# lvxianwei/DeepMerge

Measured on AMD Instinct MI355X. Metric: superpixel-pairs/sec (train step), higher is better.
Workload: dtype bf16; 1 GPU; ShfitScaleFormer_v3 depth [3, 2, 1], scales [32, 64, 128, 256] x 4ch (256x256x4 patches), 32 pairs/GPU/step, fwd+loss+bwd+allreduce+Adam (BASELINE configs[1]); pairs_per_gpu=32, global_batch=32, parallelism=dp1

## Files before the change

deepmerge_amd/_lib.py:

```python
from __future__ import annotations

import ctypes as C
import os
import re
import threading

HERE = os.path.dirname(os.path.abspath(__file__))
ROOT = os.path.dirname(HERE)
LIB_PATH = os.path.join(HERE, "libdeepmerge_hip.so")
HEADER_PATH = os.path.join(ROOT, "include", "deepmerge_hip.h")

DM_F32, DM_BF16 = 0, 1
DM_NT, DM_NN, DM_TN = 0, 1, 2
DM_BF16_PAIR = 2
DM_F64 = 3
DM_EPI_NONE, DM_EPI_GELU, DM_EPI_DGELU, DM_EPI_GELU_GRAD, DM_EPI_MUL = 0, 1, 2, 3, 4

_STATUS = {-1: "bad shape", -2: "bad dtype", -3: "bad alignment", -4: "workspace", -5: "HIP error", -6: "unsupported"}


class DeepMergeLibraryError(RuntimeError):
    pass


class DmGemmArgs(C.Structure):
    _fields_ = [
        ("layout", C.c_int32), ("ab_dtype", C.c_int32), ("c_dtype", C.c_int32), ("aux_dtype", C.c_int32),
        ("M", C.c_int32), ("N", C.c_int32), ("K", C.c_int32),
        ("epilogue", C.c_int32), ("accumulate", C.c_int32), ("split_k", C.c_int32),
        ("A", C.c_void_p), ("lda", C.c_int64),
        ("B", C.c_void_p), ("ldb", C.c_int64),
        ("C", C.c_void_p), ("ldc", C.c_int64),
        ("bias", C.c_void_p),
        ("residual", C.c_void_p), ("ldr", C.c_int64),
        ("aux", C.c_void_p), ("ldaux", C.c_int64),
        ("rows_per_group", C.c_int32), ("group_stride", C.c_int64),
        ("workspace", C.c_void_p), ("workspace_bytes", C.c_int64),
        ("colsum_a", C.c_void_p), ("colsum_accumulate", C.c_int32),
        ("k_fold", C.c_int32), ("a_fold", C.c_int64 * 3), ("b_fold", C.c_int64 * 3),
        ("c_plane", C.c_int64),
    ]


class DmReduceItem(C.Structure):
    _fields_ = [("partial", C.c_void_p), ("out0", C.c_void_p), ("out1", C.c_void_p),
                ("nrows", C.c_int32), ("width", C.c_int32), ("split", C.c_int32), ("accumulate", C.c_int32)]


class DmPairDraw(C.Structure):
    _fields_ = [("pairs", C.c_void_p), ("pair_flag", C.c_void_p), ("poly_off", C.c_void_p), ("poly_pts", C.c_void_p),
                ("pt_tile", C.c_void_p), ("pt_xy", C.c_void_p), ("pt_inner", C.c_void_p), ("pt_obj", C.c_void_p),
                ("pt_region", C.c_void_p),
                ("tile_id", C.c_void_p), ("xy", C.c_void_p), ("inner", C.c_void_p), ("obj", C.c_void_p),
                ("region", C.c_void_p), ("flag", C.c_void_p),
                ("point_id", C.c_void_p),
                ("seed", C.c_uint64),
                ("n_pairs", C.c_int32), ("n_poly", C.c_int32), ("n_poly_pts", C.c_int32), ("n_pts", C.c_int32),
                ("epoch", C.c_int32), ("batch", C.c_int32)]


class DmMergeFold(C.Structure):
    _fields_ = [("ptr", C.c_void_p), ("idx", C.c_void_p), ("edges", C.c_void_p), ("root", C.c_void_p), ("pick", C.c_void_p),
                ("rep", C.c_void_p), ("region_of", C.c_void_p),
                ("simi", C.c_void_p), ("weights", C.c_void_p),
                ("count", C.c_void_p), ("sum", C.c_void_p), ("sumsq", C.c_void_p), ("bbox", C.c_void_p), ("peri", C.c_void_p),
                ("new_id", C.c_void_p), ("hist_rank", C.c_void_p), ("new_ptr", C.c_void_p), ("new_idx", C.c_void_p),
                ("new_rep", C.c_void_p), ("new_region_of", C.c_void_p), ("n_regions", C.c_void_p),
                ("new_count", C.c_void_p), ("new_sum", C.c_void_p), ("new_sumsq", C.c_void_p), ("new_bbox", C.c_void_p),
                ("new_peri", C.c_void_p),
                ("history", C.c_void_p), ("history_simi", C.c_void_p),
                ("C", C.c_int32), ("P", C.c_int32), ("E", C.c_int32), ("S0", C.c_int32), ("bands", C.c_int32), ("round", C.c_int32),
                ("hist_base", C.c_int32), ("hist_cap", C.c_int32)]


class DmVectorTrace(C.Structure):
    _fields_ = [("dart", C.c_void_p), ("next", C.c_void_p), ("lab", C.c_void_p), ("other", C.c_void_p), ("flags", C.c_void_p),
                ("key", C.c_void_p), ("sum", C.c_void_p), ("ring_of_slot", C.c_void_p), ("ring_ptr", C.c_void_p),
                ("arc_base", C.c_void_p), ("xy", C.c_void_p), ("area2", C.c_void_p),
                ("arc_first", C.c_void_p), ("arc_left", C.c_void_p), ("arc_right", C.c_void_p), ("arc_vstart", C.c_void_p),
                ("arc_count", C.c_void_p), ("arc_pos", C.c_void_p), ("arc_ptr", C.c_void_p), ("arc_xy", C.c_void_p),
                ("W", C.c_int32), ("D", C.c_int32), ("R", C.c_int32), ("n_arcs", C.c_int32)]


class DmSceneVectorTrace(C.Structure):
    _fields_ = [("dart", C.c_void_p), ("next", C.c_void_p), ("lab", C.c_void_p), ("other", C.c_void_p), ("flags", C.c_void_p),
                ("key", C.c_void_p), ("sum", C.c_void_p), ("ring_of_slot", C.c_void_p), ("ring_ptr", C.c_void_p),
                ("arc_base", C.c_void_p), ("xy", C.c_void_p), ("area2", C.c_void_p),
                ("arc_first", C.c_void_p), ("arc_left", C.c_void_p), ("arc_right", C.c_void_p), ("arc_vstart", C.c_void_p),
                ("arc_count", C.c_void_p), ("arc_pos", C.c_void_p), ("arc_ptr", C.c_void_p), ("arc_xy", C.c_void_p),
                ("W", C.c_int64), ("D", C.c_int32), ("R", C.c_int32), ("n_arcs", C.c_int32)]


class DmSceneSimplifyRings(C.Structure):
    _fields_ = [("xy", C.c_void_p), ("ring_ptr", C.c_void_p), ("vert_ring", C.c_void_p), ("node_row", C.c_void_p), ("node_col", C.c_void_p),
                ("kept_row", C.c_void_p), ("status", C.c_void_p),
                ("n_nodes", C.c_int64), ("n_kept", C.c_int64), ("scene_h", C.c_int64), ("scene_w", C.c_int64),
                ("V", C.c_int32), ("R", C.c_int32)]


class DmSimplifyTopology(C.Structure):
    _fields_ = [("arc_xy", C.c_void_p), ("arc_ptr", C.c_void_p), ("new_ptr", C.c_void_p), ("keep", C.c_void_p),
                ("point_count", C.c_void_p), ("point_fill", C.c_void_p), ("point_ptr", C.c_void_p), ("point_xy", C.c_void_p),
                ("seg", C.c_void_p), ("kind", C.c_void_p), ("cell_count", C.c_void_p), ("cell_fill", C.c_void_p),
                ("cell_ptr", C.c_void_p), ("cell_seg", C.c_void_p), ("stack", C.c_void_p), ("status", C.c_void_p),
                ("Va", C.c_int64), ("cap", C.c_int64), ("A", C.c_int32), ("H", C.c_int32), ("W", C.c_int32), ("q", C.c_int32)]


class DmSceneSimplifyTopology(C.Structure):
    _fields_ = [("arc_xy", C.c_void_p), ("arc_ptr", C.c_void_p), ("new_ptr", C.c_void_p), ("arc_keep", C.c_void_p),
                ("point_count", C.c_void_p), ("point_fill", C.c_void_p), ("point_ptr", C.c_void_p), ("point_xy", C.c_void_p),
                ("seg", C.c_void_p), ("kind", C.c_void_p), ("cell_count", C.c_void_p), ("cell_fill", C.c_void_p),
                ("cell_ptr", C.c_void_p), ("cell_seg", C.c_void_p), ("stack", C.c_void_p), ("status", C.c_void_p),
                ("Va", C.c_int64), ("cap", C.c_int64), ("A", C.c_int32), ("H", C.c_int32), ("W", C.c_int32), ("q", C.c_int32),
                ("cell_log2", C.c_int32)]


class DmProfRow(C.Structure):
    _fields_ = [("name", C.c_char * 64), ("launches", C.c_int64), ("total_ms", C.c_double),
                ("total_flops", C.c_double), ("total_bytes", C.c_double)]


_P, _I, _L, _F, _D = C.c_void_p, C.c_int32, C.c_int64, C.c_float, C.c_double

SIGNATURES = {
    "dm_abi_version": (_I, []),
    "dm_last_error": (C.c_char_p, []),
    "dm_arch": (C.c_char_p, []),
    "dm_gemm": (_I, [C.POINTER(DmGemmArgs), _P]),
    "dm_gemm_workspace_bytes": (_L, [_I, _I, _I, _I]),
    "dm_gemm_grouped": (_I, [C.POINTER(DmGemmArgs), _I, _P]),
    "dm_attention_fwd": (_I, [_P, _P, _P, _P, _I, _I, _I, _I, _F, _I, _P]),
    "dm_attention_relpos_inkernel": (_I, [_I, _I, _I, _I, _I, _I, _I, _I]),
    "dm_attention_fwd_relpos": (_I, [_P, _P, _I, _I, _I, _P, _P, _I, _I, _I, _I, _F, _I, _P]),
    "dm_attention_split_ok": (_I, [_I, _I, _I, _I, _I, _I, _I, _I]),
    "dm_attention_split_fwd": (_I, [_P, _P, _P, _P, _I, _I, _I, _P, _P, _I, _I, _I, _I, _F, _P]),
    "dm_attention_split_fwd_pair": (_I, [_P, _P, _P, _P, _I, _I, _I, _P, _P, _P, _I, _I, _I, _I, _F, _P]),
    "dm_attention_split_bwd_chunks": (_I, [_I, _I, _I]),
    "dm_attention_split_bwd": (_I, [_P, _P, _P, _I, _I, _I, _P, _P, _P, _P, _P, _P, _P, _P, _I, _I, _I, _I, _F, _P]),
    "dm_attention_split_bwd_pair": (_I, [_P, _P, _P, _I, _I, _I, _P, _P, _P, _P, _P, _P, _P, _P, _I, _I, _I, _I, _F, _P]),
    "dm_attention_bwd_relpos": (_I, [_P, _P, _I, _I, _I, _P, _P, _P, _P, _P, _P, _P, _P, _I, _I, _I, _I, _F, _I, _P]),
    "dm_attention_bwd": (_I, [_P, _P, _P, _P, _P, _P, _P, _P, _P, _I, _I, _I, _I, _F, _I, _P]),
    "dm_attention_bwd_batch_chunks": (_I, [_I, _I, _I, _I]),
    "dm_relpos_bias_gather": (_I, [_P, _P, _P, _P, _I, _I, _I, _P]),
    "dm_relpos_bias_reduce": (_I, [_P, _P, _P, _P, _I, _I, _I, _I, _I, _P]),
    "dm_layernorm_fwd": (_I, [_P, _P, _P, _P, _I, _P, _P, _I, _I, _F, _P]),
    "dm_layernorm_bwd": (_I, [_P, _I, _P, _P, _P, _P, _P, _P, _P, _P, _P, _I, _P, _I, _I, _P]),
    "dm_layernorm_bwd_partials": (_I, [_P, _I, _P, _P, _P, _P, _P, _P, _P, _P, _I, _I, C.POINTER(C.c_int32), _P]),
    "dm_layernorm_bwd_partials_pair": (_I, [_P, _I, _P, _P, _P, _P, _P, _P, _P, _P, _I, _I, C.POINTER(C.c_int32), _P]),
    "dm_layernorm_bwd_partials_regroup": (_I, [_P, _I, _P, _P, _P, _P, _P, _P, _P, _P, _I, _I, _I, _I, C.POINTER(C.c_int32), _P]),
    "dm_pool_layernorm_ok": (_I, [_I]),
    "dm_pool_layernorm_fwd": (_I, [_P, _P, _P, _P, _P, _P, _P, _I, _I, _I, _I, _F, _P]),
    "dm_pool_layernorm_bwd": (_I, [_P, _P, _P, _P, _P, _P, _P, _P, _P, _I, _P, C.POINTER(C.c_int32), _I, _I, _I, _I, _P]),
    "dm_partial_reduce_batch": (_I, [C.POINTER(DmReduceItem), _I, _P]),
    "dm_layernorm_bwd_partial_floats": (_L, [_I]),
    "dm_token_pool_fwd": (_I, [_P, _P, _I, _I, _I, _I, _P]),
    "dm_token_pool_bwd": (_I, [_P, _P, _I, _I, _I, _I, _P]),
    "dm_group_mean_fwd": (_I, [_P, _P, _I, _I, _I, _P]),
    "dm_group_mean_bwd": (_I, [_P, _P, _I, _I, _I, _P]),
    "dm_colsum": (_I, [_P, _I, _L, _P, _I, _I, _I, _P, _P]),
    "dm_colsum_partial_floats": (_L, [_I]),
    "dm_cast": (_I, [_P, _P, _I, _L, _P]),
    "dm_split_bf16": (_I, [_P, _L, _L, _L, _P, _I, _I, _P]),
    "dm_split_colsum_partial_floats": (_L, [_L, _L]),
    "dm_split_bf16_colsum": (_I, [_P, _L, _L, _L, _P, _I, _I, _P, _P, _P]),
    "dm_split_bf16_planes": (_I, [_P, _L, _L, _L, _P, _P, _P, _P]),
    "dm_patchify": (_I, [_P, _P, _I, _I, _I, _I, _I, _P]),
    "dm_contrastive_loss": (_I, [_P, _P, _P, _F, _F, _P, _P, _P, _I, _I, _P]),
    "dm_cross_entropy": (_I, [_P, _P, _P, _F, _P, _P, _I, _I, _P]),
    "dm_batchnorm_workspace_bytes": (_L, [_I, _I]),
    "dm_batchnorm_fwd": (_I, [_P, _P, _P, _P, _P, _P, _I, _P, _P, _P, _I, _I, _F, _F, _I, _I, _P, _P]),
    "dm_batchnorm_bwd": (_I, [_P, _P, _P, _P, _P, _I, _P, _P, _P, _P, _P, _I, _I, _I, _I, _I, _P, _P]),
    "dm_adam_step": (_I, [_P, _P, _P, _P, _P, _L, _I, _D, _D, _D, _D, _D, _P]),
    "dm_adam_hyper": (_I, [_I, _D, _D, _D, _P]),
    "dm_adam_step_dev": (_I, [_P, _P, _P, _P, _P, _L, _P, _D, _D, _D, _D, _P]),
    "dm_adam_step_dev_pair": (_I, [_P, _P, _P, _P, _P, _P, _L, _P, _D, _D, _D, _D, _P]),
    "dm_segment_mean": (_I, [_P, _P, _P, _P, _I, _I, _P]),
    "dm_edge_similarity": (_I, [_P, _P, _P, _P, _I, _I, _F, _P]),
    "dm_pairwise_distance": (_I, [_P, _P, _P, _I, _I, _I, _I, _P]),
    "dm_patch_pyramid": (_I, [_P, _I, _I, _I, _P, _P, _I, _I, _I, _I, _P, _P]),
    "dm_patch_pyramid_cols": (_I, [_P, _I, _I, _I, _P, _P, _I, _I, _I, _I, _I, _P, _I, _P]),
    "dm_pair_batch_gather": (_I, [_P, _I, _I, _I, _I, _P, _P, _P, _P, _I, _I, _I, _I, _I, _I, _P, _I, _P, _P, _P, _P]),
    "dm_pair_epoch_draw": (_I, [C.POINTER(DmPairDraw), _P]),
    "dm_contrastive_terms": (_I, [_P, _P, _P, _F, _P, _P, _I, _I, _P]),
    "dm_pair_eval_workspace_bytes": (_L, [_L, _I]),
    "dm_pair_eval_summary": (_I, [_P, _P, _P, _L, _P, _I, _P, _P, _P, _P, _P]),
    "dm_label_stats": (_I, [_P, _P, _I, _I, _I, _I, _P, _P, _P, _P, _P, _P]),
    "dm_label_features": (_I, [_P, _P, _P, _P, _P, _I, _I, _P, _P]),
    "dm_rag_edges": (_I, [_P, _I, _I, _I, _P, _P, _I, _P, _P, _I, _P, _P, _P]),
    "dm_seam_stitch": (_I, [_P, _P, _L, _L, _P, _P, _P, _I, _P, _P, _I, _P, _P, _P]),
    "dm_merge_round": (_I, [_P, _P, _I, _I, _P, _P, _I, _P]),
    "dm_merge_best": (_I, [_P, _P, _I, _I, _F, _P, _P]),
    "dm_merge_match": (_I, [_P, _P, _I, _I, _P, _P, _P, _P, _P]),
    "dm_merge_fold_regions": (_I, [C.POINTER(DmMergeFold), _P]),
    "dm_merge_edge_keys": (_I, [_P, _P, _P, _I, _I, _P, _P]),
    "dm_merge_fold_edges": (_I, [_P, _P, _P, _I, _P, _P, _P, _P]),
    "dm_relabel_raster": (_I, [_P, _P, _P, _L, _I, _P]),
    "dm_region_merge_cost": (_I, [_P, _P, _P, _P, _P, _P, _P, _I, _I, _I, _D, _D, _D, _D, _D, _P, _P]),
    "dm_pixel_regions": (_I, [_P, _I, _I, _I, _P, _P, _P, _P, _P, _P, _P, _P]),
    "dm_label_clearance": (_I, [_P, _I, _I, _I, _P, _P, _P, _P]),
    "dm_point_select_round": (_I, [_P, _P, _I, _I, _I, _I, _I, _P, _P, _P, _P, _P, _P]),
    "dm_point_emit": (_I, [_P, _P, _P, _P, _I, _I, _I, _I, _P, _P, _P, _P, _P, _P, _P]),
    "dm_scene_point_init": (_I, [_P, _P, _P, _I, _P]),
    "dm_scene_point_select": (_I, [_P, _P, _I, _I, _I, _I, _I, _I, _L, _L, _L, _L, _I, _I, _I, _P, _P, _P, _P, _P]),
    "dm_scene_point_commit": (_I, [_P, _L, _L, _I, _I, _P, _P, _P, _P]),
    "dm_label_overlap": (_I, [_P, _P, _I, _I, _L, _L, _P, _P, _I, _P, _P, _I, _P, _P, _P]),
    "dm_overlap_reduce": (_I, [_P, _P, _I, _L, _L, _P, _P, _P, _P, _P, _P, _P, _P, _P]),
    "dm_pair_flags": (_I, [_P, _I, _P, _P, _P, _I, _I, _P, _P]),
    "dm_boundary_bits": (_I, [_P, _I, _I, _I, _P, _P, _P, _P]),
    "dm_boundary_counts": (_I, [_P, _P, _P, _I, _I, _I, _I, _I, _I, _I, _P, _P]),
    "dm_slic_iterate": (_I, [_P, _I, _I, _I, _I, _I, _I, _P, _P, _P, _P]),
    "dm_connected_labels": (_I, [_P, _I, _I, _I, _I, _P, _P, _P, _P, _P]),
    "dm_label_area": (_I, [_P, _I, _I, _I, _P, _P]),
    "dm_slic_absorb_pick": (_I, [_P, _P, _I, _P, _I, _I, _P, _P, _P, _P]),
    "dm_scene_slic_init": (_I, [_P, _I, _I, _I, _I, _I, _I, _I, _I, _P, _P, _P]),
    "dm_scene_slic_pass": (_I, [_P, _I, _I, _I, _I, _I, _I, _I, _I, _I, _P, _P, _P, _P]),
    "dm_scene_slic_update": (_I, [_I, _P, _P, _P]),
    "dm_vector_count": (_I, [_P, _I, _I, _P, _P, _P, _P]),
    "dm_vector_emit": (_I, [_P, _P, _I, _I, _P, _P, _P]),
    "dm_vector_link": (_I, [_P, _P, _P, _P, _I, _I, _I, _P, _P, _P, _P, _P, _P]),
    "dm_vector_head_round": (_I, [_P, _P, _P, _P, _I, _P, _P]),
    "dm_vector_rank_init": (_I, [_P, _P, _P, _P, _I, _P, _P, _P, _P, _P, _I, _P]),
    "dm_vector_rank_round": (_I, [_P, _P, _P, _P, _I, _P, _P]),
    "dm_vector_ring_emit": (_I, [C.POINTER(DmVectorTrace), _P]),
    "dm_vector_arc_emit": (_I, [C.POINTER(DmVectorTrace), _P]),
    "dm_scene_vector_count": (_I, [_P, _I, _I, _I, _I, _I, _I, _P, _P, _P, _P, _P]),
    "dm_scene_vector_link": (_I, [_P, _P, _P, _I, _I, _I, _L, _L, _L, _L, _P, _P, _P, _P, _P, _P]),
    "dm_scene_vector_ring_emit": (_I, [C.POINTER(DmSceneVectorTrace), _P]),
    "dm_scene_vector_arc_emit": (_I, [C.POINTER(DmSceneVectorTrace), _P]),
    "dm_rasterize_count": (_I, [_P, _P, _P, _I, _I, _I, _I, _P, _P]),
    "dm_rasterize_emit": (_I, [_P, _P, _P, _P, _P, _I, _I, _L, _I, _I, _L, _P, _P]),
    "dm_rasterize_fill": (_I, [_P, _L, _I, _I, _I, _P, _P, _P]),
    "dm_rasterize_count_rows": (_I, [_P, _P, _P, _I, _I, _I, _I, _I, _I, _P, _P]),
    "dm_rasterize_emit_rows": (_I, [_P, _P, _P, _P, _P, _I, _I, _L, _I, _I, _I, _I, _L, _P, _P]),
    "dm_rasterize_fill_window": (_I, [_P, _L, _I, _I, _I, _I, _I, _I, _I, _P, _P, _P]),
    "dm_simplify_nodes": (_I, [_P, _I, _I, _P, _P]),
    "dm_simplify_chains": (_I, [_P, _P, _I, _L, _I, _I, _I, _P, _P, _P]),
    "dm_simplify_arc_count": (_I, [_P, _P, _I, _L, _I, _I, _P, _P, _P]),
    "dm_simplify_arc_emit": (_I, [_P, _P, _P, _I, _L, _L, _I, _I, _P, _P, _P]),
    "dm_simplify_ring_count": (_I, [_P, _P, _P, _I, _I, _I, _I, _P, _P, _P]),
    "dm_simplify_ring_emit": (_I, [_P, _P, _P, _P, _P, _I, _I, _L, _I, _I, _P, _P, _P, _P]),
    "dm_simplify_topology_point_count": (_I, [C.POINTER(DmSimplifyTopology), _P]),
    "dm_simplify_topology_point_fill": (_I, [C.POINTER(DmSimplifyTopology), _P]),
    "dm_simplify_topology_segments": (_I, [C.POINTER(DmSimplifyTopology), _P]),
    "dm_simplify_topology_bin_count": (_I, [C.POINTER(DmSimplifyTopology), _P]),
    "dm_simplify_topology_bin_fill": (_I, [C.POINTER(DmSimplifyTopology), _P]),
    "dm_simplify_topology_pairs": (_I, [C.POINTER(DmSimplifyTopology), _P]),
    "dm_simplify_topology_jumps": (_I, [C.POINTER(DmSimplifyTopology), _P]),
    "dm_simplify_topology_refine": (_I, [C.POINTER(DmSimplifyTopology), _I, _P]),
    "dm_scene_simplify_node_count": (_I, [_P, _I, _I, _I, _I, _I, _I, _L, _L, _L, _L, _P, _P, _P]),
    "dm_scene_simplify_node_emit": (_I, [_P, _I, _I, _I, _I, _I, _I, _L, _L, _L, _L, _P, _I, _P, _P]),
    "dm_scene_simplify_chains": (_I, [_P, _P, _I, _L, _L, _L, _I, _P, _P, _P]),
    "dm_scene_simplify_arc_count": (_I, [_P, _P, _I, _L, _L, _L, _P, _P, _P]),
    "dm_scene_simplify_arc_emit": (_I, [_P, _P, _P, _I, _L, _L, _L, _L, _P, _P, _P]),
    "dm_scene_simplify_ring_count": (_I, [C.POINTER(DmSceneSimplifyRings), _P, _P]),
    "dm_scene_simplify_ring_emit": (_I, [C.POINTER(DmSceneSimplifyRings), _P, _P, _L, _P, _P, _P]),
    "dm_scene_simplify_topology_point_count": (_I, [C.POINTER(DmSceneSimplifyTopology), _P]),
    "dm_scene_simplify_topology_point_fill": (_I, [C.POINTER(DmSceneSimplifyTopology), _P]),
    "dm_scene_simplify_topology_segments": (_I, [C.POINTER(DmSceneSimplifyTopology), _P]),
    "dm_scene_simplify_topology_bin_count": (_I, [C.POINTER(DmSceneSimplifyTopology), _P]),
    "dm_scene_simplify_topology_bin_fill": (_I, [C.POINTER(DmSceneSimplifyTopology), _P]),
    "dm_scene_simplify_topology_pairs": (_I, [C.POINTER(DmSceneSimplifyTopology), _P]),
    "dm_scene_simplify_topology_jumps": (_I, [C.POINTER(DmSceneSimplifyTopology), _P]),
    "dm_scene_simplify_topology_refine": (_I, [C.POINTER(DmSceneSimplifyTopology), _I, _P]),
    "dm_gru_cell_fwd": (_I, [_P, _L, _P, _P, _P, _P, _I, _I, _P]),
    "dm_gru_cell_bwd": (_I, [_P, _P, _P, _P, _P, _P, _I, _I, _P]),
    "dm_prof_enable": (_I, [_I]),
    "dm_prof_collect": (_I, [C.POINTER(DmProfRow), _I]),
}

_lock = threading.Lock()
_lib = None


def declared_symbols(header_path: str = HEADER_PATH):
    text = open(header_path).read()
    text = re.sub(r"/\*.*?\*/", "", text, flags=re.S)
    return sorted(set(re.findall(r"\b(dm_[a-z0-9_]+)\s*\(", text)))


def lib() -> C.CDLL:
    global _lib
    if _lib is not None:
        return _lib
    with _lock:
        if _lib is not None:
            return _lib
        if not os.path.exists(LIB_PATH):
            raise DeepMergeLibraryError(
                f"{LIB_PATH} not found: build the HIP kernels first "
                f"(`python -c 'import __graft_entry__ as g; g.build()'` or `make -C deepmerge_amd/csrc`). "
                f"deepmerge_amd has no CPU fallback.")
        try:
            handle = C.CDLL(LIB_PATH)
        except OSError as e:
            raise DeepMergeLibraryError(f"cannot load {LIB_PATH}: {e}") from e
        for name, (res, args) in SIGNATURES.items():
            try:
                fn = getattr(handle, name)
            except AttributeError as e:
                raise DeepMergeLibraryError(f"{LIB_PATH} does not export {name}") from e
            fn.restype = res
            fn.argtypes = args
        if handle.dm_abi_version() != 7:
            raise DeepMergeLibraryError(f"ABI version mismatch: library {handle.dm_abi_version()} != 7")
        _lib = handle
        return _lib
# ... 11 lines not shown
```

deepmerge_amd/csrc/dm_rows.hip:

```cpp
#include <cstdlib>

#include "dm_common.h"

int dm_layernorm_wide_fwd(const float *x, const float *gamma, const float *beta, void *y, int y_dtype, float *mean, float *rstd, int rows,
                          int cols, float eps, hipStream_t s);
int dm_layernorm_wide_bwd(const void *dy, int dy_dtype, const float *x, const float *gamma, const float *mean, const float *rstd,
                          const float *dres, float *dx, void *dx_lp, float *partial, int max_slices, int *slices, int rows, int cols,
                          hipStream_t s);
int dm_patchify_any(const float *x, void *cols, int dtype, int B, int C, int side, int p, hipStream_t s);

namespace {

constexpr int MAXCH = 4;
constexpr int LN_WIDE_MAX = 8192;
static int ln_max_wg() {
  static const int v = [] { const char *e = getenv("DM_LN_WG"); return e ? atoi(e) : 768; }();
  return v;
}
constexpr int CS_MAX_SLICES = 64;

template <typename T> struct Raw4;
template <> struct Raw4<float> { typedef f32x4 type; };
template <> struct Raw4<bf16_t> { typedef bf16x4 type; };
template <typename T>
__device__ __forceinline__ typename Raw4<T>::type dm_load_raw4(const T *p) { return *reinterpret_cast<const typename Raw4<T>::type *>(p); }
__device__ __forceinline__ f32x4 dm_widen4(f32x4 v) { return v; }
__device__ __forceinline__ f32x4 dm_widen4(bf16x4 v) { return (f32x4){(float)v[0], (float)v[1], (float)v[2], (float)v[3]}; }

template <typename TY, bool PAIR, int CH, bool FULL, bool POOL = false>
__global__ __launch_bounds__(256) void layernorm_fwd_kernel(const float *__restrict__ x, const float *__restrict__ gamma,
                                                            const float *__restrict__ beta, TY *__restrict__ y,
                                                            float *__restrict__ mean_out, float *__restrict__ rstd_out,
                                                            int rows, int cols, float eps, float *__restrict__ pooled = nullptr, int pool_side = 0) {
  __shared__ f32x4 gb[2][CH * 64];
  const int lane = threadIdx.x & 63, wave = __builtin_amdgcn_readfirstlane(threadIdx.x >> 6);
  const int nch = cols >> 2;
  for (int c = threadIdx.x; c < nch; c += 256) {
    gb[0][c] = dm_load4(gamma + 4 * c);
    gb[1][c] = dm_load4(beta + 4 * c);
  }
  __syncthreads();
  const int stride = gridDim.x * 4;
  int row = blockIdx.x * 4 + wave;
  if (row >= rows) return;
  auto request = [&](int r, f32x4(&dst)[CH]) __attribute__((always_inline)) {
    if constexpr (POOL) {
      const int half = pool_side >> 1, px = r % half, q = r / half, py = q % half, bs = q / half;
      const float *src = x + (((long long)bs * pool_side + 2 * py) * pool_side + 2 * px) * cols;
      const long long down = (long long)pool_side * cols;
      float *pr = pooled + (long long)r * cols;
#pragma unroll
      for (int i = 0; i < CH; ++i) {
        const int c = lane + 64 * i;
        if (FULL || c < nch) {
          const f32x4 a = dm_load4(src + 4 * c), b = dm_load4(src + cols + 4 * c), d = dm_load4(src + down + 4 * c), e = dm_load4(src + down + cols + 4 * c);
          dst[i] = ((a + b) + (d + e)) * 0.25f;
          dm_store4(pr + 4 * c, dst[i]);
        } else {
          dst[i] = (f32x4){0.f, 0.f, 0.f, 0.f};
        }
      }
      return;
    }
    const float *xr = x + (long long)r * cols;
#pragma unroll
    for (int i = 0; i < CH; ++i) {
      const int c = lane + 64 * i;
      dst[i] = (FULL || c < nch) ? dm_load4(xr + 4 * c) : (f32x4){0.f, 0.f, 0.f, 0.f};
    }
  };
  auto finish = [&](int row, const f32x4(&v)[CH]) __attribute__((always_inline)) {
    float s = 0.f;
#pragma unroll
    for (int i = 0; i < CH; ++i) s += (v[i][0] + v[i][1]) + (v[i][2] + v[i][3]);
    const float mean = dm_wave_sum(s) / (float)cols;
    float q = 0.f;
#pragma unroll
    for (int i = 0; i < CH; ++i) {
      const int c = lane + 64 * i;
      if (FULL || c < nch) {
#pragma unroll
        for (int e = 0; e < 4; ++e) {
          const float d = v[i][e] - mean;
          q += d * d;
        }
      }
    }
    const float rstd = rsqrtf(dm_wave_sum(q) / (float)cols + eps);
    if (lane == 0) {
      mean_out[row] = mean;
      rstd_out[row] = rstd;
    }
    TY *yr = y + (long long)row * cols;
#pragma unroll
    for (int i = 0; i < CH; ++i) {
      const int c = lane + 64 * i;
      if (FULL || c < nch) {
        int cl = c;
        asm volatile("" : "+v"(cl));
        const f32x4 g = gb[0][cl], b = gb[1][cl];
        f32x4 o;
#pragma unroll
        for (int e = 0; e < 4; ++e) o[e] = (v[i][e] - mean) * rstd * g[e] + b[e];
        if constexpr (PAIR) {
          bf16x4 h, l;
#pragma unroll
          for (int e = 0; e < 4; ++e) {
            h[e] = (bf16_t)o[e];
            l[e] = (bf16_t)(o[e] - (float)h[e]);
          }
          *reinterpret_cast<bf16x4 *>(yr + 4 * c) = h;
          *reinterpret_cast<bf16x4 *>(yr + (long long)rows * cols + 4 * c) = l;
        } else {
          dm_store4(yr + 4 * c, o);
        }
      }
    }
  };
  f32x4 v[CH], nv[CH];
  if constexpr (!FULL || POOL) {
    for (; row < rows; row += stride) {
      request(row, v);
      finish(row, v);
    }
    return;
  }
  request(row, v);
  int next = row + stride;
  if (next < rows) request(next, nv);
  finish(row, v);
  while (next < rows) {
    row = next;
    next = row + stride;
#pragma unroll
    for (int i = 0; i < CH; ++i) v[i] = nv[i];
    if (next < rows) request(next, nv);
    finish(row, v);
  }
}

template <typename TDY, int CH, bool FULL, bool POOL = false>
__global__ __launch_bounds__(256) void layernorm_bwd_kernel(const TDY *__restrict__ dy, const float *__restrict__ x,
                                                            const float *__restrict__ gamma, const float *__restrict__ mean,
                                                            const float *__restrict__ rstd, const float *__restrict__ dres,
                                                            float *__restrict__ dx, bf16_t *__restrict__ dx_lp,
                                                            float *__restrict__ partial, int rows, int cols, long long lp_plane,
                                                            int pool_side = 0, int rg_s = 0, int rg_t = 0) {
  __shared__ float red[4][2][CH * 256];
  const int lane = threadIdx.x & 63, wave = __builtin_amdgcn_readfirstlane(threadIdx.x >> 6);
  const int nch = cols >> 2;
  f32x4 dg[CH], db[CH], gam[CH];
#pragma unroll
  for (int i = 0; i < CH; ++i) {
    dg[i] = db[i] = (f32x4){0.f, 0.f, 0.f, 0.f};
    const int c = lane + 64 * i;
    gam[i] = (FULL || c < nch) ? dm_load4(gamma + 4 * c) : (f32x4){0.f, 0.f, 0.f, 0.f};
  }
  f32x4 rx[CH], rdr[CH];
  typename Raw4<TDY>::type rdy[CH];
  float rmu = 0.f, rrs = 0.f;
  auto request = [&](int row) __attribute__((always_inline)) {
    const long long off = (long long)row * cols;
    rmu = mean[row];
    rrs = rstd[row];
#pragma unroll
    for (int i = 0; i < CH; ++i) {
      const int c = lane + 64 * i;
      rdr[i] = (dres && (FULL || c < nch)) ? dm_load4(dres + off + 4 * c) : (f32x4){0.f, 0.f, 0.f, 0.f};
    }
#pragma unroll
    for (int i = 0; i < CH; ++i) {
      const int c = lane + 64 * i;
      if (FULL || c < nch) {
        rx[i] = dm_load4(x + off + 4 * c);
        rdy[i] = dm_load_raw4(dy + off + 4 * c);
      }
    }
  };
  f32x4 xh[CH], g[CH], dr[CH];
  float rs = 0.f, s1 = 0.f, s2 = 0.f;
  auto consume = [&]() __attribute__((always_inline)) {
    const float mu = rmu;
    rs = rrs;
    s1 = s2 = 0.f;
#pragma unroll
    for (int i = 0; i < CH; ++i) {
      const int c = lane + 64 * i;
      dr[i] = rdr[i];
      if (FULL || c < nch) {
        const f32x4 xv = rx[i];
        const f32x4 d = dm_widen4(rdy[i]);
#pragma unroll
        for (int e = 0; e < 4; ++e) {
          xh[i][e] = (xv[e] - mu) * rs;
          g[i][e] = d[e] * gam[i][e];
          s1 += g[i][e];
          s2 += g[i][e] * xh[i][e];
          dg[i][e] += d[e] * xh[i][e];
          db[i][e] += d[e];
        }
      } else {
        xh[i] = g[i] = (f32x4){0.f, 0.f, 0.f, 0.f};
      }
    }
  };
  auto finish = [&](int row) __attribute__((always_inline)) {
    const long long off = (long long)row * cols;
    float t1 = s1, t2 = s2;
#pragma unroll
    for (int o = 32; o > 0; o >>= 1) {
      const float u1 = __shfl_xor(t1, o, 64), u2 = __shfl_xor(t2, o, 64);
      t1 += u1;
      t2 += u2;
    }
    const float c1 = t1 / (float)cols, c2 = t2 / (float)cols;
    if constexpr (POOL) {
      const int half = pool_side >> 1, px = row % half, q = row / half, py = q % half, bs = q / half;
      const long long base = (((long long)bs * pool_side + 2 * py) * pool_side + 2 * px) * cols, down = (long long)pool_side * cols;
#pragma unroll
      for (int i = 0; i < CH; ++i) {
        const int c = lane + 64 * i;
        if (FULL || c < nch) {
          f32x4 o;
#pragma unroll
          for (int e = 0; e < 4; ++e) o[e] = rs * (g[i][e] - c1 - xh[i][e] * c2);
          o = o * 0.25f;
          const long long at[4] = {base, base + cols, base + down, base + down + cols};
#pragma unroll
          for (int k = 0; k < 4; ++k) {
            dm_store4(dx + at[k] + 4 * c, o);
            if (dx_lp) dm_store4(dx_lp + at[k] + 4 * c, o);
          }
        }
      }
      return;
    }
    long long off_lp = off;
    if (rg_t > 0) {
      const int st = rg_s * rg_t, b = row / st, rem = row - b * st, sc = rem / rg_t, t = rem - sc * rg_t;
      off_lp = ((long long)(sc * (rows / st) + b) * rg_t + t) * cols;
    }
#pragma unroll
    for (int i = 0; i < CH; ++i) {
      const int c = lane + 64 * i;
      if (FULL || c < nch) {
        f32x4 o;
#pragma unroll
        for (int e = 0; e < 4; ++e) o[e] = rs * (g[i][e] - c1 - xh[i][e] * c2);
        if (dres) o += dr[i];
        dm_store4(dx + off + 4 * c, o);
        if (dx_lp) {
          if (lp_plane > 0) {
            bf16x4 h, l;
#pragma unroll
            for (int e = 0; e < 4; ++e) {
              h[e] = (bf16_t)o[e];
              l[e] = (bf16_t)(o[e] - (float)h[e]);
            }
            *reinterpret_cast<bf16x4 *>(dx_lp + off + 4 * c) = h;
            *reinterpret_cast<bf16x4 *>(dx_lp + lp_plane + off + 4 * c) = l;
          } else {
            dm_store4(dx_lp + off_lp + 4 * c, o);
          }
        }
      }
    }
  };
  int row = blockIdx.x * 4 + wave;
  const int stride = gridDim.x * 4;
  if constexpr (CH == MAXCH) {
    for (; row < rows; row += stride) {
      request(row);
      consume();
      finish(row);
    }
  } else if (row < rows) {
    request(row);
    consume();
    for (;;) {
      const int next = row + stride;
      if (next < rows) request(next);
      finish(row);
      if (next >= rows) break;
      row = next;
      consume();
    }
  }
#pragma unroll
  for (int i = 0; i < CH; ++i) {
#pragma unroll
    for (int e = 0; e < 4; ++e) {
      red[wave][0][(lane + 64 * i) * 4 + e] = dg[i][e];
      red[wave][1][(lane + 64 * i) * 4 + e] = db[i][e];
    }
  }
  __syncthreads();
  float *prow = partial + (long long)blockIdx.x * 2 * cols;
  for (int c = threadIdx.x; c < 2 * cols; c += 256) {
    const int which = c / cols, col = c % cols;
    prow[c] = (red[0][which][col] + red[1][which][col]) + (red[2][which][col] + red[3][which][col]);
  }
}

__global__ __launch_bounds__(256) void partial_reduce_kernel(const float *__restrict__ partial, float *__restrict__ out0,
                                                             float *__restrict__ out1, int nrows, int width, int split,
                                                             int accumulate) {
  __shared__ float red[16][17];
  const int tx = threadIdx.x & 15, ty = threadIdx.x >> 4;
  const int j = blockIdx.x * 16 + tx;
  float s = 0.f;
  if (j < width) {
    float s0 = 0.f, s1 = 0.f, s2 = 0.f, s3 = 0.f;
    int r = ty;
    for (; r + 48 < nrows; r += 64) {
      s0 += partial[(long long)r * width + j];
      s1 += partial[(long long)(r + 16) * width + j];
      s2 += partial[(long long)(r + 32) * width + j];
      s3 += partial[(long long)(r + 48) * width + j];
    }
    for (; r < nrows; r += 16) s0 += partial[(long long)r * width + j];
    s = (s0 + s1) + (s2 + s3);
  }
  red[ty][tx] = s;
  __syncthreads();
  if (ty == 0 && j < width) {
    float t[16];
#pragma unroll
    for (int k = 0; k < 16; ++k) t[k] = red[k][tx];
#pragma unroll
    for (int w = 8; w > 0; w >>= 1)
#pragma unroll
      for (int k = 0; k < w; ++k) t[k] = t[2 * k] + t[2 * k + 1];
    s = t[0];
    float *o = (j < split) ? out0 + j : out1 + (j - split);
    *o = accumulate ? *o + s : s;
  }
}

struct ReduceBatch {
  DmReduceItem it[32];
  int start[33];
  int n;
};
__global__ __launch_bounds__(256) void partial_reduce_batch_kernel(const ReduceBatch rb) {
  __shared__ float red[16][17];
  int job = 0;
  while (job + 1 < rb.n && (int)blockIdx.x >= rb.start[job + 1]) ++job;
  const DmReduceItem &it = rb.it[job];
  const float *__restrict__ partial = it.partial;
  const int nrows = it.nrows, width = it.width;
  const int tx = threadIdx.x & 15, ty = threadIdx.x >> 4;
  const int j = ((int)blockIdx.x - rb.start[job]) * 16 + tx;
  float s = 0.f;
  if (j < width) {
    float s0 = 0.f, s1 = 0.f, s2 = 0.f, s3 = 0.f;
    int r = ty;
    for (; r + 48 < nrows; r += 64) {
      s0 += partial[(long long)r * width + j];
      s1 += partial[(long long)(r + 16) * width + j];
      s2 += partial[(long long)(r + 32) * width + j];
      s3 += partial[(long long)(r + 48) * width + j];
    }
    for (; r < nrows; r += 16) s0 += partial[(long long)r * width + j];
    s = (s0 + s1) + (s2 + s3);
  }
  red[ty][tx] = s;
  __syncthreads();
  if (ty == 0 && j < width) {
    float t[16];
#pragma unroll
    for (int k = 0; k < 16; ++k) t[k] = red[k][tx];
#pragma unroll
    for (int w = 8; w > 0; w >>= 1)
#pragma unroll
      for (int k = 0; k < w; ++k) t[k] = t[2 * k] + t[2 * k + 1];
    s = t[0];
    float *o = (j < it.split) ? it.out0 + j : it.out1 + (j - it.split);
    *o = it.accumulate ? *o + s : s;
  }
}

__global__ void token_pool_fwd_kernel(const float *__restrict__ x, float *__restrict__ y, int B, int S, int side, int C) {
  const int half = side >> 1, c4 = C >> 2;
  const long long total = (long long)B * S * half * half * c4;
  for (long long i = (long long)blockIdx.x * blockDim.x + threadIdx.x; i < total; i += (long long)gridDim.x * blockDim.x) {
    const int c = (int)(i % c4);
    long long r = i / c4;
    const int px = (int)(r % half); r /= half;
    const int py = (int)(r % half); r /= half;
    const float *src = x + ((r * side + 2 * py) * side + 2 * px) * (long long)C + 4 * c;
    const f32x4 a = dm_load4(src), b = dm_load4(src + C), d = dm_load4(src + (long long)side * C), e = dm_load4(src + (long long)side * C + C);
    dm_store4(y + ((r * half + py) * half + px) * (long long)C + 4 * c, ((a + b) + (d + e)) * 0.25f);
  }
}
__global__ void token_pool_bwd_kernel(const float *__restrict__ dy, float *__restrict__ dx, int B, int S, int side, int C) {
  const int half = side >> 1, c4 = C >> 2;
  const long long total = (long long)B * S * side * side * c4;
  for (long long i = (long long)blockIdx.x * blockDim.x + threadIdx.x; i < total; i += (long long)gridDim.x * blockDim.x) {
    const int c = (int)(i % c4);
    long long r = i / c4;
    const int xx = (int)(r % side); r /= side;
    const int yy = (int)(r % side); r /= side;
    const f32x4 g = dm_load4(dy + ((r * half + (yy >> 1)) * half + (xx >> 1)) * (long long)C + 4 * c);
    dm_store4(dx + ((r * side + yy) * side + xx) * (long long)C + 4 * c, g * 0.25f);
  }
}
__global__ void group_mean_fwd_kernel(const float *__restrict__ x, float *__restrict__ y, int rows, int g, int C) {
  const int c4 = C >> 2;
  const long long total = (long long)rows * c4;
  const float inv = 1.0f / (float)g;
  for (long long i = (long long)blockIdx.x * blockDim.x + threadIdx.x; i < total; i += (long long)gridDim.x * blockDim.x) {
    const int c = (int)(i % c4);
    const long long r = i / c4;
    f32x4 s = {0.f, 0.f, 0.f, 0.f};
    for (int k = 0; k < g; ++k) s += dm_load4(x + (r * g + k) * C + 4 * c);
    dm_store4(y + r * C + 4 * c, s * inv);
  }
}
__global__ void group_mean_bwd_kernel(const float *__restrict__ dy, float *__restrict__ dx, int rows, int g, int C) {
  const int c4 = C >> 2;
  const long long total = (long long)rows * g * c4;
  const float inv = 1.0f / (float)g;
  for (long long i = (long long)blockIdx.x * blockDim.x + threadIdx.x; i < total; i += (long long)gridDim.x * blockDim.x) {
    const int c = (int)(i % c4);
    const long long r = i / c4;
    dm_store4(dx + r * C + 4 * c, dm_load4(dy + (r / g) * C + 4 * c) * inv);
  }
}

template <typename T>
__global__ __launch_bounds__(256) void colsum_kernel(const T *__restrict__ X, long long ldx, float *__restrict__ partial,
                                                     int M, int N, int rows_per_slice, int direct) {
  __shared__ f32x4 red[16][16];
  const int tx = threadIdx.x & 15, ty = threadIdx.x >> 4;
  const int n = blockIdx.x * 64 + tx * 4;
  const int r0 = blockIdx.y * rows_per_slice, r1 = min(M, r0 + rows_per_slice);
  f32x4 s = {0.f, 0.f, 0.f, 0.f};
  if (n < N)
    for (int r = r0 + ty; r < r1; r += 16) s += dm_load4(X + (long long)r * ldx + n);
  red[ty][tx] = s;
  __syncthreads();
  if (ty == 0 && n < N) {
    f32x4 a = red[0][tx];
#pragma unroll
    for (int k = 1; k < 16; ++k) a += red[k][tx];
    if (direct == 1) a = dm_load4(partial + n) + a;
    dm_store4(partial + (long long)blockIdx.y * N + n, a);
  }
}

template <typename T>
__global__ __launch_bounds__(256) void colsum_generic_kernel(const T *__restrict__ X, long long ldx, float *__restrict__ partial,
                                                             int M, int N, int rows_per_slice) {
  const int n = blockIdx.x * 256 + threadIdx.x;
  if (n >= N) return;
  const int r0 = blockIdx.y * rows_per_slice, r1 = min(M, r0 + rows_per_slice);
  float s = 0.f;
  for (int r = r0; r < r1; ++r) s += (float)X[(long long)r * ldx + n];
  partial[(long long)blockIdx.y * N + n] = s;
}

__global__ void cast_bf16_kernel(const float *__restrict__ src, bf16_t *__restrict__ dst, long long n) {
  const long long n8 = n >> 3;
  for (long long i = (long long)blockIdx.x * blockDim.x + threadIdx.x; i < n8; i += (long long)gridDim.x * blockDim.x) {
    const f32x4 a = dm_load4(src + 8 * i), b = dm_load4(src + 8 * i + 4);
    bf16x8 o = {(bf16_t)a[0], (bf16_t)a[1], (bf16_t)a[2], (bf16_t)a[3], (bf16_t)b[0], (bf16_t)b[1], (bf16_t)b[2], (bf16_t)b[3]};
    *reinterpret_cast<bf16x8 *>(dst + 8 * i) = o;
  }
  if (blockIdx.x == 0 && threadIdx.x < (n & 7)) dst[(n8 << 3) + threadIdx.x] = (bf16_t)src[(n8 << 3) + threadIdx.x];
}
__global__ void split_bf16_kernel(const float *__restrict__ src, long long ld, long long rows, long long cols, bf16_t *__restrict__ dst,
                                  int stack, int pattern) {
  const long long c4 = cols >> 2, total = rows * c4;
  const long long piece = stack ? rows * cols : cols, ldd = stack ? cols : 3 * cols;
  for (long long i = (long long)blockIdx.x * blockDim.x + threadIdx.x; i < total; i += (long long)gridDim.x * blockDim.x) {
    const long long r = i / c4, c = (i - r * c4) << 2;
    const f32x4 x = dm_load4(src + r * ld + c);
    bf16x4 hi, lo;
#pragma unroll
    for (int j = 0; j < 4; ++j) {
      hi[j] = (bf16_t)x[j];
      lo[j] = (bf16_t)(x[j] - (float)hi[j]);
    }
    bf16_t *d = dst + r * ldd + c;
#pragma unroll
    for (int j = 0; j < 3; ++j) *reinterpret_cast<bf16x4 *>(d + j * piece) = ((pattern >> j) & 1) ? lo : hi;
  }
}
template <bool CS>
__global__ __launch_bounds__(256) void split_bf16_rows_kernel(const float *__restrict__ src, long long ld, int rows, int cols,
                                                              bf16_t *__restrict__ dst, int stack, int pattern, float *__restrict__ partial, int pieces) {
  __shared__ float red[CS ? 8 : 1][CS ? 264 : 1];
  const int c = (blockIdx.x * 32 + threadIdx.x) * 8;
  const bool live = c < cols;
  if (!CS && !live) return;
  const long long piece = stack ? (long long)rows * cols : cols, ldd = stack ? cols : 3LL * cols;
  float cs[8] = {0.f, 0.f, 0.f, 0.f, 0.f, 0.f, 0.f, 0.f};
  for (int r = blockIdx.y * 8 + threadIdx.y; live && r < rows; r += gridDim.y * 8) {
    const float *sp = src + (long long)r * ld + c;
    const f32x4 x0 = dm_load4(sp), x1 = dm_load4(sp + 4);
    if constexpr (CS) {
#pragma unroll
      for (int j = 0; j < 4; ++j) { cs[j] += x0[j]; cs[4 + j] += x1[j]; }
    }
    u32x4 hi, lo;
#pragma unroll
    for (int j = 0; j < 4; ++j) {
      const float a = j < 2 ? x0[2 * j] : x1[2 * j - 4], b = j < 2 ? x0[2 * j + 1] : x1[2 * j - 3];
      const bf16x2 h2 = {(bf16_t)a, (bf16_t)b};
      const bf16x2 l2 = {(bf16_t)(a - (float)h2[0]), (bf16_t)(b - (float)h2[1])};
      hi[j] = __builtin_bit_cast(unsigned, h2);
      lo[j] = __builtin_bit_cast(unsigned, l2);
    }
    bf16_t *d = dst + (long long)r * ldd + c;
#pragma unroll
    for (int j = 0; j < 3; ++j)
      if (j < pieces) *reinterpret_cast<u32x4 *>(d + j * piece) = ((pattern >> j) & 1) ? lo : hi;
  }
  if constexpr (CS) {
#pragma unroll
    for (int j = 0; j < 8; ++j) red[threadIdx.y][threadIdx.x * 8 + j] = cs[j];
    __syncthreads();
    if (threadIdx.y == 0 && live) {
#pragma unroll
      for (int j = 0; j < 8; ++j) {
        const int x = threadIdx.x * 8 + j;
        partial[(long long)blockIdx.y * cols + c + j] = ((red[0][x] + red[1][x]) + (red[2][x] + red[3][x])) + ((red[4][x] + red[5][x]) + (red[6][x] + red[7][x]));
      }
    }
  }
}
__global__ void copy_f32_kernel(const float *__restrict__ src, float *__restrict__ dst, long long n) {
  const long long n4 = n >> 2;
  for (long long i = (long long)blockIdx.x * blockDim.x + threadIdx.x; i < n4; i += (long long)gridDim.x * blockDim.x)
    dm_store4(dst + 4 * i, dm_load4(src + 4 * i));
  if (blockIdx.x == 0 && threadIdx.x < (n & 3)) dst[(n4 << 2) + threadIdx.x] = src[(n4 << 2) + threadIdx.x];
}

template <typename T>
__global__ void patchify_kernel(const float *__restrict__ x, T *__restrict__ cols, int B, int C, int side, int p) {
  const int grid = side / p, p4 = p >> 2;
  const long long K = (long long)C * p * p;
  const long long total = (long long)B * grid * grid * (K >> 2);
  for (long long i = (long long)blockIdx.x * blockDim.x + threadIdx.x; i < total; i += (long long)gridDim.x * blockDim.x) {
    long long r = i;
    const int dx4 = (int)(r % p4); r /= p4;
    const int dy = (int)(r % p); r /= p;
    const int c = (int)(r % C); r /= C;
    const int px = (int)(r % grid);
    const long long bp = r / grid;
    const int py = (int)(bp % grid);
    const long long b = bp / grid;
    const f32x4 v = dm_load4(x + ((b * C + c) * side + (py * p + dy)) * (long long)side + px * p + 4 * dx4);
    dm_store4(cols + r * K + ((long long)c * p + dy) * p + 4 * dx4, v);
  }
}

__global__ __launch_bounds__(256) void contrastive_loss_kernel(const float *__restrict__ a, const float *__restrict__ b,
                                                               const float *__restrict__ flag, float margin, float upstream,
                                                               float *__restrict__ loss, float *__restrict__ da,
                                                               float *__restrict__ db, int B, int D) {
  __shared__ float wsum[4];
  const int lane = threadIdx.x & 63, wave = threadIdx.x >> 6;
  float acc = 0.f;
  const float gscale = upstream / (float)B;
  for (int r = wave; r < B; r += 4) {
    float d = 0.f;
    for (int c = lane; c < D; c += 64) {
      const float t = a[(long long)r * D + c] - b[(long long)r * D + c];
      d += t * t;
    }
    d = dm_wave_sum(d);
    const float f = flag[r];
    const float hinge = margin - d;
    acc += f * d + (1.f - f) * fmaxf(hinge, 0.f);
    if (da) {
      const float coef = (f - (1.f - f) * (hinge > 0.f ? 1.f : 0.f)) * 2.f * gscale;
      for (int c = lane; c < D; c += 64) {
        const float t = a[(long long)r * D + c] - b[(long long)r * D + c];
        da[(long long)r * D + c] = coef * t;
        db[(long long)r * D + c] = -coef * t;
      }
    }
  }
  if (lane == 0) wsum[wave] = acc;
  __syncthreads();
  if (threadIdx.x == 0) loss[0] = ((wsum[0] + wsum[1]) + (wsum[2] + wsum[3])) / (float)B;
}

__global__ __launch_bounds__(256) void cross_entropy_kernel(const float *__restrict__ logits, const long long *__restrict__ tidx,
                                                            const float *__restrict__ tprob, float upstream,
                                                            float *__restrict__ loss, float *__restrict__ dlogits, int B, int K) {
  __shared__ float wsum[4];
  const int lane = threadIdx.x & 63, wave = threadIdx.x >> 6;
  const float gscale = upstream / (float)B;
  float acc = 0.f;
  for (int r = wave; r < B; r += 4) {
    const float *x = logits + (long long)r * K;
    float mx = -INFINITY;
    for (int c = lane; c < K; c += 64) mx = fmaxf(mx, x[c]);
    mx = dm_wave_max(mx);
    float se = 0.f;
    for (int c = lane; c < K; c += 64) se += expf(x[c] - mx);
    se = dm_wave_sum(se);
    const float lse = mx + logf(se);
    float l = 0.f, psum = 0.f;
    if (tidx) {
      const long long t = tidx[r];
      if (lane == 0) l = lse - x[t];
      psum = 1.f;
    } else {
      const float *q = tprob + (long long)r * K;
      for (int c = lane; c < K; c += 64) { l += q[c] * (lse - x[c]); psum += q[c]; }
      psum = dm_wave_sum(psum);
    }
    acc += dm_wave_sum(l);
    if (dlogits) {
      float *g = dlogits + (long long)r * K;
      for (int c = lane; c < K; c += 64) {
        const float sm = expf(x[c] - lse);
        const float tgt = tidx ? ((long long)c == tidx[r] ? 1.f : 0.f) : tprob[(long long)r * K + c];
        g[c] = (sm * psum - tgt) * gscale;
      }
    }
  }
  if (lane == 0) wsum[wave] = acc;
  __syncthreads();
  if (threadIdx.x == 0) loss[0] = ((wsum[0] + wsum[1]) + (wsum[2] + wsum[3])) / (float)B;
}

__global__ void adam_kernel(float *__restrict__ param, const float *__restrict__ grad, float *__restrict__ m,
                            float *__restrict__ v, bf16_t *__restrict__ lp, long long n, float beta1, float beta2,
                            float omb1, float omb2, float eps, float step_size, float bc2_sqrt, float grad_scale,
                            const float *__restrict__ hyper, bf16_t *__restrict__ lo = nullptr) {
  if (hyper) {
    step_size = hyper[0];
    bc2_sqrt = hyper[1];
  }
  const long long n4 = n >> 2;
  for (long long i = (long long)blockIdx.x * blockDim.x + threadIdx.x; i < n4; i += (long long)gridDim.x * blockDim.x) {
    f32x4 p = __builtin_nontemporal_load(reinterpret_cast<const f32x4 *>(param + 4 * i));
    f32x4 g = __builtin_nontemporal_load(reinterpret_cast<const f32x4 *>(grad + 4 * i)) * grad_scale;
    f32x4 mm = __builtin_nontemporal_load(reinterpret_cast<const f32x4 *>(m + 4 * i)), vv = __builtin_nontemporal_load(reinterpret_cast<const f32x4 *>(v + 4 * i));
#pragma unroll
    for (int e = 0; e < 4; ++e) {
      mm[e] = mm[e] * beta1 + g[e] * omb1;
      vv[e] = vv[e] * beta2 + (g[e] * g[e]) * omb2;
      const float denom = sqrtf(vv[e]) / bc2_sqrt + eps;
      p[e] = p[e] - step_size * (mm[e] / denom);
    }
    __builtin_nontemporal_store(p, reinterpret_cast<f32x4 *>(param + 4 * i));
    __builtin_nontemporal_store(mm, reinterpret_cast<f32x4 *>(m + 4 * i));
    __builtin_nontemporal_store(vv, reinterpret_cast<f32x4 *>(v + 4 * i));
    if (lp) dm_store4(lp + 4 * i, p);
    if (lo) {
      bf16x4 l;
#pragma unroll
      for (int e = 0; e < 4; ++e) l[e] = (bf16_t)(p[e] - (float)(bf16_t)p[e]);
      *reinterpret_cast<bf16x4 *>(lo + 4 * i) = l;
    }
  }
  if (blockIdx.x == 0 && threadIdx.x < (n & 3)) {
    const long long i = (n4 << 2) + threadIdx.x;
    const float g = grad[i] * grad_scale;
    const float mm = m[i] * beta1 + g * omb1;
    const float vv = v[i] * beta2 + (g * g) * omb2;
    const float p = param[i] - step_size * (mm / (sqrtf(vv) / bc2_sqrt + eps));
    param[i] = p; m[i] = mm; v[i] = vv;
    if (lp) lp[i] = (bf16_t)p;
    if (lo) lo[i] = (bf16_t)(p - (float)(bf16_t)p);
  }
}

__global__ void relpos_gather_kernel(const float *__restrict__ table, const int *__restrict__ index,
                                     float *__restrict__ bias, float *__restrict__ bias_t, int N, int H, int n_bins) {
  const int NN = N * N;
  for (int ij = blockIdx.x * blockDim.x + threadIdx.x; ij < NN; ij += gridDim.x * blockDim.x) {
    int bin = index[ij];
    bin = min(max(bin, 0), n_bins - 1);
    for (int h = 0; h < H; ++h) bias[(long long)h * NN + ij] = table[bin * H + h];
    if (bias_t) {
      const int i = ij / N, j = ij % N;
      int bt = index[j * N + i];
      bt = min(max(bt, 0), n_bins - 1);
      for (int h = 0; h < H; ++h) bias_t[(long long)h * NN + ij] = table[bt * H + h];
    }
  }
}
template <int U>
__device__ __forceinline__ void chunk_add(f32x4 &v, const float *slab, long long plane4, long long i, int c) {
  f32x4 a[U];
#pragma unroll
  for (int u = 0; u < U; ++u) a[u] = dm_load4(slab + ((long long)(c + u) * plane4 + i) * 4);
#pragma unroll
  for (int u = 0; u < U; ++u) v += a[u];
}
__global__ void chunk_sum_kernel(float *__restrict__ slab, long long plane4, int chunks) {
  for (long long i = (long long)blockIdx.x * blockDim.x + threadIdx.x; i < plane4; i += (long long)gridDim.x * blockDim.x) {
    f32x4 v = dm_load4(slab + 4 * i);
    int c = 1;
    for (; c + 8 <= chunks; c += 8) chunk_add<8>(v, slab, plane4, i, c);
    if (c + 4 <= chunks) { chunk_add<4>(v, slab, plane4, i, c); c += 4; }
    if (c + 2 <= chunks) { chunk_add<2>(v, slab, plane4, i, c); c += 2; }
    if (c < chunks) chunk_add<1>(v, slab, plane4, i, c);
    dm_store4(slab + 4 * i, v);
  }
}

__global__ __launch_bounds__(256) void relpos_reduce_kernel(const float *__restrict__ slab, const int *__restrict__ pos,
                                                            const int *__restrict__ off, float *__restrict__ dtable, int chunks,
                                                            int H, int N, int n_bins, int accumulate) {
  const int lane = threadIdx.x & 63, wave = threadIdx.x >> 6;
  const int bin = blockIdx.x, h = blockIdx.y * 4 + wave;
  if (h >= H) return;
  const int beg = off[bin], cnt = off[bin + 1] - beg;
  const long long plane = (long long)N * N;
  float acc = 0.f;
  for (int c = 0; c < chunks; ++c) {
    const float *pl = slab + ((long long)c * H + h) * plane;
#pragma unroll 4
    for (int j = lane; j < cnt; j += 64) acc += pl[pos[beg + j]];
  }
  acc = dm_wave_sum(acc);
  if (lane == 0) {
    float *o = dtable + (long long)bin * H + h;
    *o = accumulate ? *o + acc : acc;
  }
}

inline int grid_for(long long work_items, int block = 256, int cap = 4096) {
  long long g = (work_items + block - 1) / block;
  if (g < 1) g = 1;
  if (g > cap) g = cap;
  return (int)g;
}

static int adam_grid(long long n) {
  static const int cap = [] { const char *e = getenv("DM_ADAM_GRID"); return e ? atoi(e) : 16384; }();
  return grid_for(n / 4 + 1, 256, cap);
}

}

extern "C" int dm_layernorm_fwd(const float *x, const float *gamma, const float *beta, void *y, int32_t y_dtype,
                                float *mean, float *rstd, int32_t rows, int32_t cols, float eps, void *stream) {
  DM_REQUIRE(rows > 0 && cols > 0 && cols % 4 == 0 && cols <= LN_WIDE_MAX, DM_ERR_BAD_SHAPE,
             "dm_layernorm_fwd: rows=%d cols=%d (cols must be a multiple of 4, <= %d)", rows, cols, LN_WIDE_MAX);
  DM_REQUIRE(x && gamma && beta && y && mean && rstd, DM_ERR_BAD_SHAPE, "dm_layernorm_fwd: null pointer");
  hipStream_t s = reinterpret_cast<hipStream_t>(stream);
  if (cols > MAXCH * 256) {
    DM_REQUIRE(y_dtype != DM_BF16_PAIR, DM_ERR_UNSUPPORTED, "dm_layernorm_fwd: a plane-pair result needs cols <= %d", MAXCH * 256);
    const int rc = dm_layernorm_wide_fwd(x, gamma, beta, y, y_dtype, mean, rstd, rows, cols, eps, s);
    DM_REQUIRE(rc == DM_OK, rc, "dm_layernorm_fwd: bad y_dtype %d", y_dtype);
    DM_LAUNCH_CHECK("dm_layernorm_fwd(wide)");
    return DM_OK;
  }
  const int grid = grid_for((long long)rows, 4, 2048);
  const bool full3 = cols == 768;
#define DM_LN_FWD(T, PAIR_)                                                                                                                \
  do {                                                                                                                                     \
    if (full3)                                                                                                                             \
      hipLaunchKernelGGL((layernorm_fwd_kernel<T, PAIR_, 3, true>), dim3(grid), dim3(256), 0, s, x, gamma, beta, (T *)y, mean, rstd, rows, cols, eps); \
    else                                                                                                                                   \
      hipLaunchKernelGGL((layernorm_fwd_kernel<T, PAIR_, MAXCH, false>), dim3(grid), dim3(256), 0, s, x, gamma, beta, (T *)y, mean, rstd, rows, cols, eps); \
  } while (0)
  if (y_dtype == DM_F32) DM_LN_FWD(float, false);
  else if (y_dtype == DM_BF16) DM_LN_FWD(bf16_t, false);
  else if (y_dtype == DM_BF16_PAIR) DM_LN_FWD(bf16_t, true);
  else DM_REQUIRE(false, DM_ERR_BAD_DTYPE, "dm_layernorm_fwd: bad y_dtype %d", y_dtype);
#undef DM_LN_FWD
  DM_LAUNCH_CHECK("dm_layernorm_fwd");
  return DM_OK;
}

extern "C" int64_t dm_layernorm_bwd_partial_floats(int32_t cols) { return (int64_t)ln_max_wg() * 2 * cols; }

static int ln_bwd_main(const void *dy, int32_t dy_dtype, const float *x, const float *gamma, const float *mean, const float *rstd,
                       const float *dres, float *dx, void *dx_lp, float *partial, int32_t rows, int32_t cols, int32_t *n_partial, hipStream_t s,
                       const char *who, bool lp_pair = false, int pool_side = 0, int rg_s = 0, int rg_t = 0) {
  const long long lp_plane = lp_pair ? (long long)rows * cols : 0;
  DM_REQUIRE(!lp_pair || (dx_lp && cols <= MAXCH * 256), DM_ERR_UNSUPPORTED, "%s: the plane-pair copy needs dx_lp and cols <= %d", who, MAXCH * 256);
  DM_REQUIRE(rows > 0 && cols > 0 && cols % 4 == 0 && cols <= LN_WIDE_MAX, DM_ERR_BAD_SHAPE, "%s: rows=%d cols=%d", who, rows, cols);
  DM_REQUIRE(dy && x && gamma && mean && rstd && dx && partial && n_partial, DM_ERR_BAD_SHAPE, "%s: null pointer", who);
  if (cols > MAXCH * 256) {
    int slices = 0;
    const int rc = dm_layernorm_wide_bwd(dy, dy_dtype, x, gamma, mean, rstd, dres, dx, dx_lp, partial, ln_max_wg(), &slices, rows, cols, s);
    DM_REQUIRE(rc == DM_OK, rc, "%s: bad dy_dtype %d", who, dy_dtype);
    DM_LAUNCH_CHECK("dm_layernorm_bwd(wide)");
    *n_partial = slices;
    return DM_OK;
  }
  const int grid = grid_for((long long)rows, 4, ln_max_wg());
  DM_REQUIRE(dy_dtype == DM_F32 || dy_dtype == DM_BF16, DM_ERR_BAD_DTYPE, "%s: bad dy_dtype %d", who, dy_dtype);
  if (pool_side > 0) {
    hipLaunchKernelGGL((layernorm_bwd_kernel<float, 3, true, true>), dim3(grid), dim3(256), 0, s, (const float *)dy, x, gamma, mean, rstd, (const float *)nullptr,
                       dx, (bf16_t *)dx_lp, partial, rows, cols, 0LL, pool_side, 0, 0);
    DM_LAUNCH_CHECK("dm_pool_layernorm_bwd");
    *n_partial = grid;
    return DM_OK;
  }
  const bool narrow = cols <= 768, full = cols == 768;
#define DM_LN_BWD(T, CH_, FULL_)                                                                                                      \
  hipLaunchKernelGGL((layernorm_bwd_kernel<T, CH_, FULL_>), dim3(grid), dim3(256), 0, s, (const T *)dy, x, gamma, mean, rstd, dres, dx, \
                     (bf16_t *)dx_lp, partial, rows, cols, lp_plane, 0, rg_s, rg_t)
  if (dy_dtype == DM_F32) {
    if (full) DM_LN_BWD(float, 3, true);
    else if (narrow) DM_LN_BWD(float, 3, false);
    else DM_LN_BWD(float, MAXCH, false);
  } else {
    if (full) DM_LN_BWD(bf16_t, 3, true);
    else if (narrow) DM_LN_BWD(bf16_t, 3, false);
    else DM_LN_BWD(bf16_t, MAXCH, false);
  }
#undef DM_LN_BWD
  DM_LAUNCH_CHECK("dm_layernorm_bwd");
  *n_partial = grid;
  return DM_OK;
}

extern "C" int dm_layernorm_bwd(const void *dy, int32_t dy_dtype, const float *x, const float *gamma, const float *mean,
                                const float *rstd, const float *dres, float *dx, void *dx_lp, float *dgamma, float *dbeta,
                                int32_t accumulate_params, float *partial, int32_t rows, int32_t cols, void *stream) {
  DM_REQUIRE(dgamma && dbeta, DM_ERR_BAD_SHAPE, "dm_layernorm_bwd: null pointer");
  hipStream_t s = reinterpret_cast<hipStream_t>(stream);
  int32_t slices = 0;
  if (const int rc = ln_bwd_main(dy, dy_dtype, x, gamma, mean, rstd, dres, dx, dx_lp, partial, rows, cols, &slices, s, "dm_layernorm_bwd")) return rc;
  hipLaunchKernelGGL(partial_reduce_kernel, dim3((2 * cols + 15) / 16), dim3(256), 0, s, partial, dgamma, dbeta, slices, 2 * cols, cols, accumulate_params);
  DM_LAUNCH_CHECK("dm_layernorm_bwd(reduce)");
  return DM_OK;
}

extern "C" int dm_layernorm_bwd_partials(const void *dy, int32_t dy_dtype, const float *x, const float *gamma, const float *mean,
                                         const float *rstd, const float *dres, float *dx, void *dx_lp, float *partial, int32_t rows,
                                         int32_t cols, int32_t *n_partial, void *stream) {
  return ln_bwd_main(dy, dy_dtype, x, gamma, mean, rstd, dres, dx, dx_lp, partial, rows, cols, n_partial, reinterpret_cast<hipStream_t>(stream),
                     "dm_layernorm_bwd_partials");
}

extern "C" int dm_layernorm_bwd_partials_pair(const void *dy, int32_t dy_dtype, const float *x, const float *gamma, const float *mean,
                                              const float *rstd, const float *dres, float *dx, void *dx_pair, float *partial, int32_t rows,
                                              int32_t cols, int32_t *n_partial, void *stream) {
  return ln_bwd_main(dy, dy_dtype, x, gamma, mean, rstd, dres, dx, dx_pair, partial, rows, cols, n_partial, reinterpret_cast<hipStream_t>(stream),
                     "dm_layernorm_bwd_partials_pair", true);
}

extern "C" int dm_layernorm_bwd_partials_regroup(const void *dy, int32_t dy_dtype, const float *x, const float *gamma, const float *mean,
                                                 const float *rstd, const float *dres, float *dx, void *dx_lp, float *partial, int32_t rows,
                                                 int32_t cols, int32_t S, int32_t T, int32_t *n_partial, void *stream) {
  DM_REQUIRE(dx_lp && S > 0 && T > 0 && rows > 0 && rows % (S * T) == 0, DM_ERR_BAD_SHAPE,
             "dm_layernorm_bwd_partials_regroup: rows=%d must be whole (S=%d, T=%d) groups, and dx_lp set", rows, S, T);
  DM_REQUIRE(cols <= MAXCH * 256, DM_ERR_UNSUPPORTED, "dm_layernorm_bwd_partials_regroup: cols=%d (the register-resident widths only, <= %d)", cols, MAXCH * 256);
  return ln_bwd_main(dy, dy_dtype, x, gamma, mean, rstd, dres, dx, dx_lp, partial, rows, cols, n_partial, reinterpret_cast<hipStream_t>(stream),
                     "dm_layernorm_bwd_partials_regroup", false, 0, S, T);
}

extern "C" int dm_pool_layernorm_ok(int32_t cols) { return cols == 768; }

extern "C" int dm_pool_layernorm_fwd(const float *x, const float *gamma, const float *beta, float *pooled, float *y, float *mean, float *rstd,
                                     int32_t B, int32_t S, int32_t side, int32_t C, float eps, void *stream) {
  DM_REQUIRE(B > 0 && S > 0 && side >= 2 && side % 2 == 0 && (long long)B * S * (side / 2) * (side / 2) < (1LL << 31), DM_ERR_BAD_SHAPE,
             "dm_pool_layernorm_fwd: B=%d S=%d side=%d C=%d", B, S, side, C);
  DM_REQUIRE(dm_pool_layernorm_ok(C), DM_ERR_UNSUPPORTED, "dm_pool_layernorm_fwd: C=%d (768 only: pool and normalise in two calls)", C);
  DM_REQUIRE(x && gamma && beta && pooled && y && mean && rstd, DM_ERR_BAD_SHAPE, "dm_pool_layernorm_fwd: null pointer");
  const int rows = B * S * (side / 2) * (side / 2);
  hipLaunchKernelGGL((layernorm_fwd_kernel<float, false, 3, true, true>), dim3(grid_for((long long)rows, 4, 2048)), dim3(256), 0,
                     reinterpret_cast<hipStream_t>(stream), x, gamma, beta, y, mean, rstd, rows, C, eps, pooled, side);
  DM_LAUNCH_CHECK("dm_pool_layernorm_fwd");
  return DM_OK;
}

extern "C" int dm_pool_layernorm_bwd(const float *dy, const float *pooled, const float *gamma, const float *mean, const float *rstd, float *dx,
                                     void *dx_lp, float *dgamma, float *dbeta, int32_t accumulate_params, float *partial, int32_t *n_partial,
                                     int32_t B, int32_t S, int32_t side, int32_t C, void *stream) {
  DM_REQUIRE(B > 0 && S > 0 && side >= 2 && side % 2 == 0 && (long long)B * S * (side / 2) * (side / 2) < (1LL << 31), DM_ERR_BAD_SHAPE,
             "dm_pool_layernorm_bwd: B=%d S=%d side=%d C=%d", B, S, side, C);
  DM_REQUIRE(dm_pool_layernorm_ok(C), DM_ERR_UNSUPPORTED, "dm_pool_layernorm_bwd: C=%d (768 only: the three separate calls)", C);
  DM_REQUIRE((dgamma != nullptr) == (dbeta != nullptr) && (dgamma || n_partial), DM_ERR_BAD_SHAPE,
             "dm_pool_layernorm_bwd: dgamma and dbeta together, or n_partial for the partial rows alone");
  hipStream_t s = reinterpret_cast<hipStream_t>(stream);
  const int rows = B * S * (side / 2) * (side / 2);
  int32_t slices = 0;
  if (const int rc = ln_bwd_main(dy, DM_F32, pooled, gamma, mean, rstd, nullptr, dx, dx_lp, partial, rows, C, &slices, s, "dm_pool_layernorm_bwd", false, side))
    return rc;
  if (n_partial) *n_partial = slices;
  if (dgamma) {
    hipLaunchKernelGGL(partial_reduce_kernel, dim3((2 * C + 15) / 16), dim3(256), 0, s, partial, dgamma, dbeta, slices, 2 * C, C, accumulate_params);
    DM_LAUNCH_CHECK("dm_pool_layernorm_bwd(reduce)");
  }
  return DM_OK;
}

extern "C" int dm_partial_reduce_batch(const DmReduceItem *items, int32_t n, void *stream) {
  DM_REQUIRE(items && n > 0, DM_ERR_BAD_SHAPE, "dm_partial_reduce_batch: no items");
  hipStream_t s = reinterpret_cast<hipStream_t>(stream);
  for (int32_t base = 0; base < n; base += 32) {
    ReduceBatch rb;
    rb.n = (n - base < 32) ? n - base : 32;
    int total = 0;
    for (int i = 0; i < rb.n; ++i) {
      const DmReduceItem &it = items[base + i];
      DM_REQUIRE(it.partial && it.out0 && it.out1 && it.nrows > 0 && it.width > 0 && it.split >= 0 && it.split <= it.width, DM_ERR_BAD_SHAPE,
                 "dm_partial_reduce_batch: item %d: nrows=%d width=%d split=%d", base + i, it.nrows, it.width, it.split);
      rb.it[i] = it;
      rb.start[i] = total;
      total += (it.width + 15) / 16;
    }
    for (int i = rb.n; i <= 32; ++i) rb.start[i] = total;
    hipLaunchKernelGGL(partial_reduce_batch_kernel, dim3(total), dim3(256), 0, s, rb);
    DM_LAUNCH_CHECK("dm_partial_reduce_batch");
  }
  return DM_OK;
}

extern "C" int dm_token_pool_fwd(const float *x, float *y, int32_t B, int32_t S, int32_t side, int32_t C, void *stream) {
  DM_REQUIRE(B > 0 && S > 0 && side >= 2 && side % 2 == 0 && C % 4 == 0, DM_ERR_BAD_SHAPE, "dm_token_pool_fwd: B=%d S=%d side=%d C=%d", B, S, side, C);
  const long long total = (long long)B * S * (side / 2) * (side / 2) * (C / 4);
  hipLaunchKernelGGL(token_pool_fwd_kernel, dim3(grid_for(total)), dim3(256), 0, reinterpret_cast<hipStream_t>(stream), x, y, B, S, side, C);
  DM_LAUNCH_CHECK("dm_token_pool_fwd");
  return DM_OK;
}
extern "C" int dm_token_pool_bwd(const float *dy, float *dx, int32_t B, int32_t S, int32_t side, int32_t C, void *stream) {
  DM_REQUIRE(B > 0 && S > 0 && side >= 2 && side % 2 == 0 && C % 4 == 0, DM_ERR_BAD_SHAPE, "dm_token_pool_bwd: B=%d S=%d side=%d C=%d", B, S, side, C);
  const long long total = (long long)B * S * side * side * (C / 4);
  hipLaunchKernelGGL(token_pool_bwd_kernel, dim3(grid_for(total)), dim3(256), 0, reinterpret_cast<hipStream_t>(stream), dy, dx, B, S, side, C);
  DM_LAUNCH_CHECK("dm_token_pool_bwd");
  return DM_OK;
}
extern "C" int dm_group_mean_fwd(const float *x, float *y, int32_t rows, int32_t g, int32_t C, void *stream) {
  DM_REQUIRE(rows > 0 && g > 0 && C % 4 == 0, DM_ERR_BAD_SHAPE, "dm_group_mean_fwd: rows=%d g=%d C=%d", rows, g, C);
  hipLaunchKernelGGL(group_mean_fwd_kernel, dim3(grid_for((long long)rows * (C / 4))), dim3(256), 0, reinterpret_cast<hipStream_t>(stream), x, y, rows, g, C);
  DM_LAUNCH_CHECK("dm_group_mean_fwd");
  return DM_OK;
}
extern "C" int dm_group_mean_bwd(const float *dy, float *dx, int32_t rows, int32_t g, int32_t C, void *stream) {
  DM_REQUIRE(rows > 0 && g > 0 && C % 4 == 0, DM_ERR_BAD_SHAPE, "dm_group_mean_bwd: rows=%d g=%d C=%d", rows, g, C);
  hipLaunchKernelGGL(group_mean_bwd_kernel, dim3(grid_for((long long)rows * g * (C / 4))), dim3(256), 0, reinterpret_cast<hipStream_t>(stream), dy, dx, rows, g, C);
  DM_LAUNCH_CHECK("dm_group_mean_bwd");
  return DM_OK;
}

extern "C" int64_t dm_colsum_partial_floats(int32_t N) { return (int64_t)CS_MAX_SLICES * N; }

extern "C" int dm_colsum(const void *X, int32_t dtype, int64_t ldx, float *out, int32_t M, int32_t N, int32_t accumulate,
                         float *partial, void *stream) {
  DM_REQUIRE(M > 0 && N > 0 && ldx >= N, DM_ERR_BAD_SHAPE, "dm_colsum: M=%d N=%d ldx=%lld", M, N, (long long)ldx);
  const bool vec = (N % 4 == 0) && (ldx % 4 == 0) && dm_aligned16(X);
  DM_REQUIRE(X && out && partial, DM_ERR_BAD_SHAPE, "dm_colsum: null pointer");
  hipStream_t s = reinterpret_cast<hipStream_t>(stream);
  int slices = (M + 255) / 256;
  if (slices > CS_MAX_SLICES) slices = CS_MAX_SLICES;
  const int rps = (M + slices - 1) / slices;
  slices = (M + rps - 1) / rps;
  dim3 grid((N + 63) / 64, slices), ggrid((N + 255) / 256, slices);
  const bool direct = slices == 1 && vec && dm_aligned16(out);
  float *dst = direct ? out : partial;
  const int dflag = direct ? (accumulate ? 1 : 0) : -1;
  if (dtype == DM_F32) {
    if (vec) hipLaunchKernelGGL(colsum_kernel<float>, grid, dim3(256), 0, s, (const float *)X, (long long)ldx, dst, M, N, rps, dflag);
    else hipLaunchKernelGGL(colsum_generic_kernel<float>, ggrid, dim3(256), 0, s, (const float *)X, (long long)ldx, partial, M, N, rps);
  } else if (dtype == DM_BF16) {
    if (vec) hipLaunchKernelGGL(colsum_kernel<bf16_t>, grid, dim3(256), 0, s, (const bf16_t *)X, (long long)ldx, dst, M, N, rps, dflag);
    else hipLaunchKernelGGL(colsum_generic_kernel<bf16_t>, ggrid, dim3(256), 0, s, (const bf16_t *)X, (long long)ldx, partial, M, N, rps);
  } else DM_REQUIRE(false, DM_ERR_BAD_DTYPE, "dm_colsum: bad dtype %d", dtype);
  DM_LAUNCH_CHECK("dm_colsum");
  if (direct) return DM_OK;
  hipLaunchKernelGGL(partial_reduce_kernel, dim3((N + 15) / 16), dim3(256), 0, s, partial, out, out, slices, N, N, accumulate);
  DM_LAUNCH_CHECK("dm_colsum(reduce)");
  return DM_OK;
}

extern "C" int dm_cast(const float *src, void *dst, int32_t dst_dtype, int64_t n, void *stream) {
  DM_REQUIRE(src && dst && n > 0, DM_ERR_BAD_SHAPE, "dm_cast: bad arguments");
  hipStream_t s = reinterpret_cast<hipStream_t>(stream);
  if (dst_dtype == DM_BF16) hipLaunchKernelGGL(cast_bf16_kernel, dim3(grid_for(n / 8 + 1)), dim3(256), 0, s, src, (bf16_t *)dst, (long long)n);
  else if (dst_dtype == DM_F32) hipLaunchKernelGGL(copy_f32_kernel, dim3(grid_for(n / 4 + 1)), dim3(256), 0, s, src, (float *)dst, (long long)n);
  else DM_REQUIRE(false, DM_ERR_BAD_DTYPE, "dm_cast: bad dtype %d", dst_dtype);
  DM_LAUNCH_CHECK("dm_cast");
  return DM_OK;
}

static bool split_rows_ok(const float *src, int64_t ld, int64_t rows, int64_t cols, const void *dst, int32_t stack) {
  return cols % 8 == 0 && rows < (1LL << 31) && cols < (1LL << 31) && dm_aligned16(src) && dm_aligned16(dst) && ld % 4 == 0 &&
         (stack ? (rows * cols) % 8 == 0 : true);
}
static void split_rows_grid(int64_t rows, int64_t cols, int &gx, int &gy, bool colsum = false) {
  gx = (int)((cols / 8 + 31) / 32);
  long long y = (rows + 7) / 8;
  const int blocks = colsum ? 2048 : 8192;
  const long long cap = blocks / gx > 0 ? blocks / gx : 1;
  gy = (int)(y > cap ? cap : y);
}

extern "C" int64_t dm_split_colsum_partial_floats(int64_t rows, int64_t cols) {
  if (rows <= 0 || cols <= 0 || cols % 8) return 0;
  int gx, gy;
  split_rows_grid(rows, cols, gx, gy, true);
  return (int64_t)gy * cols;
}

extern "C" int dm_split_bf16_colsum(const float *src, int64_t ld, int64_t rows, int64_t cols, void *dst, int32_t stack, int32_t pattern,
                                    float *partial, int32_t *n_partial, void *stream) {
  DM_REQUIRE(src && dst && partial && n_partial && rows > 0 && cols > 0 && ld >= cols && pattern >= 0 && pattern < 8, DM_ERR_BAD_SHAPE,
             "dm_split_bf16_colsum: bad arguments (rows=%lld cols=%lld ld=%lld)", (long long)rows, (long long)cols, (long long)ld);
  DM_REQUIRE(split_rows_ok(src, ld, rows, cols, dst, stack), DM_ERR_UNSUPPORTED,
             "dm_split_bf16_colsum: needs cols %% 8 == 0, ld %% 4 == 0 and 16-byte aligned tensors (cols=%lld ld=%lld)", (long long)cols, (long long)ld);
  int gx, gy;
  split_rows_grid(rows, cols, gx, gy, true);
  hipLaunchKernelGGL(split_bf16_rows_kernel<true>, dim3(gx, (unsigned)gy), dim3(32, 8), 0, reinterpret_cast<hipStream_t>(stream), src, (long long)ld,
                     (int)rows, (int)cols, (bf16_t *)dst, stack ? 1 : 0, pattern, partial, 3);
  DM_LAUNCH_CHECK("dm_split_bf16_colsum");
  *n_partial = gy;
  return DM_OK;
}

extern "C" int dm_split_bf16_planes(const float *src, int64_t ld, int64_t rows, int64_t cols, void *dst, float *partial, int32_t *n_partial,
                                    void *stream) {
  DM_REQUIRE(src && dst && rows > 0 && cols > 0 && ld >= cols && ((partial == nullptr) == (n_partial == nullptr)), DM_ERR_BAD_SHAPE,
             "dm_split_bf16_planes: bad arguments (rows=%lld cols=%lld ld=%lld)", (long long)rows, (long long)cols, (long long)ld);
  DM_REQUIRE(split_rows_ok(src, ld, rows, cols, dst, 1), DM_ERR_UNSUPPORTED,
             "dm_split_bf16_planes: needs cols %% 8 == 0, ld %% 4 == 0 and 16-byte aligned tensors (cols=%lld ld=%lld)", (long long)cols, (long long)ld);
  int gx, gy;
  split_rows_grid(rows, cols, gx, gy, partial != nullptr);
  hipStream_t s = reinterpret_cast<hipStream_t>(stream);
  if (partial)
    hipLaunchKernelGGL(split_bf16_rows_kernel<true>, dim3(gx, (unsigned)gy), dim3(32, 8), 0, s, src, (long long)ld, (int)rows, (int)cols, (bf16_t *)dst, 1, 0b10, partial, 2);
  else
    hipLaunchKernelGGL(split_bf16_rows_kernel<false>, dim3(gx, (unsigned)gy), dim3(32, 8), 0, s, src, (long long)ld, (int)rows, (int)cols, (bf16_t *)dst, 1, 0b10,
                       (float *)nullptr, 2);
  DM_LAUNCH_CHECK("dm_split_bf16_planes");
  if (n_partial) *n_partial = gy;
  return DM_OK;
}

extern "C" int dm_split_bf16(const float *src, int64_t ld, int64_t rows, int64_t cols, void *dst, int32_t stack, int32_t pattern,
                             void *stream) {
  DM_REQUIRE(src && dst && rows > 0 && cols > 0 && cols % 4 == 0 && ld >= cols && ld % 4 == 0, DM_ERR_BAD_SHAPE,
             "dm_split_bf16: rows=%lld cols=%lld ld=%lld (cols and ld must be multiples of 4)", (long long)rows, (long long)cols, (long long)ld);
  DM_REQUIRE(pattern >= 0 && pattern < 8, DM_ERR_BAD_SHAPE, "dm_split_bf16: pattern %d", pattern);
  hipStream_t s = reinterpret_cast<hipStream_t>(stream);
  if (split_rows_ok(src, ld, rows, cols, dst, stack)) {
    int gx, gy;
    split_rows_grid(rows, cols, gx, gy);
    hipLaunchKernelGGL(split_bf16_rows_kernel<false>, dim3(gx, (unsigned)gy), dim3(32, 8), 0, s, src, (long long)ld, (int)rows, (int)cols,
                       (bf16_t *)dst, stack ? 1 : 0, pattern, (float *)nullptr, 3);
  } else {
    hipLaunchKernelGGL(split_bf16_kernel, dim3(grid_for(rows * (cols / 4))), dim3(256), 0, s, src, (long long)ld, (long long)rows,
                       (long long)cols, (bf16_t *)dst, stack ? 1 : 0, pattern);
  }
  DM_LAUNCH_CHECK("dm_split_bf16");
  return DM_OK;
}

extern "C" int dm_patchify(const float *x, void *cols, int32_t dtype, int32_t B, int32_t C, int32_t side, int32_t p, void *stream) {
  DM_REQUIRE(B > 0 && C > 0 && p > 0 && side % p == 0, DM_ERR_BAD_SHAPE,
             "dm_patchify: B=%d C=%d side=%d patch=%d (patch must divide side)", B, C, side, p);
  hipStream_t s = reinterpret_cast<hipStream_t>(stream);
  if (p % 4 != 0) {
    const int rc = dm_patchify_any(x, cols, dtype, B, C, side, p, s);
    DM_REQUIRE(rc == DM_OK, rc, "dm_patchify: bad dtype %d", dtype);
    DM_LAUNCH_CHECK("dm_patchify(any)");
    return DM_OK;
  }
  const long long total = (long long)B * (side / p) * (side / p) * ((long long)C * p * p / 4);
  if (dtype == DM_F32) hipLaunchKernelGGL(patchify_kernel<float>, dim3(grid_for(total)), dim3(256), 0, s, x, (float *)cols, B, C, side, p);
  else if (dtype == DM_BF16) hipLaunchKernelGGL(patchify_kernel<bf16_t>, dim3(grid_for(total)), dim3(256), 0, s, x, (bf16_t *)cols, B, C, side, p);
  else DM_REQUIRE(false, DM_ERR_BAD_DTYPE, "dm_patchify: bad dtype %d", dtype);
  DM_LAUNCH_CHECK("dm_patchify");
  return DM_OK;
}

extern "C" int dm_cross_entropy(const float *logits, const int64_t *target_index, const float *target_prob, float upstream,
                                float *loss, float *dlogits, int32_t B, int32_t K, void *stream) {
  DM_REQUIRE(logits && loss && B > 0 && K > 0, DM_ERR_BAD_SHAPE, "dm_cross_entropy: bad arguments");
  DM_REQUIRE((target_index != nullptr) != (target_prob != nullptr), DM_ERR_BAD_SHAPE,
             "dm_cross_entropy: exactly one of target_index / target_prob must be given");
  hipLaunchKernelGGL(cross_entropy_kernel, dim3(1), dim3(256), 0, reinterpret_cast<hipStream_t>(stream), logits,
                     reinterpret_cast<const long long *>(target_index), target_prob, upstream, loss, dlogits, B, K);
  DM_LAUNCH_CHECK("dm_cross_entropy");
  return DM_OK;
}

extern "C" int dm_contrastive_loss(const float *a, const float *b, const float *flag, float margin, float upstream,
                                   float *loss, float *da, float *db, int32_t B, int32_t D, void *stream) {
  DM_REQUIRE(a && b && flag && loss && B > 0 && D > 0, DM_ERR_BAD_SHAPE, "dm_contrastive_loss: bad arguments");
  DM_REQUIRE((da == nullptr) == (db == nullptr), DM_ERR_BAD_SHAPE, "dm_contrastive_loss: da and db must both be set or both NULL");
  hipLaunchKernelGGL(contrastive_loss_kernel, dim3(1), dim3(256), 0, reinterpret_cast<hipStream_t>(stream), a, b, flag, margin, upstream, loss, da, db, B, D);
  DM_LAUNCH_CHECK("dm_contrastive_loss");
  return DM_OK;
}

extern "C" int dm_adam_step(float *param, const float *grad, float *m, float *v, void *param_lp, int64_t n, int32_t step,
                            double lr, double beta1, double beta2, double eps, double grad_scale, void *stream) {
  DM_REQUIRE(param && grad && m && v && n > 0 && step >= 1, DM_ERR_BAD_SHAPE, "dm_adam_step: bad arguments");
  const double bc1 = 1.0 - pow(beta1, (double)step);
  const double bc2 = 1.0 - pow(beta2, (double)step);
  const float step_size = (float)(lr / bc1);
  const float bc2_sqrt = (float)sqrt(bc2);
  hipLaunchKernelGGL(adam_kernel, dim3(adam_grid(n)), dim3(256), 0, reinterpret_cast<hipStream_t>(stream), param, grad, m, v,
                     (bf16_t *)param_lp, (long long)n, (float)beta1, (float)beta2, (float)(1.0 - beta1), (float)(1.0 - beta2),
                     (float)eps, step_size, bc2_sqrt, (float)grad_scale, (const float *)nullptr);
  DM_LAUNCH_CHECK("dm_adam_step");
  return DM_OK;
}

extern "C" int dm_adam_hyper(int32_t step, double lr, double beta1, double beta2, float *hyper_host) {
  DM_REQUIRE(step >= 1 && hyper_host, DM_ERR_BAD_SHAPE, "dm_adam_hyper: step is 1-based and hyper_host must be set");
  hyper_host[0] = (float)(lr / (1.0 - pow(beta1, (double)step)));
  hyper_host[1] = (float)sqrt(1.0 - pow(beta2, (double)step));
  return DM_OK;
}

extern "C" int dm_adam_step_dev(float *param, const float *grad, float *m, float *v, void *param_lp, int64_t n, const float *hyper_dev,
                                double beta1, double beta2, double eps, double grad_scale, void *stream) {
  DM_REQUIRE(param && grad && m && v && hyper_dev && n > 0, DM_ERR_BAD_SHAPE, "dm_adam_step_dev: bad arguments");
  DM_REQUIRE(dm_aligned16(param) && dm_aligned16(grad) && dm_aligned16(m) && dm_aligned16(v) && dm_aligned16(param_lp), DM_ERR_BAD_ALIGN,
             "dm_adam_step_dev: buffers must be 16-byte aligned");
  hipLaunchKernelGGL(adam_kernel, dim3(adam_grid(n)), dim3(256), 0, reinterpret_cast<hipStream_t>(stream), param, grad, m, v,
                     (bf16_t *)param_lp, (long long)n, (float)beta1, (float)beta2, (float)(1.0 - beta1), (float)(1.0 - beta2),
                     (float)eps, 0.f, 1.f, (float)grad_scale, hyper_dev);
  DM_LAUNCH_CHECK("dm_adam_step_dev");
  return DM_OK;
}

extern "C" int dm_adam_step_dev_pair(float *param, const float *grad, float *m, float *v, void *param_hi, void *param_lo, int64_t n,
                                     const float *hyper_dev, double beta1, double beta2, double eps, double grad_scale, void *stream) {
  DM_REQUIRE(param && grad && m && v && hyper_dev && param_hi && param_lo && n > 0, DM_ERR_BAD_SHAPE, "dm_adam_step_dev_pair: bad arguments");
  DM_REQUIRE(dm_aligned16(param) && dm_aligned16(grad) && dm_aligned16(m) && dm_aligned16(v) && dm_aligned16(param_hi) && dm_aligned16(param_lo),
             DM_ERR_BAD_ALIGN, "dm_adam_step_dev_pair: buffers must be 16-byte aligned");
  hipLaunchKernelGGL(adam_kernel, dim3(adam_grid(n)), dim3(256), 0, reinterpret_cast<hipStream_t>(stream), param, grad, m, v,
                     (bf16_t *)param_hi, (long long)n, (float)beta1, (float)beta2, (float)(1.0 - beta1), (float)(1.0 - beta2),
                     (float)eps, 0.f, 1.f, (float)grad_scale, hyper_dev, (bf16_t *)param_lo);
  DM_LAUNCH_CHECK("dm_adam_step_dev_pair");
  return DM_OK;
}

extern "C" int dm_relpos_bias_gather(const float *table, const int32_t *index, float *bias, float *bias_t, int32_t N, int32_t H,
                                     int32_t n_bins, void *stream) {
  DM_REQUIRE(table && index && bias && N > 0 && H > 0 && n_bins > 0, DM_ERR_BAD_SHAPE, "dm_relpos_bias_gather: bad arguments");
  hipLaunchKernelGGL(relpos_gather_kernel, dim3(grid_for((long long)N * N)), dim3(256), 0, reinterpret_cast<hipStream_t>(stream), table, index, bias, bias_t, N, H, n_bins);
  DM_LAUNCH_CHECK("dm_relpos_bias_gather");
  return DM_OK;
}
extern "C" int dm_relpos_bias_reduce(float *dbias_slab, const int32_t *positions, const int32_t *offsets, float *dtable,
                                     int32_t chunks, int32_t H, int32_t N, int32_t n_bins, int32_t accumulate, void *stream) {
  DM_REQUIRE(dbias_slab && positions && offsets && dtable && chunks > 0 && H > 0 && N > 0 && n_bins > 0, DM_ERR_BAD_SHAPE,
             "dm_relpos_bias_reduce: bad arguments");
  DM_REQUIRE(n_bins <= 65535 * 32, DM_ERR_BAD_SHAPE, "dm_relpos_bias_reduce: too many bins (%d)", n_bins);
  const long long plane = (long long)H * N * N;
  if (chunks > 1 && plane % 4 == 0 && dm_aligned16(dbias_slab)) {
    hipLaunchKernelGGL(chunk_sum_kernel, dim3(grid_for(plane / 4, 256, 2048)), dim3(256), 0, reinterpret_cast<hipStream_t>(stream), dbias_slab,
                       plane / 4, chunks);
    chunks = 1;
  }
  hipLaunchKernelGGL(relpos_reduce_kernel, dim3(n_bins, (H + 3) / 4), dim3(256), 0, reinterpret_cast<hipStream_t>(stream), dbias_slab,
                     positions, offsets, dtable, chunks, H, N, n_bins, accumulate);
  DM_LAUNCH_CHECK("dm_relpos_bias_reduce");
  return DM_OK;
}
```

deepmerge_amd/nets/ShfitScaleFormer.py:

```python
from __future__ import annotations

import math
from typing import List, Optional, Sequence

import torch
import torch.nn as nn

from .. import ops

__all__ = ["PatchEmbed", "Mlp", "FeatureEmbed", "CrossScaleAttention", "CrossScaleBlock", "ShfitScaleFormer",
           "ShfitScaleFormer_v2", "ShfitScaleFormer_v3", "ShfitScaleFormer_v6"]


def drop_path(x, drop_prob: float = 0., training: bool = False):
    if drop_prob == 0. or not training:
        return x
    keep = 1 - drop_prob
    mask = keep + torch.rand((x.shape[0],) + (1,) * (x.ndim - 1), dtype=x.dtype, device=x.device)
    mask.floor_()
    return x.div(keep) * mask


class DropPath(nn.Module):
    def __init__(self, drop_prob=None):
        super().__init__()
        self.drop_prob = drop_prob

    def forward(self, x):
        return drop_path(x, self.drop_prob, self.training)


def stochastic_block_forward(block, x, table_args):
    x = x.float()
    dt = ops.act_dtype(block.numerics)
    y = ops.LayerNormFn.apply(x, block.norm1.weight, block.norm1.bias, block.norm1.eps, dt)
    x = x + block.drop_path(block.attn(y))
    y = ops.LayerNormFn.apply(x, block.norm2.weight, block.norm2.bias, block.norm2.eps, dt)
    return x + block.drop_path(block.mlp(y).float())


def _mode(numerics: Optional[str], module=None) -> str:
    return ops.bind_numerics(module, numerics or ops.get_numerics())


def relative_position_index(cube: Sequence[int]) -> torch.Tensor:
    S, H, W = (int(c) for c in cube)
    t = torch.arange(S * H * W)
    z, y, x = t // (H * W), (t // W) % H, t % W
    d = lambda a, n: a[:, None] - a[None, :] + (n - 1)
    return (d(z, S) * ((2 * H - 1) * (2 * W - 1)) + d(y, H) * (2 * W - 1) + d(x, W)).to(torch.int64)


class PatchEmbed(nn.Module):

    def __init__(self, img_size=224, patch_size=16, in_c=3, out_c=768, norm_layer=None, numerics=None):
        super().__init__()
        self.img_size = (img_size, img_size)
        self.patch_size = (patch_size, patch_size)
        self.grid_size = (img_size // patch_size, img_size // patch_size)
        self.num_patches = self.grid_size[0] * self.grid_size[1]
        self.proj = nn.Conv2d(in_c, out_c, kernel_size=patch_size, stride=patch_size)
        self.norm = norm_layer(out_c) if norm_layer else nn.Identity()
        self.numerics = _mode(numerics, self)

    def operand_rows(self, x):
        B, C, H, W = x.shape
        assert H == self.img_size[0] and W == self.img_size[1], \
            f"Input image size ({H}*{W}) doesn't match model ({self.img_size[0]}*{self.img_size[1]})."
        if isinstance(x, ops.PatchCols):
            if x.patch != self.patch_size[0] or x.cols.dtype != ops.act_dtype(self.numerics):
                raise ValueError("PatchCols were built for another patch size / numerics mode")
            return x.cols
        return ops.patchify(x.float(), self.patch_size[0], ops.act_dtype(self.numerics))

    def forward(self, x):
        B = x.shape[0]
        cols = self.operand_rows(x)
        y = ops.LinearFn.apply(cols, self.proj.weight, self.proj.bias, None, torch.float32)
        return self.norm(y.view(B, self.num_patches, -1))


class Mlp(nn.Module):

    def __init__(self, in_features, hidden_features=None, out_features=None, act_layer=nn.GELU, drop=0., numerics=None):
        super().__init__()
        out_features = out_features or in_features
        hidden_features = hidden_features or in_features
        if act_layer is not nn.GELU:
            raise ValueError("the fused MLP kernel implements nn.GELU (erf) only")
        if drop != 0.:
            raise ValueError("dropout > 0 is not part of the accelerated path (reference uses drop=0)")
        self.fc1 = nn.Linear(in_features, hidden_features)
        self.act = act_layer()
        self.fc2 = nn.Linear(hidden_features, out_features)
        self.drop = nn.Dropout(drop)
        self.numerics = _mode(numerics, self)

    def _run(self, x2d, residual2d, out_dtype):
        return ops.MlpFn.apply(x2d, self.fc1.weight, self.fc1.bias, self.fc2.weight, self.fc2.bias, residual2d, out_dtype)

    def forward(self, x):
        shp = x.shape
        xin = _CastFn.apply(x.reshape(-1, shp[-1]), ops.act_dtype(self.numerics))
        y = self._run(xin, None, torch.float32)
        return y.view(*shp[:-1], y.shape[-1])


class _CastFn(torch.autograd.Function):

    @staticmethod
    def forward(ctx, x, dtype):
        return ops._as_operand(x, dtype)

    @staticmethod
    def backward(ctx, g):
        return g.float(), None


class FeatureEmbed(nn.Module):

    def __init__(self, feature_size=19, embed_dim=768, act_layer=nn.GELU, norm_layer=None, numerics=None):
        super().__init__()
        self.proj0 = nn.Conv1d(feature_size, embed_dim, kernel_size=1, stride=1)
        self.proj1 = nn.Conv1d(embed_dim, embed_dim, kernel_size=1, stride=1)
        self.proj2 = nn.Conv1d(embed_dim, embed_dim, kernel_size=1, stride=1)
        self.norm = norm_layer(embed_dim) if norm_layer else nn.Identity()
        self.act = act_layer()
        self.numerics = _mode(numerics, self)

    def forward(self, x):
        B, T, F = x.shape
        h = ops.MlpFn.apply(x.reshape(B * T, F).float(), self.proj0.weight, self.proj0.bias,
                            self.proj1.weight, self.proj1.bias, None, torch.float32)
        y = ops.LinearFn.apply(h, self.proj2.weight, self.proj2.bias, None, torch.float32)
        return self.norm(y.view(B, T, -1))


class CrossScaleAttention(nn.Module):

    def __init__(self, dim, num_heads, cube_size, qkv_bias=False, qk_scale=None, attn_drop_ratio=0., proj_drop_ratio=0,
                 numerics=None):
        super().__init__()
        if attn_drop_ratio != 0. or proj_drop_ratio != 0:
            raise ValueError("dropout > 0 is not part of the accelerated path (reference uses 0)")
        self.num_heads = num_heads
        head_dim = dim // num_heads
        self.scale = qk_scale or head_dim ** -0.5
        self.qkv = nn.Linear(dim, dim * 3, bias=qkv_bias)
        self.attn_drop = nn.Dropout(attn_drop_ratio)
        self.proj = nn.Linear(dim, dim)
        self.proj_drop = nn.Dropout(proj_drop_ratio)
        self.cube_size = cube_size
        self.relative_position_bias_table = nn.Parameter(torch.zeros(self._table_rows(cube_size), num_heads))
        self.register_buffer("relative_position_index", self._make_index(cube_size))
        nn.init.trunc_normal_(self.relative_position_bias_table, std=.02)
        self.numerics = _mode(numerics, self)
        self._idx32 = None

    @staticmethod
    def _table_rows(cube):
        return (2 * cube[0] - 1) * (2 * cube[1] - 1) * (2 * cube[2] - 1)

    @staticmethod
    def _make_index(cube):
        return relative_position_index(cube)

    def _index32(self) -> torch.Tensor:
        src = self.relative_position_index
        tag = (src.data_ptr(), src._version, src.device)
        if self._idx32 is None or self._idx32[0] != tag:
            idx = src.to(torch.int32).contiguous()
            cube = tuple(int(c) for c in self.cube_size)
            if len(cube) == 3 and tuple(src.shape) == (cube[0] * cube[1] * cube[2],) * 2 and \
                    bool((src == relative_position_index(cube).to(src.device)).all()):
                idx._dm_cube = cube
            self._idx32 = (tag, idx)
        return self._idx32[1]

    def _run(self, y, residual2d, out_dtype):
        B, N, Cc = y.shape
        H = self.num_heads
        qkv = ops.LinearFn.apply(y.reshape(B * N, Cc), self.qkv.weight, self.qkv.bias, None, y.dtype)
        o = ops.AttentionFn.apply(qkv, self.relative_position_bias_table, self._index32(), B, N, H, Cc // H, float(self.scale))
        return ops.LinearFn.apply(o.reshape(B * N, Cc), self.proj.weight, self.proj.bias, residual2d, out_dtype)

    def forward(self, x):
        B_, N, Cc = x.shape
        y = _CastFn.apply(x, ops.act_dtype(self.numerics))
        return self._run(y, None, torch.float32).view(B_, N, Cc)


class CrossScaleBlock(nn.Module):
    _dm_fused_block = True

    _attention_cls = CrossScaleAttention

    def __init__(self, dim, num_heads, cube_size, mlp_ratio=4., qkv_bias=True, qk_scale=None, drop_ratio=0.,
                 attn_drop_ratio=0., drop_path_ratio=0., act_layer=nn.GELU, norm_layer=nn.LayerNorm, numerics=None):
        super().__init__()
        self.numerics = _mode(numerics, self)
        self.norm1 = norm_layer(dim)
        self.attn = self._attention_cls(dim=dim, num_heads=num_heads, cube_size=cube_size, qkv_bias=qkv_bias,
                                        qk_scale=qk_scale, attn_drop_ratio=attn_drop_ratio, proj_drop_ratio=drop_ratio,
                                        numerics=self.numerics)
        self.drop_path = DropPath(drop_path_ratio) if drop_path_ratio > 0. else nn.Identity()
        if drop_path_ratio > 0.:
            self._dm_fused_block = False
        self.norm2 = norm_layer(dim)
        self.mlp = Mlp(in_features=dim, hidden_features=int(dim * mlp_ratio), act_layer=act_layer, drop=drop_ratio,
                       numerics=self.numerics)

    def forward(self, x):
        a, m = self.attn, self.mlp
        if self.training and isinstance(self.drop_path, DropPath):
            return stochastic_block_forward(self, x, None)
        if a.qkv.bias is None:
            raise ValueError("the fused block kernel path expects qkv_bias=True (the reference default, :165)")
        return ops.BlockFn.apply(x.float(), self.norm1.weight, self.norm1.bias, a.relative_position_bias_table, a._index32(),
                                 a.qkv.weight, a.qkv.bias, a.proj.weight, a.proj.bias, self.norm2.weight, self.norm2.bias,
                                 m.fc1.weight, m.fc1.bias, m.fc2.weight, m.fc2.bias,
                                 a.num_heads, self.norm1.eps, float(a.scale), ops.act_dtype(self.numerics))


class ShfitScaleFormer_v3(nn.Module):
    _dm_first_write_blocks = True

    def __init__(self, num_classes=11, is_designed_feature_embedding=True, FeatureEmbed=FeatureEmbed, PatchEmbed=PatchEmbed,
                 cube_size=[8, 8], input_image_scales=[32, 64, 128], embed_dim=768, depth=[6, 4, 2], num_heads=12,
                 mlp_ratio=4.0, drop_path_ratio=0., drop_ratio=0., attn_drop_ratio=0., norm_layer=nn.LayerNorm,
                 act_layer=nn.GELU, cuda=True, in_c=3, numerics=None):
        super().__init__()
        self.numerics = _mode(numerics, self)
        self.name = "S2Former_v3-3CH" + ("-3DP-SEF" if is_designed_feature_embedding else "")
        self.name = "{0}-{1}{2}{3}".format(self.name, depth[0], depth[1], depth[2])
        self.num_classes = num_classes
        self.is_designed_feature_embedding = is_designed_feature_embedding
        self.patch_embed_layer, self.feature_embed_layer = PatchEmbed, FeatureEmbed
        self.input_image_scales = input_image_scales
        self.input_scales_num = S = len(input_image_scales)
        self.cube_size = cube_size
        self.cube_size.insert(0, S)
        grid = self.cube_size[1]
        self.num_features = int(S * embed_dim)
        self.depth = depth
        self.in_c = in_c
        kw = {"numerics": self.numerics} if PatchEmbed is globals()["PatchEmbed"] else {}
        self.patch_embed_blocks = nn.ModuleList(
            [PatchEmbed(img_size=s, patch_size=int(s / grid), in_c=in_c, out_c=embed_dim, **kw) for s in input_image_scales])
        self.feature_embed = FeatureEmbed(feature_size=19, embed_dim=embed_dim) if is_designed_feature_embedding else None

        def stage(cube, n):
            return nn.Sequential(*[getattr(self, "_block_cls", CrossScaleBlock)(dim=embed_dim, num_heads=num_heads, cube_size=cube, mlp_ratio=mlp_ratio,
                                                   drop_ratio=drop_ratio, attn_drop_ratio=attn_drop_ratio, drop_path_ratio=0,
                                                   norm_layer=norm_layer, act_layer=act_layer, numerics=self.numerics)
                                   for _ in range(n)])
        self.blocks0 = stage(self.cube_size, depth[0])
        self.blocks1 = stage([S, grid // 2, grid // 2], depth[1])
        self.blocks2 = stage([S, grid // 4, grid // 4], depth[2])
        self.norm = norm_layer(embed_dim)
        self.pos_drop = nn.Dropout(p=drop_ratio)
        self.avgpool = nn.AdaptiveAvgPool1d(1)
        self.final_features = nn.Linear(int(S * embed_dim), 100)
        self.final_features_with_design = nn.Linear(int((S + 1) * embed_dim), 100)
        self.head = nn.Linear(100, num_classes) if num_classes > 0 else nn.Identity()
        self.avgpool2D = nn.AvgPool2d(kernel_size=2, stride=2)
        self.apply(self._init_weights)

    def patch_embed(self, x: List[torch.Tensor]):
        layers = list(self.patch_embed_blocks)
        if not all(type(l) is PatchEmbed and isinstance(l.norm, nn.Identity) and l.num_patches == layers[0].num_patches for l in layers):
            return torch.cat([layer(x[i]) for i, layer in enumerate(layers)], 1)
        cols = [l.operand_rows(x[i]) for i, l in enumerate(layers)]
        return ops.PatchEmbedCatFn.apply(len(layers), layers[0].num_patches, *cols, *[l.proj.weight for l in layers], *[l.proj.bias for l in layers])

    def designed_feature_embed(self, x):
        return self.feature_embed(x)

    def _ln(self, x, out_dtype=torch.float32, grad_lp=None):
        return ops.LayerNormFn.apply(x, self.norm.weight, self.norm.bias, self.norm.eps, out_dtype, grad_lp)

    def _pool_ln(self, x, side):
        return ops.pool_norm(x, self.norm.weight, self.norm.bias, self.norm.eps, self.input_scales_num, side, self.numerics)

    _dp_cut = None

    def backbone(self, x):
        S, side = self.input_scales_num, self.cube_size[1]
        if self._dp_cut is None:
            x = self.blocks0(x)
        else:
            for blk in self.blocks0:
                x = self._dp_cut(blk(x), blk)
        x = self._pool_ln(x, side)
        x = self.blocks1(x)
        x = self._pool_ln(x, side // 2)
        return self.blocks2(x)

    def _pooled_tokens(self, x):
        B = x[0].shape[0]
        x = self.pos_drop(self.patch_embed(x))
        if self._dp_cut is not None:
            x = self._dp_cut(x, self.patch_embed_blocks)
        x = self._ln(self.backbone(x), grad_lp=ops.act_dtype(self.numerics) if len(self.blocks2) else None)
        g = x.shape[1] // self.input_scales_num
        return ops.GroupMeanFn.apply(x, g).view(B, -1)

    def forward_once_design_feature(self, x, designed_features):
        x = self._pooled_tokens(x)
        d = torch.squeeze(self.designed_feature_embed(designed_features), dim=1)
        x = torch.cat((x, self._ln(d)), 1)
        return ops.LinearFn.apply(x, self.final_features_with_design.weight, self.final_features_with_design.bias, None, torch.float32)

    def forward_once(self, x):
        x = self._pooled_tokens(x)
        return ops.LinearFn.apply(x, self.final_features.weight, self.final_features.bias, None, torch.float32)

    def extract_features_with_design_features(self, x_path, x_designed_features):
        return self.forward_once_design_feature(x_path, x_designed_features)

    def extract_features(self, x_path):
        return self.forward_once(x_path)

    def forward(self, x1_patches, x1_designed_features, x2_patches=None, x2_designed_features=None):
        S = self.input_scales_num
        if self.training:
            B = x1_patches[0].shape[0]
            both = [ops.cat_batch(x1_patches[i], x2_patches[i]) for i in range(S)]
            if self.is_designed_feature_embedding:
                f = self.forward_once_design_feature(both, torch.cat((x1_designed_features, x2_designed_features), 0))
            else:
                f = self.forward_once(both)
            return ops.split_halves(f)
        if self.is_designed_feature_embedding:
            return self.forward_once_design_feature(x1_patches, x1_designed_features)
        return self.forward_once(x1_patches)

    def forward_pair_batched(self, both_patches, both_designed):
        B = both_patches[0].shape[0] // 2
        if self.is_designed_feature_embedding:
            f = self.forward_once_design_feature(both_patches, both_designed)
        else:
            f = self.forward_once(both_patches)
        return ops.split_halves(f)

    def _init_weights(self, m):
        if isinstance(m, nn.Linear):
            nn.init.trunc_normal_(m.weight, std=.02)
            if m.bias is not None:
                nn.init.constant_(m.bias, 0)
        elif isinstance(m, nn.LayerNorm):
            nn.init.constant_(m.bias, 0)
            nn.init.constant_(m.weight, 1.0)


def relative_position_index_v5(cube: Sequence[int]) -> torch.Tensor:
    base = relative_position_index(cube)
    n = base.shape[0]
    bins = CrossScaleAttention._table_rows(cube)
    col = bins + torch.arange(n, dtype=torch.int64)[:, None]
    idx = torch.cat([base, col], 1)
    row = bins + n + torch.arange(n + 1, dtype=torch.int64)[None, :]
    idx = torch.cat([idx, row], 0)
    idx[-1, -1] = idx[0, 0]
    return idx


class CrossScaleAttention_v5(CrossScaleAttention):

    @staticmethod
    def _table_rows(cube):
        return CrossScaleAttention._table_rows(cube) + 2 * cube[0] * cube[1] * cube[2]

    @staticmethod
    def _make_index(cube):
        return relative_position_index_v5(cube)


class CrossScaleBlock_v5(CrossScaleBlock):
    _attention_cls = CrossScaleAttention_v5


class AuxBolck(nn.Module):
    _v5 = False

    def __init__(self, in_c=768, out_c=100, cube_size=[3, 8, 8], norm_layer=nn.LayerNorm, numerics=None):
        super().__init__()
        self.cube_size = cube_size
        self.aux = nn.Sequential(
            nn.Conv2d(in_c, in_c, kernel_size=2, padding=0, bias=False),
            nn.BatchNorm2d(in_c),
            nn.ReLU(inplace=True),
            nn.Dropout2d(p=0.3),
            nn.Conv2d(in_c, int(in_c / cube_size[0]), kernel_size=1))
        self.avgpool = nn.AdaptiveAvgPool1d(1)
        width = in_c * 2 if self._v5 else in_c
        self.norm = norm_layer(width)
        self.out_features = nn.Linear(width, out_c)
        self.numerics = _mode(numerics, self)

    def _scale_head(self, t):
        B, n, Cc = t.shape
        side = int(math.isqrt(n))
        o = side - 1
        t4 = t.reshape(B, side, side, Cc)
        cols = torch.stack([t4[:, ky:ky + o, kx:kx + o, :] for ky in (0, 1) for kx in (0, 1)], dim=-1).reshape(B * o * o, Cc * 4)
        dt = ops.act_dtype(self.numerics)
        y = ops.LinearFn.apply(_CastFn.apply(cols, dt), self.aux[0].weight, None, None, torch.float32)
        bn, drop = self.aux[1], self.aux[3]
        if bn.momentum is None or not bn.track_running_stats or not bn.affine:
            raise ValueError("the HIP BatchNorm path implements the reference's default BatchNorm2d (affine, momentum 0.1, running stats)")
        training = self.training
        mask = None
        if training and drop.p > 0:
            mask = torch.empty((B, Cc), dtype=torch.float32, device=y.device).bernoulli_(1.0 - drop.p).div_(1.0 - drop.p)
        y = ops.BatchNormReluFn.apply(y, bn.weight, bn.bias, bn.running_mean, bn.running_var, mask, o * o, bn.eps, bn.momentum, training, True)
        if training:
            bn.num_batches_tracked += 1
        y = ops.LinearFn.apply(_CastFn.apply(y, dt), self.aux[4].weight, self.aux[4].bias, None, torch.float32)
        return ops.GroupMeanFn.apply(y.view(B, o * o, -1), o * o).view(B, -1)

    def forward(self, x):
        S, side = self.cube_size[0], self.cube_size[1]
        n = side * side
        y = torch.cat([self._scale_head(x[:, n * i:n * (i + 1), :]) for i in range(S)], 1)
        if self._v5:
# ... 300 lines not shown
```

deepmerge_amd/ops.py:

```python
from __future__ import annotations

import os

import ctypes as C
from typing import Optional

import torch

from . import _lib
from ._lib import DM_BF16, DM_EPI_DGELU, DM_EPI_GELU, DM_EPI_GELU_GRAD, DM_EPI_MUL, DM_EPI_NONE, DM_F32, DM_NN, DM_NT, DM_TN, DmGemmArgs, check

_NUMERICS = "bf16"


NUMERICS_MODES = ("bf16", "fp32", "bf16x3")
_FP32_PRODUCTS = "mfma_f32"
_SPLIT_MIN_WORK = 1 << 24
_PAIR_LN_MAX_COLS = 1024


def set_numerics(mode: str) -> None:
    global _NUMERICS
    _NUMERICS = check_numerics(mode)

# ... 185 lines not shown
        A, B, lda, ldb, K = A.t, B.t, a_cols, b_cols, 3 * K
    _need_cuda(A, B, C_out, bias, residual, aux, colsum_out)
    if A.dtype != B.dtype:
        raise ValueError(f"A/B dtype mismatch: {A.dtype} vs {B.dtype}")
    if lda is None:
        lda = A.stride(-2) if A.dim() >= 2 else K
    if ldb is None:
        ldb = B.stride(-2) if B.dim() >= 2 else K
    if (_FP32_PRODUCTS == "bf16x3" and A.dtype == torch.float32 and M * N * K >= _SPLIT_MIN_WORK
            and M % 8 == 0 and N % 8 == 0 and K % 8 == 0 and lda % 4 == 0 and ldb % 4 == 0):
        a_rows, a_cols = (M, K) if layout != DM_TN else (K, M)
        b_rows, b_cols = (N, K) if layout == DM_NT else (K, N)
        a_stack, b_stack = int(layout == DM_TN), int(layout != DM_NT)
        A3 = workspace(6 * a_rows * a_cols, A.device, ws_slot + ".split_a").view(torch.bfloat16)
        B3 = workspace(6 * b_rows * b_cols, A.device, ws_slot + ".split_b").view(torch.bfloat16)
        fused_ok = colsum_out is not None and a_cols % 8 == 0 and A.data_ptr() % 16 == 0 and (a_rows * a_cols) % 8 == 0
        n_part = _lib.lib().dm_split_colsum_partial_floats(a_rows, a_cols) if fused_ok else 0
        if n_part > 0:
            part = workspace(4 * n_part, A.device, ws_slot + ".partial").view(torch.float32)
            rows_out = C.c_int32(0)
            check(_lib.lib().dm_split_bf16_colsum(A.data_ptr(), lda, a_rows, a_cols, A3.data_ptr(), a_stack, 0b100, part.data_ptr(),
                                                  C.byref(rows_out), _stream()), "dm_split_bf16_colsum")
            item = (_lib.DmReduceItem * 1)()
            item[0].partial, item[0].out0, item[0].out1 = part.data_ptr(), colsum_out.data_ptr(), colsum_out.data_ptr()
            item[0].nrows, item[0].width, item[0].split, item[0].accumulate = rows_out.value, a_cols, a_cols, int(bool(colsum_accumulate))
            check(_lib.lib().dm_partial_reduce_batch(item, 1, _stream()), "dm_partial_reduce_batch")
        else:
            check(_lib.lib().dm_split_bf16(A.data_ptr(), lda, a_rows, a_cols, A3.data_ptr(), a_stack, 0b100, _stream()), "dm_split_bf16")
            if colsum_out is not None:
                colsum(torch.as_strided(A, (a_rows, a_cols), (lda, 1)), colsum_out, accumulate=colsum_accumulate, ws_slot=ws_slot + ".partial")
        check(_lib.lib().dm_split_bf16(B.data_ptr(), ldb, b_rows, b_cols, B3.data_ptr(), b_stack, 0b010, _stream()), "dm_split_bf16")
        return gemm(layout, A3, B3, C_out, M, N, 3 * K, lda=(a_cols if a_stack else 3 * a_cols), ldb=(b_cols if b_stack else 3 * b_cols),
                    ldc=ldc, bias=bias, residual=residual, ldr=ldr, epilogue=epilogue, aux=aux, ldaux=ldaux, accumulate=accumulate,
                    split_k=split_k, rows_per_group=rows_per_group, group_stride=group_stride, ws_slot=ws_slot)
    a = _gemm_args(layout, A, B, C_out, M, N, K, lda, ldb, ldc, bias, residual, ldr, epilogue, aux, ldaux, accumulate, split_k,
                   rows_per_group, group_stride, colsum_out, colsum_accumulate, ws_slot, c_pair, fold)
    check(_lib.lib().dm_gemm(C.byref(a), _stream()), "dm_gemm")
    return c_pair if c_pair is not None else C_out


def _gemm_args(layout, A, B, C_out, M, N, K, lda, ldb, ldc, bias, residual, ldr, epilogue, aux, ldaux, accumulate, split_k,
               rows_per_group, group_stride, colsum_out, colsum_accumulate, ws_slot, c_pair=None, fold=None, min_slabs: int = 0) -> DmGemmArgs:
    a = DmGemmArgs()
    a.layout, a.ab_dtype, a.c_dtype = layout, _dt(A), _dt(C_out)
    if c_pair is not None:
        if _dt(A) != DM_BF16:
            raise ValueError("a plane-pair result goes with bf16 / folded operands")
        a.c_dtype, a.c_plane = _lib.DM_BF16_PAIR, M * N
    a.aux_dtype = _dt(aux) if aux is not None else DM_F32
    a.M, a.N, a.K = M, N, K
    a.epilogue, a.accumulate, a.split_k = epilogue, int(accumulate), split_k
    a.A, a.lda = A.data_ptr(), lda
    a.B, a.ldb = B.data_ptr(), ldb
    a.C, a.ldc = C_out.data_ptr(), (ldc if ldc is not None else N)
    a.bias = _ptr(bias)
    if bias is not None and (bias.dtype != torch.float32 or bias.numel() < N):
        raise ValueError("bias must be fp32 with >= N elements")
    a.residual, a.ldr = _ptr(residual), (ldr if ldr is not None else N)
    if residual is not None and residual.dtype != torch.float32:
        raise ValueError("residual must be fp32")
    a.aux, a.ldaux = _ptr(aux), (ldaux if ldaux is not None else N)
    a.rows_per_group, a.group_stride = rows_per_group, group_stride
    if colsum_out is not None:
        if colsum_out.dtype != torch.float32 or colsum_out.numel() < M or not colsum_out.is_contiguous():
            raise ValueError("colsum_out must be a contiguous fp32 tensor with >= M elements")
        a.colsum_a, a.colsum_accumulate = colsum_out.data_ptr(), int(colsum_accumulate)
    if fold is not None:
        a.k_fold = fold[0]
        a.a_fold[0], a.a_fold[1], a.a_fold[2] = 0, 0, fold[1]
        a.b_fold[0], a.b_fold[1], a.b_fold[2] = 0, fold[2], 0
    ws_bytes = _lib.lib().dm_gemm_workspace_bytes(layout, M, N, K) if (split_k != 1 or colsum_out is not None) else 0
    if split_k > 1:
        ws_bytes = max(ws_bytes, _lib.lib().dm_gemm_workspace_bytes(layout, M, N, K) + split_k * M * N * 4)
    if min_slabs > 0:
        ws_bytes = max(ws_bytes, _lib.lib().dm_gemm_workspace_bytes(layout, M, N, K) + min_slabs * M * N * 4)
    if ws_bytes > 0:
        ws = workspace(ws_bytes, A.device, ws_slot)
        a.workspace, a.workspace_bytes = ws.data_ptr(), ws.numel()
    return a


def gemm_grouped(calls) -> None:
    if not calls:
        return
    plain = len(calls) > 1
    for args, kw in calls:
        A, B = args[1], args[2]
        pair = isinstance(A, Planes) and isinstance(B, Planes)
        plain = plain and not isinstance(args[3], Planes) and (pair or (not isinstance(A, Planes) and not isinstance(B, Planes) and A.dtype == torch.bfloat16))
    if not plain:
        for args, kw in calls:
            gemm(*args, **kw)
        return
    arr = (DmGemmArgs * len(calls))()
    for i, (args, kw) in enumerate(calls):
        layout, A, B, C_out, M, N, K = args
        lda, ldb, fold = kw.get("lda"), kw.get("ldb"), None
        if isinstance(A, Planes):
            a_rows, a_cols = (M, K) if layout != DM_TN else (K, M)
            b_rows, b_cols = (N, K) if layout == DM_NT else (K, N)
            if (A.rows, A.cols) != (a_rows, a_cols) or (B.rows, B.cols) != (b_rows, b_cols):
                raise ValueError(f"plane pair shapes {(A.rows, A.cols)} / {(B.rows, B.cols)} do not match the product {(a_rows, a_cols)} / {(b_rows, b_cols)}")
            fold = (K, A.t.stride(0), B.t.stride(0))
            A, B, lda, ldb, K = A.t, B.t, a_cols, b_cols, 3 * K
        _need_cuda(A, B, C_out, kw.get("colsum_out"))
        if A.dtype != B.dtype:
            raise ValueError(f"A/B dtype mismatch: {A.dtype} vs {B.dtype}")
        lda = lda if lda is not None else (A.stride(-2) if A.dim() >= 2 else K)
        ldb = ldb if ldb is not None else (B.stride(-2) if B.dim() >= 2 else K)
        arr[i] = _gemm_args(layout, A, B, C_out, M, N, K, lda, ldb, kw.get("ldc"), kw.get("bias"), kw.get("residual"), kw.get("ldr"),
                            kw.get("epilogue", DM_EPI_NONE), kw.get("aux"), kw.get("ldaux"), kw.get("accumulate", False), kw.get("split_k", 0),
                            kw.get("rows_per_group", 0), kw.get("group_stride", 0), kw.get("colsum_out"), kw.get("colsum_accumulate", False),
                            f"{kw.get('ws_slot', 'gemm')}.g{i}", None, fold, min_slabs=16 if layout == DM_TN else 0)
    check(_lib.lib().dm_gemm_grouped(arr, len(calls), _stream()), "dm_gemm_grouped")


def cast(src: torch.Tensor, dtype: torch.dtype) -> torch.Tensor:
    if src.dtype == dtype:
        return src
    _need_cuda(src)
    if src.dtype != torch.float32:
        raise ValueError("dm_cast source must be fp32")
    src = src.contiguous()
    dst = torch.empty(src.shape, dtype=dtype, device=src.device)
    check(_lib.lib().dm_cast(src.data_ptr(), dst.data_ptr(), _dt(dst), src.numel(), _stream()), "dm_cast")
    return dst


def colsum(X: torch.Tensor, out: torch.Tensor, accumulate: bool = False, ws_slot: str = "partial") -> torch.Tensor:
    _need_cuda(X, out)
    M, N = X.shape
    part = workspace(_lib.lib().dm_colsum_partial_floats(N) * 4, X.device, ws_slot)
    check(_lib.lib().dm_colsum(X.data_ptr(), _dt(X), X.stride(0), out.data_ptr(), M, N, int(accumulate), part.data_ptr(), _stream()), "dm_colsum")
    return out


def layernorm_fwd(x: torch.Tensor, gamma, beta, eps: float, out_dtype: torch.dtype, pair: bool = False):
    _need_cuda(x, gamma, beta)
    rows, cols = x.numel() // x.shape[-1], x.shape[-1]
    mean = torch.empty(rows, dtype=torch.float32, device=x.device)
    rstd = torch.empty(rows, dtype=torch.float32, device=x.device)
    if pair:
        yp = torch.empty((2, rows, cols), dtype=torch.bfloat16, device=x.device)
        check(_lib.lib().dm_layernorm_fwd(x.data_ptr(), gamma.data_ptr(), beta.data_ptr(), yp.data_ptr(), _lib.DM_BF16_PAIR, mean.data_ptr(),
                                          rstd.data_ptr(), rows, cols, eps, _stream()), "dm_layernorm_fwd")
        return Planes(yp), mean, rstd
    y = torch.empty(x.shape, dtype=out_dtype, device=x.device)
    check(_lib.lib().dm_layernorm_fwd(x.data_ptr(), gamma.data_ptr(), beta.data_ptr(), y.data_ptr(), _dt(y), mean.data_ptr(),
                                      rstd.data_ptr(), rows, cols, eps, _stream()), "dm_layernorm_fwd")
    return y, mean, rstd


_pending_reduce = []
_pending_out = set()
_flush_queued = False
_flush_task = -1


def _in_backward() -> bool:
    return torch._C._current_graph_task_id() != -1


def flush_reductions() -> None:
    global _flush_queued
    _flush_queued = False
    if not _pending_reduce:
        return
    items = (_lib.DmReduceItem * len(_pending_reduce))()
    for i, (f, _keep) in enumerate(_pending_reduce):
        items[i].partial, items[i].out0, items[i].out1, items[i].nrows, items[i].width, items[i].split, items[i].accumulate = f
    n = len(_pending_reduce)
    keep = list(_pending_reduce)
    _pending_reduce.clear()
    _pending_out.clear()
    check(_lib.lib().dm_partial_reduce_batch(items, n, _stream()), "dm_partial_reduce_batch")
    del keep


def _queue_reduce(part, out0, out1, nrows, width, split, accumulate) -> None:
    global _flush_queued, _flush_task
    task = torch._C._current_graph_task_id()
    if task != _flush_task:
        _pending_reduce.clear()
        _pending_out.clear()
        _flush_queued = False
        _flush_task = task
    keys = (out0.data_ptr(), out1.data_ptr())
    if keys[0] in _pending_out or keys[1] in _pending_out:
        flush_reductions()
    _pending_reduce.append(((part.data_ptr(), keys[0], keys[1], int(nrows), int(width), int(split), int(bool(accumulate))), (part, out0, out1)))
    _pending_out.update(keys)
    if not _flush_queued:
        torch.autograd.Variable._execution_engine.queue_callback(flush_reductions)
        _flush_queued = True


def _reduce_partials(part, dgamma, dbeta, n_part, cols, accumulate, deferred) -> None:
    if deferred:
        _queue_reduce(part, dgamma, dbeta, n_part, 2 * cols, cols, accumulate)
        return
    item = (_lib.DmReduceItem * 1)()
    item[0].partial, item[0].out0, item[0].out1 = part.data_ptr(), dgamma.data_ptr(), dbeta.data_ptr()
    item[0].nrows, item[0].width, item[0].split, item[0].accumulate = n_part, 2 * cols, cols, int(bool(accumulate))
    check(_lib.lib().dm_partial_reduce_batch(item, 1, _stream()), "dm_partial_reduce_batch")


def layernorm_bwd(dy, x, gamma, mean, rstd, dres=None, dgamma=None, dbeta=None, accumulate=False, want_lp=False, defer=False, want_pair=False,
                  regroup=None):
    _need_cuda(dy, x)
    if not (dy.is_contiguous() and x.is_contiguous()) or dy.numel() != x.numel():
        raise ValueError("layernorm_bwd: dy and x must be contiguous and of the same size (an expanded gradient has no rows to read)")
    rows, cols = x.numel() // x.shape[-1], x.shape[-1]
    dx = torch.empty(x.shape, dtype=torch.float32, device=x.device)
    dx_lp = torch.empty(x.shape, dtype=torch.bfloat16, device=x.device) if want_lp else None
    if dgamma is None:
        dgamma = torch.empty(cols, dtype=torch.float32, device=x.device)
        dbeta = torch.empty(cols, dtype=torch.float32, device=x.device)
        accumulate = False
        defer = False
    if want_pair:
        pair = torch.empty((2, rows, cols), dtype=torch.bfloat16, device=x.device)
        deferred = defer and _DEFER_REDUCTIONS and _in_backward()
        part = (torch.empty(_lib.lib().dm_layernorm_bwd_partial_floats(cols), dtype=torch.float32, device=x.device) if deferred
                else workspace(_lib.lib().dm_layernorm_bwd_partial_floats(cols) * 4, x.device, "partial").view(torch.float32))
        n_part = C.c_int32(0)
        check(_lib.lib().dm_layernorm_bwd_partials_pair(dy.data_ptr(), _dt(dy), x.data_ptr(), gamma.data_ptr(), mean.data_ptr(), rstd.data_ptr(),
                                                        _ptr(dres), dx.data_ptr(), pair.data_ptr(), part.data_ptr(), rows, cols, C.byref(n_part),
                                                        _stream()), "dm_layernorm_bwd_partials_pair")
        if deferred:
            _queue_reduce(part, dgamma, dbeta, n_part.value, 2 * cols, cols, accumulate)
        else:
            item = (_lib.DmReduceItem * 1)()
            item[0].partial, item[0].out0, item[0].out1 = part.data_ptr(), dgamma.data_ptr(), dbeta.data_ptr()
            item[0].nrows, item[0].width, item[0].split, item[0].accumulate = n_part.value, 2 * cols, cols, int(bool(accumulate))
            check(_lib.lib().dm_partial_reduce_batch(item, 1, _stream()), "dm_partial_reduce_batch")
        return dx, Planes(pair), dgamma, dbeta
    if regroup is not None:
        S, T = regroup
        if not want_lp or rows % (S * T) or cols > _PAIR_LN_MAX_COLS:
            raise ValueError("layernorm_bwd: regroup needs want_lp, rows in whole (S, T) groups and a register-resident width")
        dx_lp = torch.empty((S, rows // (S * T), T, cols), dtype=torch.bfloat16, device=x.device)
        deferred = defer and _DEFER_REDUCTIONS and _in_backward()
        part = (torch.empty(_lib.lib().dm_layernorm_bwd_partial_floats(cols), dtype=torch.float32, device=x.device) if deferred
                else workspace(_lib.lib().dm_layernorm_bwd_partial_floats(cols) * 4, x.device, "partial").view(torch.float32))
        n_part = C.c_int32(0)
        check(_lib.lib().dm_layernorm_bwd_partials_regroup(dy.data_ptr(), _dt(dy), x.data_ptr(), gamma.data_ptr(), mean.data_ptr(), rstd.data_ptr(),
                                                           _ptr(dres), dx.data_ptr(), dx_lp.data_ptr(), part.data_ptr(), rows, cols, S, T,
                                                           C.byref(n_part), _stream()), "dm_layernorm_bwd_partials_regroup")
        _reduce_partials(part, dgamma, dbeta, n_part.value, cols, accumulate, deferred)
        return dx, dx_lp, dgamma, dbeta
    if defer and _DEFER_REDUCTIONS and _in_backward():
        part = torch.empty(_lib.lib().dm_layernorm_bwd_partial_floats(cols), dtype=torch.float32, device=x.device)
        n_part = C.c_int32(0)
        check(_lib.lib().dm_layernorm_bwd_partials(dy.data_ptr(), _dt(dy), x.data_ptr(), gamma.data_ptr(), mean.data_ptr(), rstd.data_ptr(),
                                                   _ptr(dres), dx.data_ptr(), _ptr(dx_lp), part.data_ptr(), rows, cols, C.byref(n_part),
                                                   _stream()), "dm_layernorm_bwd_partials")
        _queue_reduce(part, dgamma, dbeta, n_part.value, 2 * cols, cols, accumulate)
        return (dx, dx_lp, dgamma, dbeta) if want_lp else (dx, dgamma, dbeta)
    part = workspace(_lib.lib().dm_layernorm_bwd_partial_floats(cols) * 4, x.device, "partial")
    check(_lib.lib().dm_layernorm_bwd(dy.data_ptr(), _dt(dy), x.data_ptr(), gamma.data_ptr(), mean.data_ptr(), rstd.data_ptr(),
                                      _ptr(dres), dx.data_ptr(), _ptr(dx_lp), dgamma.data_ptr(), dbeta.data_ptr(), int(accumulate),
                                      part.data_ptr(), rows, cols, _stream()), "dm_layernorm_bwd")
    return (dx, dx_lp, dgamma, dbeta) if want_lp else (dx, dgamma, dbeta)


_DEFER_REDUCTIONS = os.environ.get("DM_DEFER_REDUCTIONS", "1") != "0"
_FUSED_GLUE = os.environ.get("DM_FUSED_GLUE", "1") != "0"


def relpos_bias_gather(table: torch.Tensor, index32: torch.Tensor, N: int, transposed: bool = False):
    _need_cuda(table, index32)
    n_bins, H = table.shape
    bias = torch.empty((H, N, N), dtype=torch.float32, device=table.device)
    bias_t = torch.empty_like(bias) if transposed else None
    check(_lib.lib().dm_relpos_bias_gather(table.data_ptr(), index32.data_ptr(), bias.data_ptr(), _ptr(bias_t), N, H, n_bins, _stream()),
          "dm_relpos_bias_gather")
    return (bias, bias_t) if transposed else bias


def attention_fwd(qkv: torch.Tensor, bias: Optional[torch.Tensor], B: int, N: int, H: int, D: int, scale: float):
    _need_cuda(qkv, bias)
    out = torch.empty((B, N, H * D), dtype=qkv.dtype, device=qkv.device)
    lse = torch.empty((B, H, N), dtype=torch.float32, device=qkv.device)
    check(_lib.lib().dm_attention_fwd(qkv.data_ptr(), _ptr(bias), out.data_ptr(), lse.data_ptr(), B, N, H, D, scale, _dt(qkv), _stream()),
          "dm_attention_fwd")
    return out, lse


def _split_attention(table, index32, qkv, B, N, H, D):
    if (qkv if isinstance(qkv, torch.dtype) else qkv.dtype) != torch.float32 or _FP32_PRODUCTS != "bf16x3" or not _SPLIT_ATTENTION:
        return False, None
    cube = None if table is None else getattr(index32, "_dm_cube", None)
    if table is not None and cube is None:
        return False, None
    return attention_split_ok(B, N, H, D, cube), cube


_SPLIT_ATTENTION = os.environ.get("DM_ATTN_X3", "1") != "0"


def _inkernel_cube(table, index32, B, N, H, D, dtype):
    cube = None if table is None else getattr(index32, "_dm_cube", None)
    if cube is None or _INKERNEL_TABLE is False or not relpos_inkernel(B, N, H, D, cube, dtype):
        return None
    return cube


_INKERNEL_TABLE = os.environ.get("DM_ATTN_TABLE_IN_KERNEL", "1") != "0"


def relpos_inkernel(B: int, N: int, H: int, D: int, cube, dtype: torch.dtype) -> bool:
    if cube is None or len(cube) != 3:
        return False
    return bool(_lib.lib().dm_attention_relpos_inkernel(B, N, H, D, int(cube[0]), int(cube[1]), int(cube[2]),
                                                        DM_BF16 if dtype == torch.bfloat16 else DM_F32))


def attention_fwd_relpos(qkv: torch.Tensor, table: torch.Tensor, cube, B: int, N: int, H: int, D: int, scale: float):
    _need_cuda(qkv, table)
    if table.dtype != torch.float32 or not table.is_contiguous() or tuple(table.shape) != ((2 * cube[0] - 1) * (2 * cube[1] - 1) * (2 * cube[2] - 1), H):
        raise ValueError(f"attention_fwd_relpos: table must be contiguous fp32 [(2s-1)(2h-1)(2w-1), H], got {tuple(table.shape)} {table.dtype}")
    out = torch.empty((B, N, H * D), dtype=qkv.dtype, device=qkv.device)
    lse = torch.empty((B, H, N), dtype=torch.float32, device=qkv.device)
    check(_lib.lib().dm_attention_fwd_relpos(qkv.data_ptr(), table.data_ptr(), int(cube[0]), int(cube[1]), int(cube[2]), out.data_ptr(),
                                             lse.data_ptr(), B, N, H, D, scale, _dt(qkv), _stream()), "dm_attention_fwd_relpos")
    return out, lse


def attention_split_ok(B: int, N: int, H: int, D: int, cube=None) -> bool:
    c = (0, 0, 0) if cube is None else tuple(int(v) for v in cube)
    return bool(_lib.lib().dm_attention_split_ok(B, N, H, D, int(cube is not None), c[0], c[1], c[2]))


def attention_fwd_split(qkv: torch.Tensor, table: Optional[torch.Tensor], cube, B: int, N: int, H: int, D: int, scale: float, out_pair: bool = False):
    if table is not None and (table.dtype != torch.float32 or not table.is_contiguous()):
        raise ValueError("attention_fwd_split: table must be contiguous fp32")
    if isinstance(qkv, Planes):
        _need_cuda(qkv.t, table)
        hi, lo, src, dev = qkv.t[0], qkv.t[1], None, qkv.t.device
    else:
        _need_cuda(qkv, table)
        if qkv.dtype != torch.float32 or not qkv.is_contiguous():
            raise ValueError("attention_fwd_split: qkv must be a contiguous fp32 tensor")
        hi = torch.empty(qkv.shape, dtype=torch.bfloat16, device=qkv.device)
        lo = torch.empty(qkv.shape, dtype=torch.bfloat16, device=qkv.device)
        src, dev = qkv.data_ptr(), qkv.device
    out = torch.empty((B, N, H * D), dtype=torch.float32, device=dev)
    lse = torch.empty((B, H, N), dtype=torch.float32, device=dev)
    c = (0, 0, 0) if cube is None else tuple(int(v) for v in cube)
    if out_pair:
        op = torch.empty((2, B * N, H * D), dtype=torch.bfloat16, device=dev)
        check(_lib.lib().dm_attention_split_fwd_pair(src, hi.data_ptr(), lo.data_ptr(), _ptr(table), c[0], c[1], c[2], out.data_ptr(), op.data_ptr(),
                                                     lse.data_ptr(), B, N, H, D, scale, _stream()), "dm_attention_split_fwd_pair")
        return out, lse, hi, lo, Planes(op)
    check(_lib.lib().dm_attention_split_fwd(src, hi.data_ptr(), lo.data_ptr(), _ptr(table), c[0], c[1], c[2], out.data_ptr(),
                                            lse.data_ptr(), B, N, H, D, scale, _stream()), "dm_attention_split_fwd")
    return out, lse, hi, lo


def attention_bwd_split(hi, lo, table, cube, out, dout, lse, B, N, H, D, scale, index32=None, n_bins=0, pair=False):
    _need_cuda(hi, lo, table, out, dout, lse, index32)
    if out.dtype != torch.float32 or dout.dtype != torch.float32 or not (out.is_contiguous() and dout.is_contiguous()):
        raise ValueError("attention_bwd_split: out / dout must be contiguous fp32")
    dqkv = (torch.empty((2, B * N, 3 * H * D), dtype=torch.bfloat16, device=hi.device) if pair
            else torch.empty(hi.shape, dtype=torch.float32, device=hi.device))
    delta = torch.empty((B, H, N), dtype=torch.float32, device=hi.device)
    dhi = torch.empty(dout.shape, dtype=torch.bfloat16, device=hi.device)
    dlo = torch.empty(dout.shape, dtype=torch.bfloat16, device=hi.device)
    slab, info = None, None
    if index32 is not None and table is not None:
        chunks = _lib.lib().dm_attention_split_bwd_chunks(B, N, H)
        slab = torch.empty((chunks, H, N, N), dtype=torch.float32, device=hi.device)
        info = (chunks, N, relpos_index_csr(index32, n_bins))
    c = (0, 0, 0) if cube is None else tuple(int(v) for v in cube)
    fn = _lib.lib().dm_attention_split_bwd_pair if pair else _lib.lib().dm_attention_split_bwd
    check(fn(hi.data_ptr(), lo.data_ptr(), _ptr(table), c[0], c[1], c[2], out.data_ptr(), dout.data_ptr(),
             dhi.data_ptr(), dlo.data_ptr(), lse.data_ptr(), dqkv.data_ptr(), delta.data_ptr(), _ptr(slab),
             B, N, H, D, scale, _stream()), "dm_attention_split_bwd")
    return (Planes(dqkv) if pair else dqkv), slab, info


def relpos_index_csr(index32: torch.Tensor, n_bins: int):
    key = (index32._version, n_bins)
    hit = getattr(index32, "_dm_csr", None)
    if hit is None or hit[0] != key:
        flat = index32.reshape(-1).to(torch.int64)
        ok = (flat >= 0) & (flat < n_bins)
        where = torch.nonzero(ok).reshape(-1)
        order = torch.argsort(flat[where], stable=True)
        positions = where[order].to(torch.int32).contiguous()
        counts = torch.bincount(flat[where], minlength=n_bins)
        offsets = torch.zeros(n_bins + 1, dtype=torch.int64, device=index32.device)
        offsets[1:] = torch.cumsum(counts, 0)
        hit = index32._dm_csr = (key, positions, offsets.to(torch.int32).contiguous())
    return hit[1], hit[2]


def attention_bwd(qkv, bias, out, dout, lse, B, N, H, D, scale, index32=None, n_bins=0, bias_t=None, table=None, cube=None):
    _need_cuda(qkv, bias, out, dout, lse, index32, bias_t, table)
    dqkv = torch.empty_like(qkv)
    delta = torch.empty((B, H, N), dtype=torch.float32, device=qkv.device)
    slab, info = None, None
    if index32 is not None:
        if D != 64 or N > 256:
            raise ValueError(f"the relative-position bias gradient needs head dim 64 and N <= 256 (got D={D}, N={N})")
        chunks = _lib.lib().dm_attention_bwd_batch_chunks(B, N, H, _dt(qkv))
        slab = torch.empty((chunks, H, N, N), dtype=torch.float32, device=qkv.device)
        info = (chunks, N, relpos_index_csr(index32, n_bins))
    if table is not None and cube is not None:
        check(_lib.lib().dm_attention_bwd_relpos(qkv.data_ptr(), table.data_ptr(), int(cube[0]), int(cube[1]), int(cube[2]), _ptr(bias),
                                                 _ptr(bias_t), out.data_ptr(), dout.data_ptr(), lse.data_ptr(), dqkv.data_ptr(),
                                                 delta.data_ptr(), _ptr(slab), B, N, H, D, scale, _dt(qkv), _stream()),
              "dm_attention_bwd_relpos")
        return dqkv, slab, info
    check(_lib.lib().dm_attention_bwd(qkv.data_ptr(), _ptr(bias), _ptr(bias_t), out.data_ptr(), dout.data_ptr(), lse.data_ptr(), dqkv.data_ptr(),
                                      delta.data_ptr(), _ptr(slab), B, N, H, D, scale, _dt(qkv), _stream()),
          "dm_attention_bwd")
    return dqkv, slab, info


def relpos_bias_scatter(slab, dtable, B, H, info, n_bins, accumulate=False):
    _need_cuda(slab, dtable)
    chunks, N, (positions, offsets) = info
    check(_lib.lib().dm_relpos_bias_reduce(slab.data_ptr(), positions.data_ptr(), offsets.data_ptr(), dtable.data_ptr(), chunks, H, N,
                                           n_bins, int(accumulate), _stream()), "dm_relpos_bias_reduce")
    return dtable


def patchify(x: torch.Tensor, patch: int, dtype: torch.dtype) -> torch.Tensor:
    _need_cuda(x)
    B, Cc, H, W = x.shape
    if H != W:
        raise ValueError("square images only")
    x = x.contiguous()
    g = H // patch
    cols = torch.empty((B * g * g, Cc * patch * patch), dtype=dtype, device=x.device)
    check(_lib.lib().dm_patchify(x.data_ptr(), cols.data_ptr(), _dt(cols), B, Cc, H, patch, _stream()), "dm_patchify")
    return cols


RESIZE_RULES = {"opencv": 0, "exact_area": 1}


def _resize_rule(resize: str) -> int:
    if resize not in RESIZE_RULES:
        raise ValueError(f"resize must be one of {tuple(RESIZE_RULES)}, got {resize!r}")
    return RESIZE_RULES[resize]


def patch_pyramid(tile: torch.Tensor, xy: torch.Tensor, windows: torch.Tensor, target: int, max_window: Optional[int] = None,
                  resize: str = "opencv") -> torch.Tensor:
    _need_cuda(tile, xy, windows)
    if tile.dtype != torch.uint8:
        raise ValueError("tile must be uint8")
    bands, H, W = tile.shape
    P = xy.shape[0]
    if max_window is None:
        max_window = int(windows.max().item())
    out = torch.empty((P, bands, target, target), dtype=torch.float32, device=tile.device)
    check(_lib.lib().dm_patch_pyramid(tile.contiguous().data_ptr(), bands, H, W, xy.to(torch.int32).contiguous().data_ptr(),
                                      windows.to(torch.int32).contiguous().data_ptr(), max_window, P, target, _resize_rule(resize),
                                      out.data_ptr(), _stream()), "dm_patch_pyramid")
    return out


class PatchCols:

    def __init__(self, cols: torch.Tensor, batch: int, side: int, patch: int, bands: int):
        self.cols, self.batch, self.side, self.patch, self.bands = cols, batch, side, patch, bands

    @property
    def shape(self):
        return (self.batch, self.bands, self.side, self.side)

    def __getitem__(self, sl):
        g2 = (self.side // self.patch) ** 2
        if not isinstance(sl, slice) or sl.step not in (None, 1):
            raise TypeError("PatchCols supports contiguous batch slices only")
        a, b, _ = sl.indices(self.batch)
        return PatchCols(self.cols[a * g2:b * g2], b - a, self.side, self.patch, self.bands)

    def to(self, *_a, **_k):
        return self

    @staticmethod
    def cat(a: "PatchCols", b: "PatchCols") -> "PatchCols":
        if (a.side, a.patch, a.bands, a.cols.dtype) != (b.side, b.patch, b.bands, b.cols.dtype):
            raise ValueError("PatchCols.cat: the two sides were built for different scales / dtypes")
        ca, cb = a.cols, b.cols
        if (ca.is_contiguous() and cb.is_contiguous() and ca.untyped_storage().data_ptr() == cb.untyped_storage().data_ptr()
                and cb.data_ptr() == ca.data_ptr() + ca.numel() * ca.element_size()):
            both = ca.as_strided((ca.shape[0] + cb.shape[0], ca.shape[1]), (ca.shape[1], 1), ca.storage_offset())
        else:
            both = torch.cat((ca, cb), 0)
        return PatchCols(both, a.batch + b.batch, a.side, a.patch, a.bands)


def cat_batch(a, b):
    if isinstance(a, PatchCols) or isinstance(b, PatchCols):
        return PatchCols.cat(a, b)
    return torch.cat((a, b), 0)


def pair_batch_gather(tiles: torch.Tensor, tile_id: Optional[torch.Tensor], xy: torch.Tensor, inner: torch.Tensor, obj: torch.Tensor,
                      scale_index: int, target: int, max_window: int, out: torch.Tensor, grid: int = 0, resize: str = "opencv",
                      region_features: Optional[torch.Tensor] = None, designed: Optional[torch.Tensor] = None,
                      error_flag: Optional[torch.Tensor] = None) -> None:
    _need_cuda(tiles, tile_id, xy, inner, obj, out, region_features, designed, error_flag)
    if tiles.dtype != torch.uint8 or tiles.dim() != 4 or not tiles.is_contiguous():
        raise ValueError("tiles must be a contiguous uint8 [T, bands, H, W] tensor")
    for name, t in (("tile_id", tile_id), ("xy", xy), ("inner", inner), ("obj", obj), ("error_flag", error_flag)):
        if t is not None and (t.dtype != torch.int32 or not t.is_contiguous()):
            raise ValueError(f"{name} must be a contiguous int32 tensor (a per-step cast would be a launch of its own)")
    T, bands, H, W = tiles.shape
    P = xy.shape[0]
    if not out.is_contiguous() or out.numel() != P * bands * target * target:
        raise ValueError(f"out must be contiguous with {P * bands * target * target} elements, got {tuple(out.shape)}")
    if (region_features is None) != (designed is None):
        raise ValueError("designed rows need the region features (and vice versa)")
    if designed is not None and (designed.dtype != torch.float32 or designed.numel() != P * 19 or not designed.is_contiguous()
                                 or region_features.dtype != torch.float32 or region_features.numel() != P * 15 or not region_features.is_contiguous()):
        raise ValueError("region_features must be contiguous float32 [P, 15] and designed contiguous float32 [P, 1, 19]")
    check(_lib.lib().dm_pair_batch_gather(tiles.data_ptr(), T, bands, H, W, _ptr(tile_id), xy.data_ptr(), inner.data_ptr(), obj.data_ptr(),
                                          scale_index, max_window, P, target, grid, _resize_rule(resize), out.data_ptr(), _dt(out),
                                          _ptr(region_features), _ptr(designed), _ptr(error_flag), _stream()), "dm_pair_batch_gather")


def pair_epoch_draw(pairs: torch.Tensor, pair_flag: torch.Tensor, poly_off: torch.Tensor, poly_pts: torch.Tensor, pt_tile: torch.Tensor,
                    pt_xy: torch.Tensor, pt_inner: torch.Tensor, pt_obj: torch.Tensor, pt_region: torch.Tensor, seed: int, epoch: int, batch: int,
                    tile_id: torch.Tensor, xy: torch.Tensor, inner: torch.Tensor, obj: torch.Tensor, region: torch.Tensor, flag: torch.Tensor,
                    point_id: Optional[torch.Tensor] = None) -> None:
    if pairs.dim() != 2 or pairs.shape[1] != 2:
        raise ValueError(f"pair_epoch_draw: pairs must be [N, 2], got {tuple(pairs.shape)}")
    N, n_pts = pairs.shape[0], pt_tile.numel()
    cols = {"pairs": (pairs, torch.int32, 2 * N), "pair_flag": (pair_flag, torch.int32, N), "poly_off": (poly_off, torch.int32, poly_off.numel()),
            "poly_pts": (poly_pts, torch.int32, poly_pts.numel()), "pt_tile": (pt_tile, torch.int32, n_pts), "pt_xy": (pt_xy, torch.int32, 2 * n_pts),
            "pt_inner": (pt_inner, torch.int32, n_pts), "pt_obj": (pt_obj, torch.int32, n_pts), "pt_region": (pt_region, torch.float32, 15 * n_pts),
            "tile_id": (tile_id, torch.int32, 2 * N), "xy": (xy, torch.int32, 4 * N), "inner": (inner, torch.int32, 2 * N),
            "obj": (obj, torch.int32, 2 * N), "region": (region, torch.float32, 30 * N), "flag": (flag, torch.float32, N),
            "point_id": (point_id, torch.int32, 2 * N)}
    _need_cuda(*(t for t, _, _ in cols.values()))
    for name, (t, dtype, numel) in cols.items():
        if t is not None and (t.dtype != dtype or not t.is_contiguous() or t.numel() != numel):
            raise ValueError(f"pair_epoch_draw: {name} must be a contiguous {dtype} tensor of {numel} elements, got {t.dtype} {tuple(t.shape)}")
    a = _lib.DmPairDraw()
    for name, (t, _, _) in cols.items():
        setattr(a, name, _ptr(t))
    a.seed = int(seed) & 0xFFFFFFFFFFFFFFFF
    a.n_pairs, a.n_poly, a.n_poly_pts, a.n_pts = N, poly_off.numel() - 1, poly_pts.numel(), n_pts
    a.epoch, a.batch = int(epoch), int(batch)
    with torch.cuda.device(pairs.device):
        check(_lib.lib().dm_pair_epoch_draw(C.byref(a), _stream()), "dm_pair_epoch_draw")


def patch_pyramid_cols(tile: torch.Tensor, xy: torch.Tensor, windows: torch.Tensor, target: int, grid: int = 8,
                       dtype: torch.dtype = torch.bfloat16, max_window: Optional[int] = None, resize: str = "opencv") -> PatchCols:
    _need_cuda(tile, xy, windows)
    if tile.dtype != torch.uint8:
        raise ValueError("tile must be uint8")
    bands, H, W = tile.shape
    P = xy.shape[0]
    if target % grid:
        raise ValueError(f"target {target} is not a multiple of the token grid {grid}")
    ps = target // grid
    if max_window is None:
        max_window = int(windows.max().item())
    cols = torch.empty((P * grid * grid, bands * ps * ps), dtype=dtype, device=tile.device)
    check(_lib.lib().dm_patch_pyramid_cols(tile.contiguous().data_ptr(), bands, H, W, xy.to(torch.int32).contiguous().data_ptr(),
                                           windows.to(torch.int32).contiguous().data_ptr(), max_window, P, target, grid, _resize_rule(resize),
                                           cols.data_ptr(), _dt(cols), _stream()), "dm_patch_pyramid_cols")
    return PatchCols(cols, P, target, ps, bands)


def adam_step(param, grad, m, v, step, lr=1e-4, beta1=0.9, beta2=0.999, eps=1e-8, grad_scale=1.0, param_lp=None):
    _need_cuda(param, grad, m, v)
    check(_lib.lib().dm_adam_step(param.data_ptr(), grad.data_ptr(), m.data_ptr(), v.data_ptr(), _ptr(param_lp), param.numel(), step,
                                  lr, beta1, beta2, eps, grad_scale, _stream()), "dm_adam_step")


def adam_hyper(step: int, lr: float, beta1: float = 0.9, beta2: float = 0.999) -> torch.Tensor:
    h = torch.empty(2, dtype=torch.float32).pin_memory() if torch.cuda.is_available() else torch.empty(2, dtype=torch.float32)
    check(_lib.lib().dm_adam_hyper(step, lr, beta1, beta2, h.data_ptr()), "dm_adam_hyper")
    return h


def adam_step_dev(param, grad, m, v, hyper_dev, beta1=0.9, beta2=0.999, eps=1e-8, grad_scale=1.0, param_lp=None, param_lo=None):
    _need_cuda(param, grad, m, v, hyper_dev)
    if param_lo is not None:
        check(_lib.lib().dm_adam_step_dev_pair(param.data_ptr(), grad.data_ptr(), m.data_ptr(), v.data_ptr(), param_lp.data_ptr(), param_lo.data_ptr(),
                                               param.numel(), hyper_dev.data_ptr(), beta1, beta2, eps, grad_scale, _stream()), "dm_adam_step_dev_pair")
        return
# ... 703 lines not shown

    @staticmethod
    def forward(ctx, x, n1w, n1b, table, index32, qkv_w, qkv_b, proj_w, proj_b, n2w, n2b, fc1_w, fc1_b, fc2_w, fc2_b,
                heads, eps, scale, dtype):
        _save_products(ctx)
        lp_rows = getattr(x, "_dm_lp_rows", None)
        ctx.lp_rows = lp_rows if (lp_rows is not None and x.dim() == 3 and lp_rows[0] * lp_rows[1] == x.shape[1]) else None
        x = x.contiguous()
        B, N, Cc = x.shape
        M, Hd, D = B * N, fc1_w.shape[0], Cc // heads
        dev = x.device
        wq, wp = lp_weight(qkv_w, dtype, (3 * Cc, Cc)), lp_weight(proj_w, dtype, (Cc, Cc))
        w1, w2 = lp_weight(fc1_w, dtype, (Hd, Cc)), lp_weight(fc2_w, dtype, (Cc, Hd))
        x2d = x.view(M, Cc)
        planes = (dtype == torch.float32 and _FP32_PRODUCTS == "bf16x3" and planes_ok(M, Cc) and planes_ok(M, Hd) and planes_ok(Hd, Cc)
                  and Cc <= _PAIR_LN_MAX_COLS and M * Cc * Cc >= _SPLIT_MIN_WORK)
        if planes:
            wq, wp, w1, w2 = (pair_weight(P, w) for P, w in ((qkv_w, wq), (proj_w, wp), (fc1_w, w1), (fc2_w, w2)))
        y1, mean1, rstd1 = layernorm_fwd(x2d, n1w, n1b, eps, dtype, pair=planes)
        split, scube = _split_attention(table, index32, dtype, B, N, heads, D)
        qkv = (Planes(torch.empty((2, M, 3 * Cc), dtype=torch.bfloat16, device=dev)) if (planes and split)
               else torch.empty((M, 3 * Cc), dtype=dtype, device=dev))
        gemm(DM_NT, y1, wq, qkv, M, 3 * Cc, Cc, lda=Cc, ldb=Cc, ldc=3 * Cc, bias=qkv_b)
        bias = bias_t = None
        cube = _inkernel_cube(table, index32, B, N, heads, D, dtype)
        split_imgs = None
        if split:
            o_op = None
            if planes:
                o, lse, hi, lo, o_op = attention_fwd_split(qkv, None if table is None else table.contiguous(), scube, B, N, heads, D, scale, out_pair=True)
            else:
                o, lse, hi, lo = attention_fwd_split(qkv, None if table is None else table.contiguous(), scube, B, N, heads, D, scale)
            split_imgs = (hi, lo, scube)
        elif cube is not None:
            o, lse = attention_fwd_relpos(qkv, table.contiguous(), cube, B, N, heads, D, scale)
        else:
            if table is not None:
                bias, bias_t = relpos_bias_gather(table.contiguous(), index32, N, transposed=True)
            o, lse = attention_fwd(qkv, bias, B, N, heads, D, scale)
        x1 = torch.empty((M, Cc), dtype=torch.float32, device=dev)
        if not (planes and split):
            o_op = split_planes(o.view(M, Cc)) if planes else o.view(M, Cc)
        gemm(DM_NT, o_op, wp, x1, M, Cc, Cc, lda=Cc, ldb=Cc, ldc=Cc, bias=proj_b, residual=x2d)
        y2, mean2, rstd2 = layernorm_fwd(x1, n2w, n2b, eps, dtype, pair=planes)
        h = Planes(torch.empty((2, M, Hd), dtype=torch.bfloat16, device=dev)) if planes else torch.empty((M, Hd), dtype=dtype, device=dev)
        if any(ctx.needs_input_grad):
            pre = torch.empty((M, Hd), dtype=dtype, device=dev)
            gemm(DM_NT, y2, w1, h, M, Hd, Cc, lda=Cc, ldb=Cc, ldc=Hd, bias=fc1_b, epilogue=DM_EPI_GELU_GRAD, aux=pre, ldaux=Hd)
        else:
            pre = None
            gemm(DM_NT, y2, w1, h, M, Hd, Cc, lda=Cc, ldb=Cc, ldc=Hd, bias=fc1_b, epilogue=DM_EPI_GELU)
        x2 = torch.empty((M, Cc), dtype=torch.float32, device=dev)
        gemm(DM_NT, h, w2, x2, M, Cc, Hd, lda=Hd, ldb=Hd, ldc=Cc, bias=fc2_b, residual=x1)
        if planes:
            y1, y2, h, wq, wp, w1, w2, o_op = y1.t, y2.t, h.t, wq.t, wp.t, w1.t, w2.t, o_op.t
            if isinstance(qkv, Planes):
                qkv = qkv.t
        ctx.planes = planes
        ctx.save_for_backward(x2d, mean1, rstd1, y1, qkv, o, lse, bias, bias_t, index32, x1, mean2, rstd2, y2, pre, h,
                              wq, wp, w1, w2, n1w, n2w, o_op if planes else None)
        ctx.dims = (B, N, Cc, heads, D, Hd, scale, None if table is None else table.shape[0])
        ctx.table_in_kernel = cube is not None
        ctx.split_imgs = split_imgs
        ctx.params = (n1w, n1b, table, qkv_w, qkv_b, proj_w, proj_b, n2w, n2b, fc1_w, fc1_b, fc2_w, fc2_b)
        return x2.view(B, N, Cc)

    @staticmethod
    @_replay_products
    def backward(ctx, dx2):
        (x, mean1, rstd1, y1, qkv, o, lse, bias, bias_t, index32, x1, mean2, rstd2, y2, pre, h,
         wq, wp, w1, w2, n1w, n2w, o_op) = ctx.saved_tensors
        planes = ctx.planes
        if planes:
            y1, y2, h, wq, wp, w1, w2, o_op = (Planes(t_) for t_ in (y1, y2, h, wq, wp, w1, w2, o_op))
        (P_n1w, P_n1b, P_table, P_qkv_w, P_qkv_b, P_proj_w, P_proj_b, P_n2w, P_n2b, P_fc1_w, P_fc1_b, P_fc2_w, P_fc2_b) = ctx.params
        B, N, Cc, heads, D, Hd, scale, n_bins = ctx.dims
        M = B * N
        dtype, dev = (torch.float32 if planes else y1.dtype), x.device
        lp = dtype != torch.float32
        lp_copy = getattr(dx2, "_dm_lp_copy", None)
        dy_pair = getattr(dx2, "_dm_planes", None)
        lp_copy = lp_copy[0] if (lp_copy is not None and lp_copy[1] == _grad_tag(dx2)) else None
        dy_pair = dy_pair[0] if (dy_pair is not None and dy_pair[1] == _grad_tag(dx2)) else None
        dx2 = dx2.contiguous().view(M, Cc)
        dy = _operand_grad(dx2, dtype, lp_copy)
        if planes and isinstance(dy_pair, Planes) and (dy_pair.rows, dy_pair.cols) == (M, Cc):
            dy = dy_pair
        dw2, k_w2 = _grad_out(P_fc2_w, (Cc, Hd), dev)
        db2, k_b2 = _grad_out(P_fc2_b, (Cc,), dev)
        side = _side_stream(dev) if 0 < M <= _WGRAD_SIDE_TOKENS else None

        pending = [] if (side is None and (lp or planes) and 0 < M <= _WGRAD_GROUP_TOKENS) else None
        late = [] if (pending is None and side is None and (lp or planes) and _WGRAD_PAIR) else None

        def wgrad(*a, pair=False, **kw):
            if pending is not None:
                pending.append((a, kw))
                return None
            if late is not None and pair:
                late.append((a, kw))
                return None
            if side is None:
                return gemm(*a, **kw)
            side.wait_stream(torch.cuda.current_stream())
            with torch.cuda.stream(side):
                return gemm(*a, ws_slot="gemm_side", **kw)

        def bias_grad(g2d, db, acc_b, direct):
            if planes and not isinstance(g2d, Planes):
                g2d = split_planes(g2d)
            return g2d, dict(colsum_out=db, colsum_accumulate=acc_b)
        dy, cs = bias_grad(dy, db2, _acc(P_fc2_b, k_b2), k_b2)
        wgrad(DM_TN, dy, h, dw2, Cc, Hd, M, lda=Cc, ldb=Hd, ldc=Hd, accumulate=_acc(P_fc2_w, k_w2), **cs)
        dpre = Planes(torch.empty((2, M, Hd), dtype=torch.bfloat16, device=dev)) if planes else torch.empty((M, Hd), dtype=dtype, device=dev)
        gemm(DM_NN, dy, w2, dpre, M, Hd, Cc, lda=Cc, ldb=Hd, ldc=None if planes else Hd, epilogue=DM_EPI_MUL, aux=pre, ldaux=Hd)
        dw1, k_w1 = _grad_out(P_fc1_w, (Hd, Cc), dev)
        db1, k_b1 = _grad_out(P_fc1_b, (Hd,), dev)
        dpre, cs = bias_grad(dpre, db1, _acc(P_fc1_b, k_b1), k_b1)
        wgrad(DM_TN, dpre, y2, dw1, Hd, Cc, M, lda=Hd, ldb=Cc, ldc=Cc, accumulate=_acc(P_fc1_w, k_w1), **cs)
        dy2 = torch.empty((M, Cc), dtype=dtype, device=dev)
        gemm(DM_NN, dpre, w1, dy2, M, Cc, Hd, lda=Hd, ldb=Cc, ldc=Cc)
        dg2, k_n2 = _grad_out(P_n2w, (Cc,), dev)
        dbt2, k_n2b = _grad_out(P_n2b, (Cc,), dev)
        if k_n2 != k_n2b:
            dg2, dbt2, k_n2, k_n2b = torch.empty(Cc, device=dev), torch.empty(Cc, device=dev), False, False
        a_n2 = _acc(P_n2w, k_n2)
        _acc(P_n2b, k_n2b)
        r = layernorm_bwd(dy2, x1, n2w, mean2, rstd2, dres=dx2, dgamma=dg2, dbeta=dbt2, accumulate=a_n2, want_lp=lp, defer=bool(k_n2 and k_n2b),
                          want_pair=planes)
        dx1, dx1_lp = (r[0], r[1]) if (lp or planes) else (r[0], r[0])
        dwp, k_wp = _grad_out(P_proj_w, (Cc, Cc), dev)
        dbp, k_bp = _grad_out(P_proj_b, (Cc,), dev)
        dx1_op, cs = bias_grad(dx1_lp, dbp, _acc(P_proj_b, k_bp), k_bp)
        wgrad(DM_TN, dx1_op, o_op if planes else o.view(M, Cc), dwp, Cc, Cc, M, lda=Cc, ldb=Cc, ldc=Cc, accumulate=_acc(P_proj_w, k_wp), pair=True, **cs)
        do = torch.empty((M, Cc), dtype=dtype, device=dev)
        gemm(DM_NN, dx1_op, wp, do, M, Cc, Cc, lda=Cc, ldb=Cc, ldc=Cc)
        tab, cube = None, None
        if ctx.split_imgs is not None:
            hi, lo, scube = ctx.split_imgs
            ctx.split_imgs = None
            want_table = P_table is not None
            dqkv, slab, rows = attention_bwd_split(hi, lo, None if P_table is None else P_table.detach().contiguous(), scube, o.view(B, N, Cc),
                                                   do.view(B, N, Cc), lse, B, N, heads, D, scale, index32 if want_table else None, n_bins or 0,
                                                   pair=planes)
        else:
            if ctx.table_in_kernel:
                tab, cube = P_table.detach().contiguous(), index32._dm_cube
            want_table = bias is not None or tab is not None
            dqkv, slab, rows = attention_bwd(qkv, bias, o, do, lse, B, N, heads, D, scale,
                                             index32 if want_table else None, n_bins or 0, bias_t=bias_t, table=tab, cube=cube)
        dtable, k_t = None, False
        if want_table:
            dtable, k_t = _grad_out(P_table, (n_bins, heads), dev)
            relpos_bias_scatter(slab, dtable, B, heads, rows, n_bins, accumulate=_acc(P_table, k_t))
        dqkv2 = dqkv if isinstance(dqkv, Planes) else dqkv.view(M, 3 * Cc)
        dwq, k_wq = _grad_out(P_qkv_w, (3 * Cc, Cc), dev)
        dbq, k_bq = _grad_out(P_qkv_b, (3 * Cc,), dev)
        dqkv_op, cs = bias_grad(dqkv2, dbq, _acc(P_qkv_b, k_bq), k_bq)
        wgrad(DM_TN, dqkv_op, y1, dwq, 3 * Cc, Cc, M, lda=3 * Cc, ldb=Cc, ldc=Cc, accumulate=_acc(P_qkv_w, k_wq), pair=True, **cs)
        dy1 = torch.empty((M, Cc), dtype=dtype, device=dev)
        gemm(DM_NN, dqkv_op, wq, dy1, M, Cc, 3 * Cc, lda=3 * Cc, ldb=Cc, ldc=Cc)
        dg1, k_n1 = _grad_out(P_n1w, (Cc,), dev)
        dbt1, k_n1b = _grad_out(P_n1b, (Cc,), dev)
        if k_n1 != k_n1b:
            dg1, dbt1, k_n1, k_n1b = torch.empty(Cc, device=dev), torch.empty(Cc, device=dev), False, False
        a_n1 = _acc(P_n1w, k_n1)
        _acc(P_n1b, k_n1b)
        regroup = ctx.lp_rows if (lp and dtype == torch.bfloat16 and _FUSED_GLUE and Cc <= _PAIR_LN_MAX_COLS) else None
        r = layernorm_bwd(dy1, x, n1w, mean1, rstd1, dres=dx1, dgamma=dg1, dbeta=dbt1, accumulate=a_n1, want_lp=lp, defer=bool(k_n1 and k_n1b),
                          want_pair=planes, regroup=regroup)
        if side is not None:
            torch.cuda.current_stream().wait_stream(side)
        if pending:
            gemm_grouped(pending)
        if late:
            gemm_grouped(late)
        dx = r[0].view(B, N, Cc)
        if regroup is not None:
            dx._dm_lp_regrouped = (r[1], _grad_tag(dx), regroup)
        elif lp:
            dx._dm_lp_copy = (r[1], _grad_tag(dx))
        if planes:
            dx._dm_planes = (r[1], _grad_tag(dx))
        return (dx, _grad_done(P_n1w, dg1, k_n1), _grad_done(P_n1b, dbt1, k_n1b),
                _grad_done(P_table, dtable, k_t) if want_table else None, None,
                _grad_done(P_qkv_w, dwq, k_wq), _grad_done(P_qkv_b, dbq, k_bq),
                _grad_done(P_proj_w, dwp, k_wp), _grad_done(P_proj_b, dbp, k_bp),
                _grad_done(P_n2w, dg2, k_n2), _grad_done(P_n2b, dbt2, k_n2b),
                _grad_done(P_fc1_w, dw1, k_w1), _grad_done(P_fc1_b, db1, k_b1),
                _grad_done(P_fc2_w, dw2, k_w2), _grad_done(P_fc2_b, db2, k_b2), None, None, None, None)
```

include/deepmerge_hip.h:

```cpp
#ifndef DEEPMERGE_HIP_H
#define DEEPMERGE_HIP_H

#include <stdint.h>

#ifdef __cplusplus
extern "C" {
#endif

typedef enum { DM_F32 = 0, DM_BF16 = 1,
               DM_BF16_PAIR = 2,
               DM_F64 = 3
} DmDtype;

typedef enum {
  DM_OK = 0,
  DM_ERR_BAD_SHAPE = -1,
  DM_ERR_BAD_DTYPE = -2,
  DM_ERR_BAD_ALIGN = -3,
  DM_ERR_WORKSPACE = -4,
  DM_ERR_HIP = -5,
  DM_ERR_UNSUPPORTED = -6
} DmStatus;

int dm_abi_version(void);
const char *dm_last_error(void);
const char *dm_arch(void);

typedef enum { DM_NT = 0, DM_NN = 1, DM_TN = 2 } DmGemmLayout;
typedef enum { DM_EPI_NONE = 0, DM_EPI_GELU = 1, DM_EPI_DGELU = 2, DM_EPI_GELU_GRAD = 3, DM_EPI_MUL = 4 } DmEpilogue;

typedef struct {
  int32_t layout;
  int32_t ab_dtype;
  int32_t c_dtype;
  int32_t aux_dtype;
  int32_t M, N, K;
  int32_t epilogue;
  int32_t accumulate;
  int32_t split_k;
  const void *A; int64_t lda;
  const void *B; int64_t ldb;
  void *C; int64_t ldc;
  const float *bias;
  const float *residual; int64_t ldr;
  void *aux; int64_t ldaux;
  int32_t rows_per_group; int64_t group_stride;
  void *workspace; int64_t workspace_bytes;
  float *colsum_a; int32_t colsum_accumulate;
  int32_t k_fold;
  int64_t a_fold[3], b_fold[3];
  int64_t c_plane;
} DmGemmArgs;

int dm_gemm(const DmGemmArgs *args, void *stream);
int64_t dm_gemm_workspace_bytes(int32_t layout, int32_t M, int32_t N, int32_t K);
int dm_gemm_grouped(const DmGemmArgs *args, int32_t n, void *stream);

int dm_attention_fwd(const void *qkv, const float *bias, void *out, float *lse,
                     int32_t B, int32_t N, int32_t H, int32_t D, float scale, int32_t dtype, void *stream);
int32_t dm_attention_relpos_inkernel(int32_t B, int32_t N, int32_t H, int32_t D, int32_t cube_s, int32_t cube_h,
                                     int32_t cube_w, int32_t dtype);
int dm_attention_fwd_relpos(const void *qkv, const float *table, int32_t cube_s, int32_t cube_h, int32_t cube_w,
                            void *out, float *lse, int32_t B, int32_t N, int32_t H, int32_t D, float scale,
                            int32_t dtype, void *stream);
int dm_attention_bwd(const void *qkv, const float *bias, const float *bias_t, const void *out, const void *dout,
                     const float *lse, void *dqkv, float *delta, float *dbias_slab, int32_t B, int32_t N, int32_t H,
                     int32_t D, float scale, int32_t dtype, void *stream);
int dm_attention_bwd_relpos(const void *qkv, const float *table, int32_t cube_s, int32_t cube_h, int32_t cube_w,
                            const float *bias, const float *bias_t, const void *out, const void *dout, const float *lse,
                            void *dqkv, float *delta, float *dbias_slab, int32_t B, int32_t N, int32_t H, int32_t D,
                            float scale, int32_t dtype, void *stream);
int32_t dm_attention_split_ok(int32_t B, int32_t N, int32_t H, int32_t D, int32_t has_table, int32_t cube_s, int32_t cube_h,
                              int32_t cube_w);
int dm_attention_split_fwd(const float *qkv, void *qkv_hi, void *qkv_lo, const float *table, int32_t cube_s, int32_t cube_h,
                           int32_t cube_w, float *out, float *lse, int32_t B, int32_t N, int32_t H, int32_t D, float scale,
                           void *stream);
int dm_attention_split_fwd_pair(const float *qkv, void *qkv_hi, void *qkv_lo, const float *table, int32_t cube_s, int32_t cube_h,
                                int32_t cube_w, float *out, void *out_pair, float *lse, int32_t B, int32_t N, int32_t H, int32_t D,
                                float scale, void *stream);
int32_t dm_attention_split_bwd_chunks(int32_t B, int32_t N, int32_t H);
int dm_attention_split_bwd(const void *qkv_hi, const void *qkv_lo, const float *table, int32_t cube_s, int32_t cube_h,
                           int32_t cube_w, const float *out, const float *dout, void *dout_hi, void *dout_lo,
                           const float *lse, float *dqkv, float *delta, float *dbias_slab, int32_t B, int32_t N,
                           int32_t H, int32_t D, float scale, void *stream);
int dm_attention_split_bwd_pair(const void *qkv_hi, const void *qkv_lo, const float *table, int32_t cube_s, int32_t cube_h,
                                int32_t cube_w, const float *out, const float *dout, void *dout_hi, void *dout_lo,
                                const float *lse, void *dqkv_pair, float *delta, float *dbias_slab, int32_t B, int32_t N,
                                int32_t H, int32_t D, float scale, void *stream);
int32_t dm_attention_bwd_batch_chunks(int32_t B, int32_t N, int32_t H, int32_t dtype);

int dm_relpos_bias_gather(const float *table, const int32_t *index, float *bias, float *bias_t,
                          int32_t N, int32_t H, int32_t n_bins, void *stream);
int dm_relpos_bias_reduce(float *dbias_slab, const int32_t *positions, const int32_t *offsets, float *dtable,
                          int32_t chunks, int32_t H, int32_t N, int32_t n_bins, int32_t accumulate, void *stream);

int dm_layernorm_fwd(const float *x, const float *gamma, const float *beta, void *y, int32_t y_dtype,
                     float *mean, float *rstd, int32_t rows, int32_t cols, float eps, void *stream);
int dm_layernorm_bwd(const void *dy, int32_t dy_dtype, const float *x, const float *gamma,
                     const float *mean, const float *rstd, const float *dres, float *dx, void *dx_lp,
                     float *dgamma, float *dbeta, int32_t accumulate_params, float *partial,
                     int32_t rows, int32_t cols, void *stream);
int64_t dm_layernorm_bwd_partial_floats(int32_t cols);
int dm_layernorm_bwd_partials(const void *dy, int32_t dy_dtype, const float *x, const float *gamma,
                              const float *mean, const float *rstd, const float *dres, float *dx, void *dx_lp,
                              float *partial, int32_t rows, int32_t cols, int32_t *n_partial, void *stream);
int dm_layernorm_bwd_partials_pair(const void *dy, int32_t dy_dtype, const float *x, const float *gamma,
                                   const float *mean, const float *rstd, const float *dres, float *dx, void *dx_pair, float *partial,
                                   int32_t rows, int32_t cols, int32_t *n_partial, void *stream);
int dm_layernorm_bwd_partials_regroup(const void *dy, int32_t dy_dtype, const float *x, const float *gamma,
                                      const float *mean, const float *rstd, const float *dres, float *dx, void *dx_lp, float *partial,
                                      int32_t rows, int32_t cols, int32_t S, int32_t T, int32_t *n_partial, void *stream);
typedef struct DmReduceItem {
  const float *partial;
  float *out0, *out1;
  int32_t nrows, width, split, accumulate;
} DmReduceItem;
int dm_partial_reduce_batch(const DmReduceItem *items, int32_t n, void *stream);

int dm_token_pool_fwd(const float *x, float *y, int32_t B, int32_t S, int32_t side, int32_t C, void *stream);
int dm_token_pool_bwd(const float *dy, float *dx, int32_t B, int32_t S, int32_t side, int32_t C, void *stream);
int dm_pool_layernorm_ok(int32_t C);
int dm_pool_layernorm_fwd(const float *x, const float *gamma, const float *beta, float *pooled, float *y, float *mean, float *rstd,
                          int32_t B, int32_t S, int32_t side, int32_t C, float eps, void *stream);
int dm_pool_layernorm_bwd(const float *dy, const float *pooled, const float *gamma, const float *mean, const float *rstd, float *dx,
                          void *dx_lp, float *dgamma, float *dbeta, int32_t accumulate_params, float *partial, int32_t *n_partial,
                          int32_t B, int32_t S, int32_t side, int32_t C, void *stream);
int dm_group_mean_fwd(const float *x, float *y, int32_t rows, int32_t g, int32_t C, void *stream);
int dm_group_mean_bwd(const float *dy, float *dx, int32_t rows, int32_t g, int32_t C, void *stream);

int dm_colsum(const void *X, int32_t dtype, int64_t ldx, float *out, int32_t M, int32_t N,
              int32_t accumulate, float *partial, void *stream);
int64_t dm_colsum_partial_floats(int32_t N);

int dm_cast(const float *src, void *dst, int32_t dst_dtype, int64_t n, void *stream);

int dm_split_bf16(const float *src, int64_t ld, int64_t rows, int64_t cols, void *dst, int32_t stack, int32_t pattern, void *stream);
int64_t dm_split_colsum_partial_floats(int64_t rows, int64_t cols);
int dm_split_bf16_planes(const float *src, int64_t ld, int64_t rows, int64_t cols, void *dst, float *partial, int32_t *n_partial, void *stream);
int dm_split_bf16_colsum(const float *src, int64_t ld, int64_t rows, int64_t cols, void *dst, int32_t stack, int32_t pattern,
                         float *partial, int32_t *n_partial, void *stream);

int dm_patchify(const float *x, void *cols, int32_t dtype, int32_t B, int32_t C, int32_t side, int32_t p, void *stream);

int dm_contrastive_loss(const float *a, const float *b, const float *flag, float margin, float upstream,
                        float *loss, float *da, float *db, int32_t B, int32_t D, void *stream);

int dm_cross_entropy(const float *logits, const int64_t *target_index, const float *target_prob, float upstream,
                     float *loss, float *dlogits, int32_t B, int32_t K, void *stream);

int dm_adam_step(float *param, const float *grad, float *m, float *v, void *param_lp, int64_t n,
                 int32_t step, double lr, double beta1, double beta2, double eps, double grad_scale, void *stream);

int dm_adam_hyper(int32_t step, double lr, double beta1, double beta2, float *hyper_host);
int dm_adam_step_dev(float *param, const float *grad, float *m, float *v, void *param_lp, int64_t n, const float *hyper_dev,
                     double beta1, double beta2, double eps, double grad_scale, void *stream);
int dm_adam_step_dev_pair(float *param, const float *grad, float *m, float *v, void *param_hi, void *param_lo, int64_t n,
                          const float *hyper_dev, double beta1, double beta2, double eps, double grad_scale, void *stream);

int dm_segment_mean(const float *F, const int32_t *ptr, const int32_t *idx, float *pooled,
                    int32_t S, int32_t D, void *stream);
int dm_edge_similarity(const float *pooled, const int32_t *edges, float *simi, uint8_t *merge,
                       int32_t E, int32_t D, float margin, void *stream);
int dm_pairwise_distance(const void *X, const void *Y, void *D, int32_t n, int32_t m, int32_t p, int32_t dtype, void *stream);

#define DM_RESIZE_OPENCV 0
#define DM_RESIZE_EXACT_AREA 1
int dm_patch_pyramid(const uint8_t *tile, int32_t bands, int32_t H, int32_t W, const int32_t *xy, const int32_t *windows,
                     int32_t max_window, int32_t P, int32_t target, int32_t resize_rule, float *out, void *stream);
int dm_patch_pyramid_cols(const uint8_t *tile, int32_t bands, int32_t H, int32_t W, const int32_t *xy, const int32_t *windows,
                          int32_t max_window, int32_t P, int32_t target, int32_t grid, int32_t resize_rule, void *cols, int32_t dtype,
                          void *stream);

int dm_pair_batch_gather(const uint8_t *tiles, int32_t n_tiles, int32_t bands, int32_t H, int32_t W, const int32_t *tile_id,
                         const int32_t *xy, const int32_t *inner, const int32_t *obj, int32_t scale_index, int32_t max_window,
                         int32_t P, int32_t target, int32_t grid, int32_t resize_rule, void *out, int32_t dtype,
                         const float *region_features, float *designed, int32_t *error_flag, void *stream);

typedef struct {
  const int32_t *pairs, *pair_flag, *poly_off, *poly_pts;
  const int32_t *pt_tile, *pt_xy, *pt_inner, *pt_obj;
  const float *pt_region;
  int32_t *tile_id, *xy, *inner, *obj;
  float *region, *flag;
  int32_t *point_id;
  uint64_t seed;
  int32_t n_pairs, n_poly, n_poly_pts, n_pts, epoch, batch;
} DmPairDraw;
int dm_pair_epoch_draw(const DmPairDraw *args, void *stream);

int dm_contrastive_terms(const float *a, const float *b, const float *flag, float margin, float *d2, float *term, int32_t B, int32_t D,
                         void *stream);
int64_t dm_pair_eval_workspace_bytes(int64_t N, int32_t T);
int dm_pair_eval_summary(const float *term, const float *simi, const float *flag, int64_t N, const float *thresholds, int32_t T,
                         void *workspace, double *loss_sum, int64_t *merged, int64_t *n_pos, void *stream);

int dm_label_stats(const int32_t *labels, const uint8_t *tile, int32_t bands, int32_t H, int32_t W, int32_t S,
                   int64_t *count, int64_t *sum, int64_t *sumsq, int32_t *bbox, int64_t *peri, void *stream);
int dm_label_features(const int64_t *count, const int64_t *sum, const int64_t *sumsq, const int32_t *bbox, const int64_t *peri,
                      int32_t S, int32_t bands, float *features, void *stream);
int dm_rag_edges(const int32_t *labels, int32_t H, int32_t W, int32_t S, int64_t *table_keys, int32_t *table_counts,
                 int32_t capacity_log2, int64_t *edge_keys, int32_t *edge_counts, int32_t max_edges, int32_t *n_edges,
                 int32_t *overflow, void *stream);

int dm_seam_stitch(const int32_t *a, const int32_t *b, int64_t n, int64_t S, int64_t *peri, int64_t *table_keys,
                   int32_t *table_counts, int32_t capacity_log2, int64_t *edge_keys, int32_t *edge_counts, int32_t max_edges,
                   int32_t *n_edges, int32_t *overflow, void *stream);

int dm_merge_round(const int32_t *edges, const uint8_t *merge, int32_t E, int32_t S, int32_t *parent, int32_t *changed,
                   int32_t init, void *stream);

typedef struct {
  const int32_t *ptr, *idx, *edges, *root, *pick, *rep, *region_of;
  const float *simi;
  const int32_t *weights;
  const int64_t *count, *sum, *sumsq;
  const int32_t *bbox;
  const int64_t *peri;
  int32_t *new_id, *hist_rank, *new_ptr, *new_idx, *new_rep, *new_region_of, *n_regions;
  int64_t *new_count, *new_sum, *new_sumsq;
  int32_t *new_bbox;
  int64_t *new_peri;
  int32_t *history;
  float *history_simi;
  int32_t C, P, E, S0, bands, round, hist_base, hist_cap;
} DmMergeFold;
int dm_merge_best(const int32_t *edges, const float *simi, int32_t E, int32_t C, float margin, uint64_t *best, void *stream);
int dm_merge_match(const int32_t *edges, const uint64_t *best, int32_t E, int32_t C, uint8_t *picked, int32_t *root, int32_t *pick,
                   int32_t *n_picked, void *stream);
int dm_merge_fold_regions(const DmMergeFold *args, void *stream);
int dm_merge_edge_keys(const int32_t *edges, const int32_t *root, const int32_t *new_id, int32_t E, int32_t C, int64_t *keys,
                       void *stream);
int dm_merge_fold_edges(const int64_t *sorted_keys, const int64_t *order, const int32_t *weights, int32_t E, int32_t *new_edges,
                        int32_t *new_weights, int32_t *n_edges, void *stream);
int dm_relabel_raster(const int32_t *labels, const int32_t *map, int32_t *out, int64_t n, int32_t S, void *stream);

int dm_region_merge_cost(const int64_t *count, const int64_t *sum, const int64_t *sumsq, const int32_t *bbox, const int64_t *peri,
                         const int32_t *edges, const int32_t *weights, int32_t E, int32_t C, int32_t bands, double bw0, double bw1,
                         double bw2, double shape, double compactness, float *cost, void *stream);
int dm_pixel_regions(const uint8_t *tile, int32_t bands, int32_t H, int32_t W, int64_t *count, int64_t *sum, int64_t *sumsq,
                     int32_t *bbox, int64_t *peri, int32_t *edges, int32_t *weights, void *stream);

int dm_label_clearance(const int32_t *labels, int32_t H, int32_t W, int32_t max_window, uint64_t *bits, uint8_t *row_dist,
                       uint16_t *clearance, void *stream);
int dm_point_select_round(const int32_t *labels, const uint16_t *clearance, int32_t H, int32_t W, int32_t S, int32_t k, int32_t round,
                          uint64_t *best, int32_t *points, int32_t *point_clearance, int32_t *counts, int32_t *bbox, void *stream);
int dm_point_emit(const int32_t *counts, const int32_t *points, const int32_t *point_clearance, const int32_t *bbox, int32_t S, int32_t k,
                  int32_t max_window, int32_t capacity, int32_t *ptr, int32_t *xy, int32_t *label, int32_t *inner, int32_t *obj,
                  int32_t *round, void *stream);

#define DM_SCENE_POINTS_MAX_PIXELS (1LL << 48)
int dm_scene_point_init(uint64_t *best, int32_t *counts, int32_t *bbox, int32_t S, void *stream);
int dm_scene_point_select(const int32_t *labels, const uint16_t *clearance, int32_t wh, int32_t ww, int32_t cy0, int32_t cy1,
                          int32_t cx0, int32_t cx1, int64_t oy, int64_t ox, int64_t scene_h, int64_t scene_w, int32_t S, int32_t k,
                          int32_t round, const int32_t *points, const int32_t *counts, uint64_t *best, int32_t *bbox, void *stream);
int dm_scene_point_commit(uint64_t *best, int64_t scene_h, int64_t scene_w, int32_t S, int32_t k, int32_t *points,
                          int32_t *point_clearance, int32_t *counts, void *stream);

int dm_label_overlap(const int32_t *labels, const int32_t *truth, int32_t H, int32_t W, int64_t S, int64_t G, int64_t *table_keys,
                     int32_t *table_counts, int32_t capacity_log2, int64_t *cell_keys, int32_t *cell_counts, int32_t max_cells,
                     int32_t *n_cells, int32_t *overflow, void *stream);
int dm_overlap_reduce(const int64_t *cell_keys, const int32_t *cell_counts, int32_t K, int64_t S, int64_t G, uint64_t *row_best,
                      int64_t *row_labelled, int64_t *area, int32_t *owner, int32_t *owner_count, int64_t *size, int32_t *cover,
                      int64_t *summary, void *stream);
int dm_pair_flags(const int32_t *edges, int32_t E, const int64_t *area, const int32_t *owner, const int32_t *owner_count, int32_t S,
                  int32_t purity_pm, int8_t *flags, void *stream);

#define DM_BOUNDARY_MAX_TOLERANCE 64
int dm_boundary_bits(const int32_t *raster, int32_t H, int32_t W, int32_t n_ids, const int32_t *mapping, uint64_t *edge,
                     uint64_t *valid, void *stream);
int dm_boundary_counts(const uint64_t *label_edge, const uint64_t *truth_edge, const uint64_t *truth_valid, int32_t H, int32_t W,
                       int32_t d, int32_t y0, int32_t y1, int32_t x0, int32_t x1, int64_t *counts, void *stream);
// ... 209 lines not shown
```

Before: 6508 pairs/s.

## Batch small row kernels into a grouped job-table launch

Adds a generic row-jobs kernel that dispatches chunk-sum, relpos-bias reduce, partial reduce and patchify work from one launch using a job table. Relpos table gradient reductions in backward are deferred and flushed together with the pending layernorm partial reductions, and the multi-scale patch embedding patchifies all scales in a single launch. The aim is to cut kernel launch count and per-launch host overhead for many tiny kernels. In exchange the reductions are delayed to the autograd callback, the ctypes job marshalling gets more complex, and the fused kernel uses shared memory even for job kinds that do not need it.

```diff
diff --git a/deepmerge_amd/_lib.py b/deepmerge_amd/_lib.py
--- a/deepmerge_amd/_lib.py
+++ b/deepmerge_amd/_lib.py
@@ -45,6 +45,31 @@
 class DmReduceItem(C.Structure):
     _fields_ = [("partial", C.c_void_p), ("out0", C.c_void_p), ("out1", C.c_void_p),
                 ("nrows", C.c_int32), ("width", C.c_int32), ("split", C.c_int32), ("accumulate", C.c_int32)]
+
+
+DM_ROWJOB_CHUNK_SUM, DM_ROWJOB_RELPOS_REDUCE, DM_ROWJOB_PARTIAL_REDUCE, DM_ROWJOB_PATCHIFY = 0, 1, 2, 3
+
+
+class _RowJobChunkSum(C.Structure):
+    _fields_ = [("slab", C.c_void_p), ("plane4", C.c_int64), ("chunks", C.c_int32)]
+
+
+class _RowJobRelpos(C.Structure):
+    _fields_ = [("slab", C.c_void_p), ("positions", C.c_void_p), ("offsets", C.c_void_p), ("dtable", C.c_void_p),
+                ("chunks", C.c_int32), ("H", C.c_int32), ("N", C.c_int32), ("n_bins", C.c_int32), ("accumulate", C.c_int32)]
+
+
+class _RowJobPatchify(C.Structure):
+    _fields_ = [("x", C.c_void_p), ("cols", C.c_void_p), ("dtype", C.c_int32), ("B", C.c_int32), ("C", C.c_int32), ("side", C.c_int32),
+                ("p", C.c_int32)]
+
+
+class _RowJobUnion(C.Union):
+    _fields_ = [("chunk_sum", _RowJobChunkSum), ("relpos", _RowJobRelpos), ("reduce", DmReduceItem), ("patchify", _RowJobPatchify)]
+
+
+class DmRowJob(C.Structure):
+    _fields_ = [("kind", C.c_int32), ("reserved", C.c_int32), ("u", _RowJobUnion)]
 
 
 class DmPairDraw(C.Structure):
@@ -152,6 +177,8 @@
     "dm_pool_layernorm_fwd": (_I, [_P, _P, _P, _P, _P, _P, _P, _I, _I, _I, _I, _F, _P]),
     "dm_pool_layernorm_bwd": (_I, [_P, _P, _P, _P, _P, _P, _P, _P, _P, _I, _P, C.POINTER(C.c_int32), _I, _I, _I, _I, _P]),
     "dm_partial_reduce_batch": (_I, [C.POINTER(DmReduceItem), _I, _P]),
+    "dm_row_jobs": (_I, [C.POINTER(DmRowJob), _I, _P]),
+    "dm_relpos_bias_reduce_jobs": (_I, [_P, _P, _P, _P, _I, _I, _I, _I, _I, C.POINTER(DmRowJob), C.POINTER(C.c_int32)]),
     "dm_layernorm_bwd_partial_floats": (_L, [_I]),
     "dm_token_pool_fwd": (_I, [_P, _P, _I, _I, _I, _I, _P]),
     "dm_token_pool_bwd": (_I, [_P, _P, _I, _I, _I, _I, _P]),
diff --git a/deepmerge_amd/csrc/dm_rows.hip b/deepmerge_amd/csrc/dm_rows.hip
--- a/deepmerge_amd/csrc/dm_rows.hip
+++ b/deepmerge_amd/csrc/dm_rows.hip
@@ -1,6 +1,8 @@
 #include <cstdlib>
+#include <cstring>
 
 #include "dm_common.h"
+#include "dm_prof.h"
 
 int dm_layernorm_wide_fwd(const float *x, const float *gamma, const float *beta, void *y, int y_dtype, float *mean, float *rstd, int rows,
                           int cols, float eps, hipStream_t s);
@@ -302,12 +304,10 @@
   }
 }
 
-__global__ __launch_bounds__(256) void partial_reduce_kernel(const float *__restrict__ partial, float *__restrict__ out0,
-                                                             float *__restrict__ out1, int nrows, int width, int split,
-                                                             int accumulate) {
-  __shared__ float red[16][17];
+__device__ __forceinline__ void partial_reduce_body(float (&red)[16][17], const float *__restrict__ partial, float *__restrict__ out0,
+                                                    float *__restrict__ out1, int nrows, int width, int split, int accumulate, int bx) {
   const int tx = threadIdx.x & 15, ty = threadIdx.x >> 4;
-  const int j = blockIdx.x * 16 + tx;
+  const int j = bx * 16 + tx;
   float s = 0.f;
   if (j < width) {
     float s0 = 0.f, s1 = 0.f, s2 = 0.f, s3 = 0.f;
@@ -335,6 +335,13 @@
     float *o = (j < split) ? out0 + j : out1 + (j - split);
     *o = accumulate ? *o + s : s;
   }
+}
+
+__global__ __launch_bounds__(256) void partial_reduce_kernel(const float *__restrict__ partial, float *__restrict__ out0,
+                                                             float *__restrict__ out1, int nrows, int width, int split,
+                                                             int accumulate) {
+  __shared__ float red[16][17];
+  partial_reduce_body(red, partial, out0, out1, nrows, width, split, accumulate, blockIdx.x);
 }
 
 struct ReduceBatch {
@@ -347,37 +354,7 @@
   int job = 0;
   while (job + 1 < rb.n && (int)blockIdx.x >= rb.start[job + 1]) ++job;
   const DmReduceItem &it = rb.it[job];
-  const float *__restrict__ partial = it.partial;
-  const int nrows = it.nrows, width = it.width;
-  const int tx = threadIdx.x & 15, ty = threadIdx.x >> 4;
-  const int j = ((int)blockIdx.x - rb.start[job]) * 16 + tx;
-  float s = 0.f;
-  if (j < width) {
-    float s0 = 0.f, s1 = 0.f, s2 = 0.f, s3 = 0.f;
-    int r = ty;
-    for (; r + 48 < nrows; r += 64) {
-      s0 += partial[(long long)r * width + j];
-      s1 += partial[(long long)(r + 16) * width + j];
-      s2 += partial[(long long)(r + 32) * width + j];
-      s3 += partial[(long long)(r + 48) * width + j];
-    }
-    for (; r < nrows; r += 16) s0 += partial[(long long)r * width + j];
-    s = (s0 + s1) + (s2 + s3);
-  }
-  red[ty][tx] = s;
-  __syncthreads();
-  if (ty == 0 && j < width) {
-    float t[16];
-#pragma unroll
-    for (int k = 0; k < 16; ++k) t[k] = red[k][tx];
-#pragma unroll
-    for (int w = 8; w > 0; w >>= 1)
-#pragma unroll
-      for (int k = 0; k < w; ++k) t[k] = t[2 * k] + t[2 * k + 1];
-    s = t[0];
-    float *o = (j < it.split) ? it.out0 + j : it.out1 + (j - it.split);
-    *o = it.accumulate ? *o + s : s;
-  }
+  partial_reduce_body(red, it.partial, it.out0, it.out1, it.nrows, it.width, it.split, it.accumulate, (int)blockIdx.x - rb.start[job]);
 }
 
 __global__ void token_pool_fwd_kernel(const float *__restrict__ x, float *__restrict__ y, int B, int S, int side, int C) {
@@ -538,11 +515,11 @@
 }
 
 template <typename T>
-__global__ void patchify_kernel(const float *__restrict__ x, T *__restrict__ cols, int B, int C, int side, int p) {
+__device__ __forceinline__ void patchify_body(const float *__restrict__ x, T *__restrict__ cols, int B, int C, int side, int p, int bx, int gx) {
   const int grid = side / p, p4 = p >> 2;
   const long long K = (long long)C * p * p;
   const long long total = (long long)B * grid * grid * (K >> 2);
-  for (long long i = (long long)blockIdx.x * blockDim.x + threadIdx.x; i < total; i += (long long)gridDim.x * blockDim.x) {
+  for (long long i = (long long)bx * blockDim.x + threadIdx.x; i < total; i += (long long)gx * blockDim.x) {
     long long r = i;
     const int dx4 = (int)(r % p4); r /= p4;
     const int dy = (int)(r % p); r /= p;
@@ -554,6 +531,10 @@
     const f32x4 v = dm_load4(x + ((b * C + c) * side + (py * p + dy)) * (long long)side + px * p + 4 * dx4);
     dm_store4(cols + r * K + ((long long)c * p + dy) * p + 4 * dx4, v);
   }
+}
+template <typename T>
+__global__ void patchify_kernel(const float *__restrict__ x, T *__restrict__ cols, int B, int C, int side, int p) {
+  patchify_body<T>(x, cols, B, C, side, p, blockIdx.x, gridDim.x);
 }
 
 __global__ __launch_bounds__(256) void contrastive_loss_kernel(const float *__restrict__ a, const float *__restrict__ b,
@@ -695,8 +676,8 @@
 #pragma unroll
   for (int u = 0; u < U; ++u) v += a[u];
 }
-__global__ void chunk_sum_kernel(float *__restrict__ slab, long long plane4, int chunks) {
-  for (long long i = (long long)blockIdx.x * blockDim.x + threadIdx.x; i < plane4; i += (long long)gridDim.x * blockDim.x) {
+__device__ __forceinline__ void chunk_sum_body(float *__restrict__ slab, long long plane4, int chunks, int bx, int gx) {
+  for (long long i = (long long)bx * blockDim.x + threadIdx.x; i < plane4; i += (long long)gx * blockDim.x) {
     f32x4 v = dm_load4(slab + 4 * i);
     int c = 1;
     for (; c + 8 <= chunks; c += 8) chunk_add<8>(v, slab, plane4, i, c);
@@ -706,12 +687,15 @@
     dm_store4(slab + 4 * i, v);
   }
 }
-
-__global__ __launch_bounds__(256) void relpos_reduce_kernel(const float *__restrict__ slab, const int *__restrict__ pos,
-                                                            const int *__restrict__ off, float *__restrict__ dtable, int chunks,
-                                                            int H, int N, int n_bins, int accumulate) {
+__global__ void chunk_sum_kernel(float *__restrict__ slab, long long plane4, int chunks) {
+  chunk_sum_body(slab, plane4, chunks, blockIdx.x, gridDim.x);
+}
+
+__device__ __forceinline__ void relpos_reduce_body(const float *__restrict__ slab, const int *__restrict__ pos, const int *__restrict__ off,
+                                                   float *__restrict__ dtable, int chunks, int H, int N, int n_bins, int accumulate,
+                                                   int bx, int by) {
   const int lane = threadIdx.x & 63, wave = threadIdx.x >> 6;
-  const int bin = blockIdx.x, h = blockIdx.y * 4 + wave;
+  const int bin = bx, h = by * 4 + wave;
   if (h >= H) return;
   const int beg = off[bin], cnt = off[bin + 1] - beg;
   const long long plane = (long long)N * N;
@@ -727,6 +711,49 @@
     *o = accumulate ? *o + acc : acc;
   }
 }
+__global__ __launch_bounds__(256) void relpos_reduce_kernel(const float *__restrict__ slab, const int *__restrict__ pos,
+                                                            const int *__restrict__ off, float *__restrict__ dtable, int chunks,
+                                                            int H, int N, int n_bins, int accumulate) {
+  relpos_reduce_body(slab, pos, off, dtable, chunks, H, N, n_bins, accumulate, blockIdx.x, blockIdx.y);
+}
+
+constexpr int ROW_JOBS_MAX = 16;
+struct RowJobTable {
+  DmRowJob job[ROW_JOBS_MAX];
+  int first[ROW_JOBS_MAX + 1];
+  int gx[ROW_JOBS_MAX];
+  int n;
+};
+__global__ __launch_bounds__(256) void row_jobs_kernel(const RowJobTable t) {
+  __shared__ float red[16][17];
+  const int b = blockIdx.x;
+  if (b >= t.first[t.n]) return;
+  int j = 0;
+  while (j + 1 < t.n && b >= t.first[j + 1]) ++j;
+  const DmRowJob &jb = t.job[j];
+  const int l = b - t.first[j], gx = t.gx[j];
+  const int bx = l % gx, by = l / gx;
+  switch (jb.kind) {
+    case DM_ROWJOB_CHUNK_SUM:
+      chunk_sum_body(jb.u.chunk_sum.slab, jb.u.chunk_sum.plane4, jb.u.chunk_sum.chunks, bx, gx);
+      break;
+    case DM_ROWJOB_RELPOS_REDUCE:
+      relpos_reduce_body(jb.u.relpos.slab, jb.u.relpos.positions, jb.u.relpos.offsets, jb.u.relpos.dtable, jb.u.relpos.chunks, jb.u.relpos.H,
+                         jb.u.relpos.N, jb.u.relpos.n_bins, jb.u.relpos.accumulate, bx, by);
+      break;
+    case DM_ROWJOB_PARTIAL_REDUCE:
+      partial_reduce_body(red, jb.u.reduce.partial, jb.u.reduce.out0, jb.u.reduce.out1, jb.u.reduce.nrows, jb.u.reduce.width,
+                          jb.u.reduce.split, jb.u.reduce.accumulate, bx);
+      break;
+    case DM_ROWJOB_PATCHIFY:
+      if (jb.u.patchify.dtype == DM_F32)
+        patchify_body<float>(jb.u.patchify.x, (float *)jb.u.patchify.cols, jb.u.patchify.B, jb.u.patchify.C, jb.u.patchify.side, jb.u.patchify.p, bx, gx);
+      else
+        patchify_body<bf16_t>(jb.u.patchify.x, (bf16_t *)jb.u.patchify.cols, jb.u.patchify.B, jb.u.patchify.C, jb.u.patchify.side, jb.u.patchify.p, bx, gx);
+      break;
+    default: break;
+  }
+}
 
 inline int grid_for(long long work_items, int block = 256, int cap = 4096) {
   long long g = (work_items + block - 1) / block;
@@ -740,6 +767,93 @@
   return grid_for(n / 4 + 1, 256, cap);
 }
 
+inline int chunk_sum_grid(long long plane4) { return grid_for(plane4, 256, 2048); }
+inline int partial_reduce_grid(int width) { return (width + 15) / 16; }
+inline int patchify_grid(int B, int C, int side, int p) {
+  return grid_for((long long)B * (side / p) * (side / p) * ((long long)C * p * p / 4));
+}
+int relpos_reduce_check(const float *slab, const int32_t *positions, const int32_t *offsets, const float *dtable, int chunks, int H, int N,
+                        int n_bins) {
+  DM_REQUIRE(slab && positions && offsets && dtable && chunks > 0 && H > 0 && N > 0 && n_bins > 0, DM_ERR_BAD_SHAPE,
+             "dm_relpos_bias_reduce: bad arguments");
+  DM_REQUIRE(n_bins <= 65535 * 32, DM_ERR_BAD_SHAPE, "dm_relpos_bias_reduce: too many bins (%d)", n_bins);
+  return DM_OK;
+}
+int row_job_grid(const DmRowJob &jb, int index, int *gx, long long *gy) {
+  *gy = 1;
+  switch (jb.kind) {
+    case DM_ROWJOB_CHUNK_SUM: {
+      const auto &a = jb.u.chunk_sum;
+      DM_REQUIRE(a.slab && a.plane4 >= 1 && a.chunks >= 1, DM_ERR_BAD_SHAPE, "dm_row_jobs: job %d (chunk_sum): plane4=%lld chunks=%d", index,
+                 (long long)a.plane4, a.chunks);
+      DM_REQUIRE(dm_aligned16(a.slab), DM_ERR_BAD_ALIGN, "dm_row_jobs: job %d (chunk_sum): the slab must be 16-byte aligned", index);
+      *gx = chunk_sum_grid(a.plane4);
+      return DM_OK;
+    }
+    case DM_ROWJOB_RELPOS_REDUCE: {
+      const auto &a = jb.u.relpos;
+      const int rc = relpos_reduce_check(a.slab, a.positions, a.offsets, a.dtable, a.chunks, a.H, a.N, a.n_bins);
+      if (rc != DM_OK) return rc;
+      *gx = a.n_bins;
+      *gy = (a.H + 3) / 4;
+      return DM_OK;
+    }
+    case DM_ROWJOB_PARTIAL_REDUCE: {
+      const DmReduceItem &it = jb.u.reduce;
+      DM_REQUIRE(it.partial && it.out0 && it.out1 && it.nrows > 0 && it.width > 0 && it.split >= 0 && it.split <= it.width, DM_ERR_BAD_SHAPE,
+                 "dm_row_jobs: job %d (partial_reduce): nrows=%d width=%d split=%d", index, it.nrows, it.width, it.split);
+      *gx = partial_reduce_grid(it.width);
+      return DM_OK;
+    }
+    case DM_ROWJOB_PATCHIFY: {
+      const auto &a = jb.u.patchify;
+      DM_REQUIRE(a.x && a.cols && a.B > 0 && a.C > 0 && a.p > 0 && a.side > 0 && a.side % a.p == 0, DM_ERR_BAD_SHAPE,
+                 "dm_row_jobs: job %d (patchify): B=%d C=%d side=%d patch=%d (patch must divide side)", index, a.B, a.C, a.side, a.p);
+      DM_REQUIRE(a.p % 4 == 0, DM_ERR_UNSUPPORTED, "dm_row_jobs: job %d (patchify): patch=%d is not a multiple of 4 (use dm_patchify)", index, a.p);
+      DM_REQUIRE(a.dtype == DM_F32 || a.dtype == DM_BF16, DM_ERR_BAD_DTYPE, "dm_row_jobs: job %d (patchify): bad dtype %d", index, a.dtype);
+      DM_REQUIRE(dm_aligned16(a.x) && dm_aligned16(a.cols), DM_ERR_BAD_ALIGN, "dm_row_jobs: job %d (patchify): x and cols must be 16-byte aligned", index);
+      *gx = patchify_grid(a.B, a.C, a.side, a.p);
+      return DM_OK;
+    }
+    default:
+      DM_REQUIRE(false, DM_ERR_BAD_SHAPE, "dm_row_jobs: job %d: bad kind %d", index, jb.kind);
+  }
+  return DM_OK;
+}
+
+}
+
+extern "C" int dm_row_jobs(const DmRowJob *jobs, int32_t n, void *stream) {
+  DM_REQUIRE(jobs && n >= 1, DM_ERR_BAD_SHAPE, "dm_row_jobs: no jobs");
+  hipStream_t s = reinterpret_cast<hipStream_t>(stream);
+  for (int32_t base = 0; base < n; base += ROW_JOBS_MAX) {
+    long long total = 0;
+    for (int32_t i = base; i < n && i < base + ROW_JOBS_MAX; ++i) {
+      int gx = 0;
+      long long gy = 0;
+      const int rc = row_job_grid(jobs[i], i, &gx, &gy);
+      if (rc != DM_OK) return rc;
+      total += gx * gy;
+    }
+    DM_REQUIRE(total <= 0x7fffffffLL, DM_ERR_BAD_SHAPE, "dm_row_jobs: jobs %d.. need %lld workgroups", base, total);
+  }
+  for (int32_t base = 0; base < n; base += ROW_JOBS_MAX) {
+    RowJobTable t = {};
+    t.n = (n - base < ROW_JOBS_MAX) ? n - base : ROW_JOBS_MAX;
+    int total = 0;
+    for (int i = 0; i < t.n; ++i) {
+      long long gy = 0;
+      t.job[i] = jobs[base + i];
+      row_job_grid(t.job[i], base + i, &t.gx[i], &gy);
+      t.first[i] = total;
+      total += (int)(t.gx[i] * gy);
+    }
+    for (int i = t.n; i <= ROW_JOBS_MAX; ++i) t.first[i] = total;
+    DmProfScope prof("small_jobs", s, 0.0, 0.0);
+    hipLaunchKernelGGL(row_jobs_kernel, dim3(total), dim3(256), 0, s, t);
+    DM_LAUNCH_CHECK("dm_row_jobs");
+  }
+  return DM_OK;
 }
 
 extern "C" int dm_layernorm_fwd(const float *x, const float *gamma, const float *beta, void *y, int32_t y_dtype,
@@ -903,7 +1017,7 @@
                  "dm_partial_reduce_batch: item %d: nrows=%d width=%d split=%d", base + i, it.nrows, it.width, it.split);
       rb.it[i] = it;
       rb.start[i] = total;
-      total += (it.width + 15) / 16;
+      total += partial_reduce_grid(it.width);
     }
     for (int i = rb.n; i <= 32; ++i) rb.start[i] = total;
     hipLaunchKernelGGL(partial_reduce_batch_kernel, dim3(total), dim3(256), 0, s, rb);
@@ -1061,9 +1175,9 @@
     DM_LAUNCH_CHECK("dm_patchify(any)");
     return DM_OK;
   }
-  const long long total = (long long)B * (side / p) * (side / p) * ((long long)C * p * p / 4);
-  if (dtype == DM_F32) hipLaunchKernelGGL(patchify_kernel<float>, dim3(grid_for(total)), dim3(256), 0, s, x, (float *)cols, B, C, side, p);
-  else if (dtype == DM_BF16) hipLaunchKernelGGL(patchify_kernel<bf16_t>, dim3(grid_for(total)), dim3(256), 0, s, x, (bf16_t *)cols, B, C, side, p);
+  const int grid = patchify_grid(B, C, side, p);
+  if (dtype == DM_F32) hipLaunchKernelGGL(patchify_kernel<float>, dim3(grid), dim3(256), 0, s, x, (float *)cols, B, C, side, p);
+  else if (dtype == DM_BF16) hipLaunchKernelGGL(patchify_kernel<bf16_t>, dim3(grid), dim3(256), 0, s, x, (bf16_t *)cols, B, C, side, p);
   else DM_REQUIRE(false, DM_ERR_BAD_DTYPE, "dm_patchify: bad dtype %d", dtype);
   DM_LAUNCH_CHECK("dm_patchify");
   return DM_OK;
@@ -1143,17 +1257,49 @@
 }
 extern "C" int dm_relpos_bias_reduce(float *dbias_slab, const int32_t *positions, const int32_t *offsets, float *dtable,
                                      int32_t chunks, int32_t H, int32_t N, int32_t n_bins, int32_t accumulate, void *stream) {
-  DM_REQUIRE(dbias_slab && positions && offsets && dtable && chunks > 0 && H > 0 && N > 0 && n_bins > 0, DM_ERR_BAD_SHAPE,
-             "dm_relpos_bias_reduce: bad arguments");
-  DM_REQUIRE(n_bins <= 65535 * 32, DM_ERR_BAD_SHAPE, "dm_relpos_bias_reduce: too many bins (%d)", n_bins);
+  DmRowJob jobs[2];
+  int32_t n = 0;
+  const int rc = dm_relpos_bias_reduce_jobs(dbias_slab, positions, offsets, dtable, chunks, H, N, n_bins, accumulate, jobs, &n);
+  if (rc != DM_OK) return rc;
+  hipStream_t s = reinterpret_cast<hipStream_t>(stream);
+  if (n == 2) {
+    const auto &c = jobs[0].u.chunk_sum;
+    hipLaunchKernelGGL(chunk_sum_kernel, dim3(chunk_sum_grid(c.plane4)), dim3(256), 0, s, c.slab, (long long)c.plane4, c.chunks);
+  }
+  const auto &r = jobs[n - 1].u.relpos;
+  hipLaunchKernelGGL(relpos_reduce_kernel, dim3(r.n_bins, (r.H + 3) / 4), dim3(256), 0, s, r.slab, r.positions, r.offsets, r.dtable, r.chunks, r.H,
+                     r.N, r.n_bins, r.accumulate);
+  DM_LAUNCH_CHECK("dm_relpos_bias_reduce");
+  return DM_OK;
+}
+extern "C" int dm_relpos_bias_reduce_jobs(float *dbias_slab, const int32_t *positions, const int32_t *offsets, float *dtable, int32_t chunks,
+                                          int32_t H, int32_t N, int32_t n_bins, int32_t accumulate, DmRowJob *jobs_out, int32_t *n_out) {
+  const int rc = relpos_reduce_check(dbias_slab, positions, offsets, dtable, chunks, H, N, n_bins);
+  if (rc != DM_OK) return rc;
+  DM_REQUIRE(jobs_out && n_out, DM_ERR_BAD_SHAPE, "dm_relpos_bias_reduce_jobs: jobs_out and n_out must be set");
   const long long plane = (long long)H * N * N;
+  int32_t n = 0;
   if (chunks > 1 && plane % 4 == 0 && dm_aligned16(dbias_slab)) {
-    hipLaunchKernelGGL(chunk_sum_kernel, dim3(grid_for(plane / 4, 256, 2048)), dim3(256), 0, reinterpret_cast<hipStream_t>(stream), dbias_slab,
-                       plane / 4, chunks);
+    DmRowJob &c = jobs_out[n++];
+    memset(&c, 0, sizeof(c));
+    c.kind = DM_ROWJOB_CHUNK_SUM;
+    c.u.chunk_sum.slab = dbias_slab;
+    c.u.chunk_sum.plane4 = plane / 4;
+    c.u.chunk_sum.chunks = chunks;
     chunks = 1;
   }
-  hipLaunchKernelGGL(relpos_reduce_kernel, dim3(n_bins, (H + 3) / 4), dim3(256), 0, reinterpret_cast<hipStream_t>(stream), dbias_slab,
-                     positions, offsets, dtable, chunks, H, N, n_bins, accumulate);
-  DM_LAUNCH_CHECK("dm_relpos_bias_reduce");
-  return DM_OK;
-}
+  DmRowJob &r = jobs_out[n++];
+  memset(&r, 0, sizeof(r));
+  r.kind = DM_ROWJOB_RELPOS_REDUCE;
+  r.u.relpos.slab = dbias_slab;
+  r.u.relpos.positions = positions;
+  r.u.relpos.offsets = offsets;
+  r.u.relpos.dtable = dtable;
+  r.u.relpos.chunks = chunks;
+  r.u.relpos.H = H;
+  r.u.relpos.N = N;
+  r.u.relpos.n_bins = n_bins;
+  r.u.relpos.accumulate = accumulate;
+  *n_out = n;
+  return DM_OK;
+}
diff --git a/deepmerge_amd/nets/ShfitScaleFormer.py b/deepmerge_amd/nets/ShfitScaleFormer.py
--- a/deepmerge_amd/nets/ShfitScaleFormer.py
+++ b/deepmerge_amd/nets/ShfitScaleFormer.py
@@ -63,10 +63,13 @@
         self.norm = norm_layer(out_c) if norm_layer else nn.Identity()
         self.numerics = _mode(numerics, self)
 
-    def operand_rows(self, x):
+    def check_size(self, x):
         B, C, H, W = x.shape
         assert H == self.img_size[0] and W == self.img_size[1], \
             f"Input image size ({H}*{W}) doesn't match model ({self.img_size[0]}*{self.img_size[1]})."
+
+    def operand_rows(self, x):
+        self.check_size(x)
         if isinstance(x, ops.PatchCols):
             if x.patch != self.patch_size[0] or x.cols.dtype != ops.act_dtype(self.numerics):
                 raise ValueError("PatchCols were built for another patch size / numerics mode")
@@ -270,7 +273,12 @@
         layers = list(self.patch_embed_blocks)
         if not all(type(l) is PatchEmbed and isinstance(l.norm, nn.Identity) and l.num_patches == layers[0].num_patches for l in layers):
             return torch.cat([layer(x[i]) for i, layer in enumerate(layers)], 1)
-        cols = [l.operand_rows(x[i]) for i, l in enumerate(layers)]
+        if ops._JOB_GROUPS and not any(isinstance(x[i], ops.PatchCols) for i in range(len(layers))) and len({l.numerics for l in layers}) == 1:
+            for i, l in enumerate(layers):
+                l.check_size(x[i])
+            cols = ops.patchify_group([x[i].float() for i in range(len(layers))], [l.patch_size[0] for l in layers], ops.act_dtype(layers[0].numerics))
+        else:
+            cols = [l.operand_rows(x[i]) for i, l in enumerate(layers)]
         return ops.PatchEmbedCatFn.apply(len(layers), layers[0].num_patches, *cols, *[l.proj.weight for l in layers], *[l.proj.bias for l in layers])
 
     def designed_feature_embed(self, x):
diff --git a/deepmerge_amd/ops.py b/deepmerge_amd/ops.py
--- a/deepmerge_amd/ops.py
+++ b/deepmerge_amd/ops.py
@@ -361,6 +361,7 @@
 
 
 _pending_reduce = []
+_pending_tables = []
 _pending_out = set()
 _flush_queued = False
 _flush_task = -1
@@ -373,35 +374,62 @@
 def flush_reductions() -> None:
     global _flush_queued
     _flush_queued = False
-    if not _pending_reduce:
+    if not _pending_reduce and not _pending_tables:
         return
-    items = (_lib.DmReduceItem * len(_pending_reduce))()
-    for i, (f, _keep) in enumerate(_pending_reduce):
-        items[i].partial, items[i].out0, items[i].out1, items[i].nrows, items[i].width, items[i].split, items[i].accumulate = f
-    n = len(_pending_reduce)
-    keep = list(_pending_reduce)
+    keep, tables = list(_pending_reduce), list(_pending_tables)
     _pending_reduce.clear()
+    _pending_tables.clear()
     _pending_out.clear()
-    check(_lib.lib().dm_partial_reduce_batch(items, n, _stream()), "dm_partial_reduce_batch")
-    del keep
-
-
-def _queue_reduce(part, out0, out1, nrows, width, split, accumulate) -> None:
+    if not tables:
+        items = (_lib.DmReduceItem * len(keep))()
+        for i, (f, _keep) in enumerate(keep):
+            items[i].partial, items[i].out0, items[i].out1, items[i].nrows, items[i].width, items[i].split, items[i].accumulate = f
+        check(_lib.lib().dm_partial_reduce_batch(items, len(keep), _stream()), "dm_partial_reduce_batch")
+        return
+    sums = [job for jobs, _keep in tables for job in jobs[:-1]]
+    rest = []
+    for f, _keep in keep:
+        job = _lib.DmRowJob()
+        job.kind = _lib.DM_ROWJOB_PARTIAL_REDUCE
+        r = job.u.reduce
+        r.partial, r.out0, r.out1, r.nrows, r.width, r.split, r.accumulate = f
+        rest.append(job)
+    rest += [jobs[-1] for jobs, _keep in tables]
+    if sums:
+        _launch_row_jobs(sums)
+    _launch_row_jobs(rest)
+
+
+def _launch_row_jobs(jobs) -> None:
+    arr = (_lib.DmRowJob * len(jobs))(*jobs)
+    check(_lib.lib().dm_row_jobs(arr, len(jobs), _stream()), "dm_row_jobs")
+
+
+def _queue_enter(keys) -> None:
     global _flush_queued, _flush_task
     task = torch._C._current_graph_task_id()
     if task != _flush_task:
         _pending_reduce.clear()
+        _pending_tables.clear()
         _pending_out.clear()
         _flush_queued = False
         _flush_task = task
-    keys = (out0.data_ptr(), out1.data_ptr())
-    if keys[0] in _pending_out or keys[1] in _pending_out:
+    if any(k in _pending_out for k in keys):
         flush_reductions()
-    _pending_reduce.append(((part.data_ptr(), keys[0], keys[1], int(nrows), int(width), int(split), int(bool(accumulate))), (part, out0, out1)))
     _pending_out.update(keys)
     if not _flush_queued:
-        torch.autograd.Variable._execution_engine.queue_callback(flush_reductions)
+        _book_flush()
         _flush_queued = True
+
+
+def _book_flush() -> None:
+    torch.autograd.Variable._execution_engine.queue_callback(flush_reductions)
+
+
+def _queue_reduce(part, out0, out1, nrows, width, split, accumulate) -> None:
+    keys = (out0.data_ptr(), out1.data_ptr())
+    _queue_enter(keys)
+    _pending_reduce.append(((part.data_ptr(), keys[0], keys[1], int(nrows), int(width), int(split), int(bool(accumulate))), (part, out0, out1)))
 
 
 def _reduce_partials(part, dgamma, dbeta, n_part, cols, accumulate, deferred) -> None:
@@ -475,6 +503,7 @@
 
 _DEFER_REDUCTIONS = os.environ.get("DM_DEFER_REDUCTIONS", "1") != "0"
 _FUSED_GLUE = os.environ.get("DM_FUSED_GLUE", "1") != "0"
+_JOB_GROUPS = os.environ.get("DM_JOB_GROUPS", "1") != "0"
 
 
 def relpos_bias_gather(table: torch.Tensor, index32: torch.Tensor, N: int, transposed: bool = False):
@@ -628,9 +657,16 @@
     return dqkv, slab, info
 
 
-def relpos_bias_scatter(slab, dtable, B, H, info, n_bins, accumulate=False):
+def relpos_bias_scatter(slab, dtable, B, H, info, n_bins, accumulate=False, defer=False):
     _need_cuda(slab, dtable)
     chunks, N, (positions, offsets) = info
+    if defer and _JOB_GROUPS and _DEFER_REDUCTIONS and _in_backward():
+        jobs, n = (_lib.DmRowJob * 2)(), C.c_int32(0)
+        check(_lib.lib().dm_relpos_bias_reduce_jobs(slab.data_ptr(), positions.data_ptr(), offsets.data_ptr(), dtable.data_ptr(), chunks, H, N,
+                                                    n_bins, int(accumulate), jobs, C.byref(n)), "dm_relpos_bias_reduce_jobs")
+        _queue_enter((dtable.data_ptr(),))
+        _pending_tables.append(([_lib.DmRowJob.from_buffer_copy(jobs[i]) for i in range(n.value)], (slab, positions, offsets, dtable)))
+        return dtable
     check(_lib.lib().dm_relpos_bias_reduce(slab.data_ptr(), positions.data_ptr(), offsets.data_ptr(), dtable.data_ptr(), chunks, H, N,
                                            n_bins, int(accumulate), _stream()), "dm_relpos_bias_reduce")
     return dtable
@@ -646,6 +682,28 @@
     cols = torch.empty((B * g * g, Cc * patch * patch), dtype=dtype, device=x.device)
     check(_lib.lib().dm_patchify(x.data_ptr(), cols.data_ptr(), _dt(cols), B, Cc, H, patch, _stream()), "dm_patchify")
     return cols
+
+
+def patchify_group(xs, patches, dtype: torch.dtype):
+    xs = [x.contiguous() for x in xs]
+    _need_cuda(*xs)
+    if (not _JOB_GROUPS or len(xs) < 2 or any(p % 4 != 0 or x.shape[2] != x.shape[3] or x.shape[2] % p != 0 or x.data_ptr() % 16 != 0
+                                              or x.dtype != torch.float32 for x, p in zip(xs, patches))):
+        return [patchify(x, p, dtype) for x, p in zip(xs, patches)]
+    out, jobs = [], []
+    for x, p in zip(xs, patches):
+        B, Cc, H, _ = x.shape
+        g = H // p
+        cols = torch.empty((B * g * g, Cc * p * p), dtype=dtype, device=x.device)
+        job = _lib.DmRowJob()
+        job.kind = _lib.DM_ROWJOB_PATCHIFY
+        a = job.u.patchify
+        a.x, a.cols, a.dtype, a.B, a.C, a.side, a.p = x.data_ptr(), cols.data_ptr(), _dt(cols), B, Cc, H, p
+        out.append(cols)
+        jobs.append(job)
+    order = sorted(range(len(jobs)), key=lambda i: -xs[i].numel())
+    _launch_row_jobs([jobs[i] for i in order])
+    return out
 
 
 RESIZE_RULES = {"opencv": 0, "exact_area": 1}
@@ -1655,7 +1713,7 @@
         dtable, k_t = None, False
         if want_table:
             dtable, k_t = _grad_out(P_table, (n_bins, heads), dev)
-            relpos_bias_scatter(slab, dtable, B, heads, rows, n_bins, accumulate=_acc(P_table, k_t))
+            relpos_bias_scatter(slab, dtable, B, heads, rows, n_bins, accumulate=_acc(P_table, k_t), defer=bool(k_t))
         dqkv2 = dqkv if isinstance(dqkv, Planes) else dqkv.view(M, 3 * Cc)
         dwq, k_wq = _grad_out(P_qkv_w, (3 * Cc, Cc), dev)
         dbq, k_bq = _grad_out(P_qkv_b, (3 * Cc,), dev)
diff --git a/include/deepmerge_hip.h b/include/deepmerge_hip.h
--- a/include/deepmerge_hip.h
+++ b/include/deepmerge_hip.h
@@ -117,6 +117,22 @@
 } DmReduceItem;
 int dm_partial_reduce_batch(const DmReduceItem *items, int32_t n, void *stream);
 
+enum { DM_ROWJOB_CHUNK_SUM = 0, DM_ROWJOB_RELPOS_REDUCE = 1, DM_ROWJOB_PARTIAL_REDUCE = 2, DM_ROWJOB_PATCHIFY = 3, DM_ROWJOB_KINDS = 4 };
+typedef struct DmRowJob {
+  int32_t kind;
+  int32_t reserved;
+  union {
+    struct { float *slab; int64_t plane4; int32_t chunks; } chunk_sum;
+    struct { const float *slab; const int32_t *positions; const int32_t *offsets; float *dtable;
+             int32_t chunks, H, N, n_bins, accumulate; } relpos;
+    DmReduceItem reduce;
+    struct { const float *x; void *cols; int32_t dtype, B, C, side, p; } patchify;
+  } u;
+} DmRowJob;
+int dm_row_jobs(const DmRowJob *jobs, int32_t n, void *stream);
+int dm_relpos_bias_reduce_jobs(float *dbias_slab, const int32_t *positions, const int32_t *offsets, float *dtable, int32_t chunks,
+                               int32_t H, int32_t N, int32_t n_bins, int32_t accumulate, DmRowJob *jobs_out, int32_t *n_out);
+
 int dm_token_pool_fwd(const float *x, float *y, int32_t B, int32_t S, int32_t side, int32_t C, void *stream);
 int dm_token_pool_bwd(const float *dy, float *dx, int32_t B, int32_t S, int32_t side, int32_t C, void *stream);
 int dm_pool_layernorm_ok(int32_t C);
```

Result: no change. 6555 pairs/s (median of 6 runs) (+0.7%).
